# thomasdeppisch/eMagLS

Measured on AMD Instinct MI355X. Metric: eMagLS filter sets/s (N=4, 2702 dirs, 512 taps), higher is better.
Workload: dtype f64; 1 GPU; BASELINE config 3: getEMagLsFilters em32 r=4.2cm N=4 complex-SH, 2702 dirs, 512 taps, 48 kHz; one filter set per step, inputs resident in HBM; dirs=2702, taps=512, sim_order=19, bins=512, k_cut=43, designs_resident_per_gpu=128, designs_per_batch=32, batches_in_flight=4, distinct_hrir_sets_resident=20, parallelism=independent jobs per GPU, one RCCL gather

## Files before the change

emagls_amd/_lib.py:

```python
from __future__ import annotations

import ctypes as C
import os

_HERE = os.path.dirname(os.path.abspath(__file__))
LIB_PATH = os.environ.get("EMAGLS_LIB_PATH") or os.path.join(_HERE, "lib", "libemagls.so")

OK, ERR_ARG, ERR_UNSUPPORTED, ERR_HIP, ERR_NUMERIC = 0, 1, 2, 3, 4
BASIS = {"real": 0, "complex": 1}
KIND_LS, KIND_MAGLS, KIND_EMAGLS, KIND_EMAGLS2, KIND_FROM_ATF, KIND_EMA_CH, KIND_MAGLS_2D, KIND_EMA_SH = range(8)
RADIAL = {"tikhonov": 0, "softlimit": 1, "full": 2, "none": 3}
LAYOUT = {"sh": 0, "ch": 1}
MODEL = {"sh": 0, "emagls": 1, "emagls2": 2, "atf": 3, "ema_ch": 5, "ema_sh": 6}

c_dp = C.POINTER(C.c_double)
c_i64 = C.c_int64


class DesignDesc(C.Structure):
    _fields_ = [("kind", C.c_int), ("basis", C.c_int), ("order", C.c_int), ("fs", C.c_double), ("len", c_i64),
                ("nsamp", c_i64), ("ndirs", c_i64), ("mic_radius", C.c_double), ("nmics", c_i64),
                ("f_trans", C.c_double), ("atf_taps", c_i64), ("natf", c_i64), ("custom_basis", C.c_int),
                ("diffuseness", C.c_int), ("sim_order_pad", C.c_int)]


class PlanInfo(C.Structure):
    _fields_ = [("nfft", C.c_int), ("num_pos_freqs", C.c_int), ("k_cut", C.c_int), ("sim_order", C.c_int),
                ("num_sh_sim", C.c_int), ("num_channels", C.c_int), ("out_is_complex", C.c_int),
                ("out_rows", c_i64), ("out_cols", c_i64), ("grp_delay_l", C.c_double), ("grp_delay_r", C.c_double),
                ("mean_grid_dev_deg", C.c_double), ("num_sweep_launches", C.c_int), ("device_bytes", c_i64),
                ("gram_from", C.c_int), ("hh_end", C.c_int), ("hh_orders", C.c_int), ("g_first", C.c_int),
                ("sim_order_own", C.c_int), ("sweep_form", C.c_int), ("sweep_units", C.c_int)]


class Job(C.Structure):
    _fields_ = [("desc", DesignDesc), ("hL", C.c_void_p), ("hR", C.c_void_p), ("hrir_azi", C.c_void_p), ("hrir_zen", C.c_void_p),
                ("mic_azi", C.c_void_p), ("mic_zen", C.c_void_p), ("atf", C.c_void_p), ("atf_azi", C.c_void_p), ("atf_zen", C.c_void_p),
                ("wL", C.c_void_p), ("wR", C.c_void_p)]


JOBS_SHARE_GEOMETRY = 1
JOBS_INDEPENDENT = 2

SYMBOLS = {
    "emagls_last_error": (C.c_char_p, []),
    "emagls_version": (C.c_int, []),
    "emagls_device_count": (C.c_int, [C.POINTER(C.c_int)]),
    "emagls_set_device": (C.c_int, [C.c_int]),
    "emagls_cache_clear": (C.c_int, []),
    "emagls_cache_release_designs": (C.c_int, []),
    "emagls_fp64_peak_tflops": (C.c_int, [C.c_int, C.POINTER(C.c_double)]),
    "emagls_fp64_peak_tflops_ex": (C.c_int, [C.c_int, C.c_int, C.POINTER(C.c_double), C.POINTER(C.c_double)]),
    "emagls_self_test": (C.c_int, [C.c_int, C.POINTER(C.c_double)]),
    "emagls_debug_synth_operand": (C.c_int, [C.c_void_p, C.c_int, C.c_int, C.c_void_p, c_i64, C.c_int, C.c_void_p, C.c_void_p]),
    "emagls_debug_synth_cosines": (C.c_int, [C.c_void_p, C.c_void_p, c_i64, C.c_void_p, C.c_void_p, C.c_int, C.c_void_p]),
    "emagls_sh_basis": (C.c_int, [C.c_int, c_i64, C.c_void_p, C.c_void_p, C.c_int, C.c_void_p]),
    "emagls_sh_basis_device": (C.c_int, [C.c_int, c_i64, C.c_void_p, C.c_void_p, C.c_int, C.c_void_p, C.c_void_p]),
    "emagls_modal_bn": (C.c_int, [C.c_int, c_i64, C.c_void_p, C.c_void_p]),
    "emagls_get_ls_filters": (C.c_int, [C.c_void_p, C.c_void_p, c_i64, c_i64, C.c_void_p, C.c_void_p, C.c_int, C.c_int,
                                        C.c_void_p, C.c_void_p]),
    "emagls_get_magls_filters": (C.c_int, [C.c_void_p, C.c_void_p, c_i64, c_i64, C.c_void_p, C.c_void_p, C.c_int,
                                           C.c_double, c_i64, C.c_int, C.c_void_p, C.c_void_p]),
    "emagls_get_emagls_filters": (C.c_int, [C.c_void_p, C.c_void_p, c_i64, c_i64, C.c_void_p, C.c_void_p, C.c_double,
                                            C.c_void_p, C.c_void_p, c_i64, C.c_int, C.c_double, c_i64, C.c_int,
                                            C.c_void_p, C.c_void_p]),
    "emagls_get_emagls2_filters": (C.c_int, [C.c_void_p, C.c_void_p, c_i64, c_i64, C.c_void_p, C.c_void_p, C.c_double,
                                             C.c_void_p, C.c_void_p, c_i64, C.c_int, C.c_double, c_i64, C.c_int,
                                             C.c_void_p, C.c_void_p]),
    "emagls_get_emagls_filters_ema_in_ch": (C.c_int, [C.c_void_p, C.c_void_p, c_i64, c_i64, C.c_void_p, C.c_void_p, C.c_double,
                                                      C.c_void_p, c_i64, C.c_int, C.c_double, c_i64, C.c_int, C.c_void_p, C.c_void_p]),
    "emagls_get_emagls_filters_ema_in_sh": (C.c_int, [C.c_void_p, C.c_void_p, c_i64, c_i64, C.c_void_p, C.c_void_p, C.c_double,
                                                      C.c_void_p, c_i64, C.c_int, C.c_double, c_i64, C.c_int, C.c_void_p, C.c_void_p]),
    "emagls_get_emagls_filters_from_atf": (C.c_int, [C.c_void_p, C.c_void_p, c_i64, c_i64, C.c_void_p, C.c_void_p,
                                                     C.c_void_p, c_i64, c_i64, c_i64, C.c_void_p, C.c_void_p,
                                                     C.c_double, c_i64, C.c_double, C.c_void_p, C.c_void_p,
                                                     C.POINTER(C.c_double)]),
    "emagls_simulation_order": (C.c_int, [C.c_int, C.c_int, C.c_double, C.c_double]),
    "emagls_get_ls_filters_with_basis": (C.c_int, [C.c_void_p, C.c_void_p, c_i64, c_i64, C.c_void_p, C.c_int, C.c_int, C.c_void_p, C.c_void_p]),
    "emagls_get_magls_filters_with_basis": (C.c_int, [C.c_void_p, C.c_void_p, c_i64, c_i64, C.c_void_p, C.c_int, C.c_double, c_i64, C.c_int,
                                                      C.c_void_p, C.c_void_p]),
    "emagls_get_emagls_filters_with_basis": (C.c_int, [C.c_void_p, C.c_void_p, c_i64, c_i64, C.c_void_p, C.c_double, C.c_void_p, c_i64, C.c_int,
                                                       C.c_double, c_i64, C.c_int, C.c_void_p, C.c_void_p]),
    "emagls_get_emagls2_filters_with_basis": (C.c_int, [C.c_void_p, C.c_void_p, c_i64, c_i64, C.c_void_p, C.c_double, C.c_void_p, c_i64, C.c_int,
                                                        C.c_double, c_i64, C.c_int, C.c_void_p, C.c_void_p]),
    "emagls_plan_set_basis": (C.c_int, [C.c_void_p, C.c_void_p, C.c_void_p]),
    "emagls_binaural_decode": (C.c_int, [C.c_void_p, c_i64, c_i64, C.c_void_p, C.c_void_p, c_i64, C.c_int, C.c_void_p]),
    "emagls_binaural_decode_complex": (C.c_int, [C.c_void_p, C.c_int, c_i64, c_i64, C.c_void_p, C.c_void_p, C.c_int, c_i64, C.c_int,
                                                 C.c_void_p, C.c_void_p]),
    "emagls_binaural_decode_device": (C.c_int, [C.c_void_p, C.c_int, c_i64, c_i64, C.c_void_p, C.c_void_p, C.c_int, c_i64, C.c_void_p,
                                                C.c_void_p, C.c_void_p]),
    "emagls_rotate_yaw": (C.c_int, [C.c_void_p, C.c_int, c_i64, c_i64, C.c_int, C.c_int, C.c_void_p, c_i64, C.c_void_p]),
    "emagls_binaural_decode_render": (C.c_int, [C.c_void_p, C.c_int, c_i64, c_i64, C.c_void_p, C.c_void_p, C.c_int, c_i64, C.c_int,
                                                C.c_int, C.c_int, C.c_void_p, c_i64, C.c_void_p, c_i64, C.c_void_p, C.c_void_p]),
    "emagls_binaural_decode_render_device": (C.c_int, [C.c_void_p, C.c_int, c_i64, c_i64, C.c_void_p, C.c_void_p, C.c_int, c_i64,
                                                       C.c_int, C.c_int, C.c_void_p, c_i64, C.c_void_p, c_i64, C.c_void_p, C.c_void_p,
                                                       C.c_void_p]),
    "emagls_sh_rotation_matrix": (C.c_int, [C.c_int, C.c_int, C.c_double, C.c_double, C.c_double, C.c_void_p]),
    "emagls_rotate_sh": (C.c_int, [C.c_void_p, C.c_int, c_i64, c_i64, C.c_int, C.c_void_p, c_i64, C.c_void_p, c_i64, C.c_void_p, c_i64,
                                   C.c_void_p]),
    "emagls_binaural_decode_render_ypr": (C.c_int, [C.c_void_p, C.c_int, c_i64, c_i64, C.c_void_p, C.c_void_p, C.c_int, c_i64, C.c_int,
                                                    C.c_int, C.c_int, C.c_void_p, c_i64, C.c_void_p, c_i64, C.c_void_p, c_i64,
                                                    C.c_void_p, c_i64, C.c_void_p, C.c_void_p]),
    "emagls_binaural_decode_render_ypr_device": (C.c_int, [C.c_void_p, C.c_int, c_i64, c_i64, C.c_void_p, C.c_void_p, C.c_int, c_i64,
                                                           C.c_int, C.c_int, C.c_void_p, c_i64, C.c_void_p, c_i64, C.c_void_p, c_i64,
                                                           C.c_void_p, c_i64, C.c_void_p, C.c_void_p, C.c_void_p]),
    "emagls_resample_length": (c_i64, [c_i64, c_i64, c_i64]),
    "emagls_resample": (C.c_int, [C.c_void_p, C.c_int, c_i64, c_i64, c_i64, c_i64, C.c_void_p]),
    "emagls_resample_device": (C.c_int, [C.c_void_p, C.c_int, c_i64, c_i64, c_i64, c_i64, C.c_void_p, C.c_void_p]),
    "emagls_binaural_decode_render_fs": (C.c_int, [C.c_void_p, C.c_int, c_i64, c_i64, C.c_void_p, C.c_void_p, C.c_int, c_i64, C.c_int,
                                                   C.c_int, C.c_int, C.c_void_p, c_i64, C.c_void_p, c_i64, C.c_void_p, c_i64,
                                                   C.c_void_p, c_i64, C.c_double, C.c_double, C.c_double, C.c_void_p, C.c_void_p]),
    "emagls_binaural_decode_render_fs_device": (C.c_int, [C.c_void_p, C.c_int, c_i64, c_i64, C.c_void_p, C.c_void_p, C.c_int, c_i64,
                                                          C.c_int, C.c_int, C.c_void_p, c_i64, C.c_void_p, c_i64, C.c_void_p, c_i64,
                                                          C.c_void_p, c_i64, C.c_double, C.c_double, C.c_double, C.c_void_p,
                                                          C.c_void_p, C.c_void_p]),
    "emagls_decode_stream_create": (C.c_int, [c_i64, C.c_void_p, C.c_void_p, C.c_int, c_i64, C.c_int, C.c_int, C.c_int, c_i64,
                                              C.POINTER(C.c_void_p)]),
    "emagls_decode_stream_push": (C.c_int, [C.c_void_p, C.c_void_p, c_i64, C.c_void_p, c_i64, C.c_void_p, c_i64, C.c_void_p, c_i64,
                                            C.c_void_p]),
    "emagls_decode_stream_push_device": (C.c_int, [C.c_void_p, C.c_void_p, c_i64, C.c_void_p, c_i64, C.c_void_p, c_i64, C.c_void_p, c_i64,
                                                   C.c_void_p, C.c_void_p]),
    "emagls_decode_stream_reset": (C.c_int, [C.c_void_p]),
    "emagls_decode_stream_info": (C.c_int, [C.c_void_p, C.POINTER(c_i64), C.POINTER(c_i64), C.POINTER(c_i64), C.POINTER(c_i64),
                                            C.POINTER(C.c_int)]),
    "emagls_decode_stream_destroy": (C.c_int, [C.c_void_p]),
    "emagls_decode_stream_create_bank": (C.c_int, [c_i64, c_i64, C.c_void_p, C.c_void_p, C.c_int, c_i64, C.c_int, C.c_int, C.c_int, c_i64,
                                                   C.POINTER(C.c_void_p)]),
    "emagls_decode_stream_push_sets": (C.c_int, [C.c_void_p, C.c_void_p, c_i64, C.c_void_p, c_i64, C.c_void_p, c_i64, C.c_void_p, c_i64,
                                                 C.c_void_p, c_i64, C.c_void_p]),
    "emagls_decode_stream_push_sets_device": (C.c_int, [C.c_void_p, C.c_void_p, c_i64, C.c_void_p, c_i64, C.c_void_p, c_i64, C.c_void_p,
                                                        c_i64, C.c_void_p, c_i64, C.c_void_p, C.c_void_p]),
    "emagls_decode_stream_sets": (C.c_int, [C.c_void_p, C.POINTER(c_i64)]),
    "emagls_decode_group_create": (C.c_int, [c_i64, c_i64, C.c_void_p, C.c_void_p, C.c_int, c_i64, C.c_int, C.c_int, C.c_int, c_i64, c_i64,
                                             C.POINTER(C.c_void_p)]),
    "emagls_decode_group_push": (C.c_int, [C.c_void_p, C.c_void_p, c_i64, C.c_void_p, c_i64, C.c_void_p, c_i64, C.c_void_p, c_i64,
                                           C.c_void_p, c_i64, C.c_void_p]),
    "emagls_decode_group_push_device": (C.c_int, [C.c_void_p, C.c_void_p, c_i64, C.c_void_p, c_i64, C.c_void_p, c_i64, C.c_void_p, c_i64,
                                                  C.c_void_p, c_i64, C.c_void_p, C.c_void_p]),
    "emagls_decode_group_reset": (C.c_int, [C.c_void_p, c_i64]),
    "emagls_decode_group_info": (C.c_int, [C.c_void_p, C.POINTER(c_i64), C.POINTER(c_i64), C.POINTER(c_i64), C.POINTER(c_i64),
                                           C.POINTER(c_i64), C.POINTER(C.c_int)]),
    "emagls_decode_group_destroy": (C.c_int, [C.c_void_p]),
    "emagls_decode_stream_create_encoded": (C.c_int, [c_i64, C.c_void_p, C.c_int, c_i64, c_i64, C.c_void_p, C.c_void_p, C.c_int, c_i64, C.c_int,
                                                      C.c_int, c_i64, C.POINTER(C.c_void_p)]),
    "emagls_decode_group_create_encoded": (C.c_int, [c_i64, C.c_void_p, C.c_int, c_i64, c_i64, C.c_void_p, C.c_void_p, C.c_int, c_i64, C.c_int,
                                                     C.c_int, c_i64, c_i64, C.POINTER(C.c_void_p)]),
    "emagls_get_magls_filters_dc": (C.c_int, [C.c_void_p, C.c_void_p, c_i64, c_i64, C.c_void_p, C.c_void_p, C.c_int,
                                              C.c_double, c_i64, C.c_int, C.c_int, C.c_void_p, C.c_void_p]),
    "emagls_get_emagls_filters_dc": (C.c_int, [C.c_void_p, C.c_void_p, c_i64, c_i64, C.c_void_p, C.c_void_p, C.c_double,
                                               C.c_void_p, C.c_void_p, c_i64, C.c_int, C.c_double, c_i64, C.c_int, C.c_int,
                                               C.c_void_p, C.c_void_p]),
    "emagls_get_emagls2_filters_dc": (C.c_int, [C.c_void_p, C.c_void_p, c_i64, c_i64, C.c_void_p, C.c_void_p, C.c_double,
                                                C.c_void_p, C.c_void_p, c_i64, C.c_int, C.c_double, c_i64, C.c_int, C.c_int,
                                                C.c_void_p, C.c_void_p]),
    "emagls_get_magls_filters_2d": (C.c_int, [C.c_void_p, C.c_void_p, c_i64, c_i64, C.c_void_p, C.c_int, C.c_double, c_i64, C.c_int,
                                              C.c_void_p, C.c_void_p]),
    "emagls_get_radial_filter": (C.c_int, [C.c_int, C.c_double, C.c_double, c_i64, C.c_int, C.c_int, C.c_double, C.c_double, C.c_void_p]),
    "emagls_apply_radial_filter_rows": (c_i64, [c_i64, c_i64, C.c_int]),
    "emagls_apply_radial_filter": (C.c_int, [C.c_void_p, c_i64, C.c_int, C.c_double, C.c_double, c_i64, C.c_int, C.c_int, C.c_double,
                                             C.c_double, C.c_void_p]),
    "emagls_sh_encode": (C.c_int, [C.c_void_p, c_i64, c_i64, C.c_void_p, C.c_void_p, C.c_int, C.c_int, C.c_void_p]),
    "emagls_ch_basis": (C.c_int, [C.c_int, c_i64, C.c_void_p, C.c_int, C.c_void_p]),
    "emagls_get_smair_matrix": (C.c_int, [C.c_int, C.c_double, c_i64, C.c_int, C.c_double, C.c_void_p, C.c_void_p, c_i64, C.c_int, C.c_int,
                                          C.c_int, C.c_double, C.c_double, C.c_void_p, C.POINTER(C.c_int)]),
    "emagls_rendered_hrtfs": (C.c_int, [C.c_int, C.c_void_p, C.c_void_p, C.c_int, c_i64, c_i64, c_i64, C.c_void_p, C.c_void_p, c_i64, C.c_double,
                                        C.c_int, C.c_int, C.c_double, C.c_void_p, C.c_void_p, c_i64, C.c_void_p, c_i64, c_i64, C.c_void_p,
                                        C.c_void_p, c_i64, c_i64, C.c_void_p, C.c_void_p, C.c_void_p, C.c_void_p, C.c_void_p, C.c_void_p]),
    "emagls_eq_filter_nfft": (c_i64, [c_i64]),
    "emagls_get_magls_spherical_head_filter": (C.c_int, [C.c_double, C.c_int, C.c_double, c_i64, C.c_void_p, C.c_void_p]),
    "emagls_get_magls_array_diffuse_filter": (C.c_int, [C.c_double, C.c_void_p, C.c_void_p, c_i64, C.c_int, C.c_double, c_i64, C.c_int,
                                                        C.c_void_p, C.c_void_p]),
    "emagls_plan_create": (C.c_int, [C.POINTER(DesignDesc), C.POINTER(C.c_void_p)]),
    "emagls_plan_destroy": (C.c_int, [C.c_void_p]),
    "emagls_plan_set_hrir_grid": (C.c_int, [C.c_void_p, C.c_void_p, C.c_void_p]),
    "emagls_plan_set_mic_grid": (C.c_int, [C.c_void_p, C.c_void_p, C.c_void_p]),
    "emagls_plan_set_hrirs": (C.c_int, [C.c_void_p, C.c_void_p, C.c_void_p]),
    "emagls_plan_set_atfs": (C.c_int, [C.c_void_p, C.c_void_p, C.c_void_p, C.c_void_p]),
    "emagls_plan_execute": (C.c_int, [C.c_void_p]),
    "emagls_plan_synchronize": (C.c_int, [C.c_void_p]),
    "emagls_plan_get_filters": (C.c_int, [C.c_void_p, C.c_void_p, C.c_void_p]),
    "emagls_plan_get_info": (C.c_int, [C.c_void_p, C.POINTER(PlanInfo)]),
    "emagls_plan_sweep_form_in_batch": (C.c_int, [C.c_void_p, C.c_int, C.POINTER(C.c_int)]),
    "emagls_plan_set_profiling": (C.c_int, [C.c_void_p, C.c_int]),
    "emagls_plan_set_streams": (C.c_int, [C.c_void_p, C.c_int]),
    "emagls_plan_num_stages": (C.c_int, [C.c_void_p]),
    "emagls_plan_stage_name": (C.c_char_p, [C.c_void_p, C.c_int]),
    "emagls_plan_stage_times": (C.c_int, [C.c_void_p, c_dp, C.c_int]),
    "emagls_plan_sweep_kernel_time": (C.c_int, [C.c_void_p, c_dp, C.POINTER(C.c_int)]),
    "emagls_plan_debug_buffer": (C.c_int, [C.c_void_p, C.c_char_p, C.c_void_p, C.POINTER(C.c_size_t)]),
    "emagls_plan_stream": (C.c_void_p, [C.c_void_p]),
    "emagls_batch_create": (C.c_int, [C.POINTER(C.c_void_p), C.c_int, C.POINTER(C.c_void_p)]),
    "emagls_batch_execute": (C.c_int, [C.c_void_p]),
    "emagls_batch_synchronize": (C.c_int, [C.c_void_p]),
    "emagls_batch_get_filters": (C.c_int, [C.c_void_p, C.POINTER(C.c_void_p), C.POINTER(C.c_void_p)]),
    "emagls_batch_set_profiling": (C.c_int, [C.c_void_p, C.c_int]),
    "emagls_batch_lane_mode": (C.c_int, [C.c_void_p, C.POINTER(C.c_int)]),
    "emagls_batch_set_stream": (C.c_int, [C.c_void_p, C.c_void_p]),
    "emagls_set_batch_max": (C.c_int, [C.c_int, C.POINTER(C.c_int)]),
    "emagls_batch_shares_atf_side": (C.c_int, [C.c_void_p, C.POINTER(C.c_int)]),
    "emagls_design_hrir_sets": (C.c_int, [C.c_int, C.c_void_p, C.c_void_p, C.c_int64, C.c_int64, C.c_int64, C.c_void_p, C.c_void_p, C.c_double,
                                          C.c_void_p, C.c_void_p, C.c_int64, C.c_int, C.c_double, C.c_int64, C.c_int, C.c_void_p, C.c_void_p]),
    "emagls_from_atf_hrir_sets": (C.c_int, [C.c_void_p, C.c_void_p, C.c_int64, C.c_int64, C.c_int64, C.c_void_p, C.c_void_p, C.c_void_p, C.c_int64,
                                            C.c_int64, C.c_int64, C.c_void_p, C.c_void_p, C.c_double, C.c_int64, C.c_double, C.c_void_p, C.c_void_p,
                                            C.POINTER(C.c_double)]),
    "emagls_jobs_run": (C.c_int, [C.POINTER(Job), C.c_int64, C.c_int, C.c_int, C.c_int]),
    "emagls_design_out_shape": (C.c_int, [C.POINTER(DesignDesc), C.POINTER(c_i64), C.POINTER(c_i64), C.POINTER(C.c_int)]),
    "emagls_jobs_shard": (C.c_int, [C.POINTER(Job), C.c_int64, C.c_int, C.c_int, C.POINTER(C.c_int), C.POINTER(C.c_int), C.POINTER(C.c_int)]),
    "emagls_jobs_run_devices": (C.c_int, [C.POINTER(Job), C.c_int64, C.POINTER(C.c_int), C.c_int, C.c_int, C.c_int, C.c_int]),
    "emagls_jobs_set_profiling": (C.c_int, [C.c_int]),
    "emagls_jobs_sweep_times": (C.c_int, [C.POINTER(C.c_double), C.POINTER(C.c_int), C.c_int, C.POINTER(C.c_int)]),
    "emagls_batch_set_geometry_sharing": (C.c_int, [C.c_void_p, C.c_int]),
    "emagls_batch_shares_geometry": (C.c_int, [C.c_void_p, C.POINTER(C.c_int)]),
    "emagls_batch_geometry_runs": (C.c_int, [C.c_void_p, C.POINTER(C.c_longlong), C.POINTER(C.c_longlong)]),
    "emagls_jobs_geometry_runs": (C.c_int, [C.POINTER(C.c_longlong), C.POINTER(C.c_longlong), C.POINTER(C.c_longlong)]),
    "emagls_jobs_would_share_geometry": (C.c_int, [C.c_void_p, C.c_int, C.POINTER(C.c_int)]),
    "emagls_batch_set_side_stream": (C.c_int, [C.c_void_p, C.c_void_p]),
    "emagls_batch_set_streams": (C.c_int, [C.c_void_p, C.c_int]),
    "emagls_batch_set_stage_order": (C.c_int, [C.c_void_p, C.c_int]),
    "emagls_batch_sweep_time": (C.c_int, [C.c_void_p, C.POINTER(C.c_double)]),
    "emagls_batch_destroy": (C.c_int, [C.c_void_p]),
}


class EmaglsError(RuntimeError):
    def __init__(self, code, msg):
        super().__init__("emagls error %d: %s" % (code, msg))
        self.code = code


_lib = None


def load():
    global _lib
    if _lib is not None:
        return _lib
    if not os.path.exists(LIB_PATH):
        raise ImportError("HIP library not built: %s is missing (run `python -m emagls_amd.build`)" % LIB_PATH)
    lib = C.CDLL(LIB_PATH, mode=C.RTLD_GLOBAL)
    for name, (res, args) in SYMBOLS.items():
        fn = getattr(lib, name)
        fn.restype = res
        fn.argtypes = args
    _lib = lib
    return lib


def check(rc):
    if rc != OK:
        raise EmaglsError(rc, load().emagls_last_error().decode("utf-8", "replace"))
```

emagls_amd/csrc/batch_run.hip:

```cpp
#include "host_internal.hpp"

void emagls_batch_forget(emagls_batch* b, emagls_plan* p) {
    for (auto& q : b->plans) if (q == p) q = nullptr;
}

namespace {
void batch_sweep_stage(emagls_batch& b) {
    const int nb = (int)b.plans.size();
    std::vector<HalfSweepArgs> ha((size_t)nb);
    for (int j = 0; j < nb; ++j) ha[j] = emagls_half_args(*b.plans[j]);
    if (b.atf_share || b.geo_share)
        for (int j = 1; j < nb; ++j) {
            ha[j].G = ha[0].G; ha[j].Yri = ha[0].Yri; ha[j].Mw = ha[0].Mw; ha[j].cond_ok = ha[0].cond_ok;
            ha[j].bsc = ha[0].bsc; ha[j].smap = ha[0].smap;
            ha[j].skip_flag = ha[0].skip_flag;
        }
    const bool reg = b.plans[0]->sweep_persist && reg_sweep_wanted(b.plans.data(), nb);
    for (auto* q : b.plans) q->reg_sweep = reg;
    if (!reg && nb > SWEEP_MULTI_MAX) throw Error(EMAGLS_ERR_UNSUPPORTED, "internal: more than 16 designs in a batch need the register-resident sweep");
    HalfSweepMulti h{};
    h.n = std::min(nb, SWEEP_MULTI_MAX);
    for (int j = 0; j < h.n; ++j) h.a[j] = ha[j];
    emagls_plan& q0 = *b.plans[0];
    const int kk0 = std::max(q0.kcut0, 1);
    if (kk0 >= q0.P) return;
    if (q0.sweep_persist) {
        hipStream_t ss = b.stream;
        {
            SweepGate gate(ss, reg ? reg_sweep_gate_cost((int)q0.D, nb) : 0);
            if (b.lanes) { BatchScope sc(nb, b.stride); launch_zero(q0.get("ll"), q0.bufs["ll"].bytes, ss); }
            else for (auto* q : b.plans) launch_zero(q->get("ll"), q->bufs["ll"].bytes, ss);
            if (reg) {
                if (!b.sweep_args_dev) HIP_CHECK(hipMalloc(&b.sweep_args_dev, sizeof(HalfSweepArgs) * (size_t)REG_SWEEP_MAX));
                reg_args_upload(ha.data(), nb, b.sweep_args_dev, b.sweep_args_last, ss);
            }
            if (b.prof_level >= 1) HIP_CHECK(hipEventRecord(b.sweep_ev[0], ss));
            if (reg) launch_sweep_reg(static_cast<const HalfSweepArgs*>(b.sweep_args_dev), ha[0], nb, ss);
            else if (q0.synth) launch_sweep_synth(h, ss); else launch_sweep_persist(h, ss);
            if (b.prof_level >= 1) HIP_CHECK(hipEventRecord(b.sweep_ev[1], ss));
        }
        if (ss != b.stream) b.depend(b.stream, ss);
        return;
    }
    for (int kb = kk0; kb < q0.P; ++kb) launch_sweep_half(h, kb, b.stream);
    launch_sweep_half_finalize(h, q0.P - 1, b.stream);
}

static int stagger_mode() {
    static const int m = [] { const char* e = getenv("EMAGLS_STAGGER"); return e ? atoi(e) : 1; }();
    return m;
}
bool batch_defers_hh(const emagls_batch& b) {
    static const int defer_mode = [] { const char* e = getenv("EMAGLS_DEFER_HH"); return e ? atoi(e) : 1; }();
    if (!b.lanes || !(b.alone || defer_mode == 2) || b.geo_share || b.atf_share) return false;
    for (const emagls_plan* p : b.plans) if (!p || !plan_defers_hh_route(*p)) return false;
    return true;
}
void batch_lanes_part(emagls_batch& b, int part, int first, int count, hipStream_t st, int group = 0) {
    emagls_plan& p0 = *b.plans[first];
    const int ns = (part == 0 && b.groups == 1) ? b.nstreams : 1;
    int order = 0;
    if (part == 0 && ns == 1) {
        const int sm = stagger_mode();
        if (sm == 1) order = b.groups > 1 ? 1 + group % 2 : (b.order_hint ? 1 + (b.order_hint - 1) % 2 : 0);
        else if (sm >= 10) order = group == 0 ? sm / 10 % 10 : sm % 10;
    }
    Scoped stream(p0.stream, st);
    Scoped nstreams(p0.nstreams, ns);
    Scoped stage_order(p0.stage_order, order);
    Scoped side0(p0.side[0], ns > 1 ? b.side[0] : p0.side[0]), side1(p0.side[1], ns > 1 ? b.side[1] : p0.side[1]),
        side2(p0.side[2], ns > 1 ? b.side[2] : p0.side[2]);
    Scoped pre_phase(p0.pre_phase, part == 3 ? 2 : (part == 0 && b.defer_hh) ? 1 : 0);
    BatchScope sc(count, b.stride);
    if (part == 0) plan_pre_stage(p0); else if (part == 3) emagls_pre_sweep(p0); else emagls_post_sweep(p0);
}
void mark_executed(emagls_batch& b, int launches) {
    for (auto* p : b.plans) { p->executed = true; p->sweep_launches = launches; }
}
int sweep_launch_count(const emagls_plan& p0) { return p0.sweep_persist ? 1 : p0.P - std::max(p0.kcut0, 1); }
int batch_group_first(const emagls_batch& b, int g) { const int n = (int)b.plans.size(), h = (n + b.groups - 1) / b.groups; return std::min(n, g * h); }
void batch_execute_lanes(emagls_batch& b) {
    const bool replay = b.use_graph && b.eager_runs >= 1 && !(b.groups == 1 && b.nstreams > 1);
    const int n = (int)b.plans.size();
    const int ng = b.groups;
    for (int g = 1; g < ng; ++g) if (!b.side[g - 1]) b.side[g - 1] = emagls::pool_stream_take();
    hipStream_t gs[4] = {b.stream, b.stream, b.stream, b.stream};
    for (int g = 1; g < ng; ++g) gs[g] = b.side[g - 1];
    if (!replay || !b.group[0]) b.defer_hh = batch_defers_hh(b);
    const bool defer = b.defer_hh;
    if (defer) for (int g = 0; g < ng; ++g) if (!b.hh_stream[g]) b.hh_stream[g] = emagls::pool_stream_take();
    if (replay && !b.group[0]) {
        for (int g = 0; g < ng; ++g) {
            const int f = batch_group_first(b, g), c = batch_group_first(b, g + 1) - f;
            b.group[g].capture(gs[g], [&] { batch_lanes_part(b, 0, f, c, gs[g], g); });
            if (defer) b.group_hh[g].capture(b.hh_stream[g], [&] { batch_lanes_part(b, 3, f, c, b.hh_stream[g], g); });
        }
        b.post.capture(b.stream, [&] { batch_lanes_part(b, 2, 0, n, b.stream); });
    }
    b.used = 0;
    for (int g = 1; g < ng; ++g) b.depend(gs[g], b.stream);
    if (replay && ng > 1) {
        hipError_t err[4] = {hipSuccess, hipSuccess, hipSuccess, hipSuccess};
        const int dev = b.device;
        std::vector<std::thread> th;
        for (int g = 1; g < ng; ++g)
            th.emplace_back([&, g] { err[g] = hipSetDevice(dev); if (err[g] == hipSuccess) err[g] = hipGraphLaunch(b.group[g].exec, gs[g]); });
        err[0] = hipGraphLaunch(b.group[0].exec, gs[0]);
        for (auto& t : th) t.join();
        for (int g = 0; g < ng; ++g) HIP_CHECK(err[g]);
    } else {
        for (int g = 0; g < ng; ++g) {
            const int f = batch_group_first(b, g), c = batch_group_first(b, g + 1) - f;
            if (replay) b.group[g].launch(gs[g]); else batch_lanes_part(b, 0, f, c, gs[g], g);
        }
    }
    if (defer) for (int g = 0; g < ng; ++g) b.depend(b.hh_stream[g], gs[g]);
    for (int g = 1; g < ng; ++g) b.depend(b.stream, gs[g]);
    batch_sweep_stage(b);
    if (defer) {
        for (int g = 0; g < ng; ++g) {
            const int f = batch_group_first(b, g), c = batch_group_first(b, g + 1) - f;
            if (replay) b.group_hh[g].launch(b.hh_stream[g]); else batch_lanes_part(b, 3, f, c, b.hh_stream[g], g);
            b.depend(b.stream, b.hh_stream[g]);
        }
    }
    if (replay) b.post.launch(b.stream); else batch_lanes_part(b, 2, 0, n, b.stream);
    mark_executed(b, sweep_launch_count(*b.plans[0]));
    if (!replay) ++b.eager_runs;
}

bool batch_inputs_same(emagls_batch& b, std::initializer_list<const char*> names, uint64_t& checked_version, bool& same) {
    uint64_t ver = 0;
    for (auto* p : b.plans) ver = ver * 1000003ull + p->atf_side_version;
    if (ver == checked_version) return same;
    if (!b.cmp_flag) HIP_CHECK(hipMalloc(&b.cmp_flag, 16));
    HIP_CHECK(hipStreamSynchronize(b.stream));
    HIP_CHECK(hipMemsetAsync(b.cmp_flag, 0, 16, b.stream));
    emagls_plan& p0 = *b.plans[0];
    for (size_t j = 1; j < b.plans.size(); ++j)
        for (const char* name : names) launch_compare_words(p0.get(name), b.plans[j]->get(name), p0.bufs[name].bytes, b.cmp_flag, b.stream);
    int differ = 0;
    HIP_CHECK(hipMemcpyAsync(&differ, b.cmp_flag, sizeof differ, hipMemcpyDeviceToHost, b.stream));
    HIP_CHECK(hipStreamSynchronize(b.stream));
    checked_version = ver;
    return same = differ == 0;
}
void batch_set_sharing(emagls_batch& b, bool& field, bool share) {
    if (share == field) return;
    for (auto* p : b.plans) drop_plan_graphs(*p);
    drop_batch_graphs(b);
    if (&field == &b.geo_share) batch_geo_forget(b);
    field = share;
}
void batch_run_two_graphs(emagls_batch& b, CapturedGraph& pre, void (*stage)(emagls_batch&, int), int pre_part, int launches) {
    const bool replay = b.use_graph && b.eager_runs >= 1;
    if (replay && !pre) pre.capture(b.stream, [&] { stage(b, pre_part); });
    if (replay && !b.post) b.post.capture(b.stream, [&] { stage(b, 2); });
    b.used = 0;
    if (replay) pre.launch(b.stream); else stage(b, pre_part);
    batch_sweep_stage(b);
    if (replay) b.post.launch(b.stream); else stage(b, 2);
    mark_executed(b, launches);
    if (!replay) ++b.eager_runs;
}
template <typename Pre> void batch_run_per_plan(emagls_batch& b, bool replay, Pre pre, void (*post)(emagls_plan&), int launches) {
    emagls_plan& p0 = *b.plans[0];
    if (replay && !p0.pre) {
        for (auto* p : b.plans) p->pre.capture(p->stream, [&] { pre(*p); });
        if (!p0.sweep_persist) b.group[0].capture(b.stream, [&] { batch_sweep_stage(b); });
    }
    b.used = 0;
    for (auto* p : b.plans) b.depend(p->stream, b.stream);
    for (auto* p : b.plans) {
        if (replay) p->pre.launch(p->stream); else pre(*p);
        b.depend(b.stream, p->stream);
    }
    if (b.atf_share)
        for (size_t j = 1; j < b.plans.size(); ++j) from_atf_ls_rows(*b.plans[j], p0, b.stream);
    if (p0.sweep_persist) batch_sweep_stage(b);
    else if (replay) b.group[0].launch(b.stream); else batch_sweep_stage(b);
    for (auto* p : b.plans) {
        b.depend(p->stream, b.stream);
        post(*p);
        b.depend(b.stream, p->stream);
    }
    mark_executed(b, launches);
    if (!replay) ++b.eager_runs;
}

void batch_atf_decide_sharing(emagls_batch& b) {
    const bool same = batch_inputs_same(b, {"atf", "atf_azi", "atf_zen", "hrir_azi", "hrir_zen"}, b.atf_checked_version, b.atf_inputs_same);
    bool routes_ok = true;
    for (auto* p : b.plans) routes_ok = routes_ok && p->gram_from == 1 && p->sweep_persist == b.plans[0]->sweep_persist;
    batch_set_sharing(b, b.atf_share, same && routes_ok && b.plans.size() > 1);
}
void from_atf_subject_pre_stage(emagls_plan& p) {
    subject_reset(p, p.stream);
    from_atf_subject_stage(p);
}
void batch_atf_shared_stage(emagls_batch& b, int part) {
    emagls_plan& p0 = *b.plans[0];
    StreamLoan loan(b.plans, b.stream);
    if (part == 2) {
        for (auto* p : b.plans) from_atf_post_sweep(*p);
        return;
    }
    plan_pre_stage(p0);
    for (size_t j = 1; j < b.plans.size(); ++j) {
        emagls_plan& p = *b.plans[j];
        subject_reset(p, b.stream);
        HIP_CHECK(hipMemcpyAsync(p.get("match_idx"), p0.get("match_idx"), sizeof(int64_t) * (size_t)p.Dm, hipMemcpyDeviceToDevice, b.stream));
        HIP_CHECK(hipMemcpyAsync(p.get("match_dev"), p0.get("match_dev"), sizeof(double) * (size_t)p.Dm, hipMemcpyDeviceToDevice, b.stream));
        HIP_CHECK(hipMemcpyAsync(p.get("mean_dev"), p0.get("mean_dev"), sizeof(double), hipMemcpyDeviceToDevice, b.stream));
        stage_prologue(p, 1, p.hrir_smaller ? nullptr : p.get<int64_t>("match_idx"), p.Dm);
        from_atf_ls_rows(p, p0, b.stream);
    }
}
void batch_execute_atf(emagls_batch& b) {
    for (auto* p : b.plans)
        if (!p->have_hrirs || !p->have_hrir_grid || !p->have_atfs)
            throw Error(EMAGLS_ERR_ARG, "every plan of the batch needs its HRIRs, its grid and the ATFs");
    batch_atf_decide_sharing(b);
    emagls_plan& p0 = *b.plans[0];
    static const bool one_stream = [] { const char* e = getenv("EMAGLS_ATF_ONE_STREAM"); return !(e && e[0] == '0'); }();
    if (b.atf_share && p0.sweep_persist && one_stream) { batch_run_two_graphs(b, b.group[0], batch_atf_shared_stage, 0, 1); return; }
    batch_run_per_plan(b, b.use_graph && b.eager_runs >= 1,
                       [&](emagls_plan& p) { if (b.atf_share && &p != &p0) from_atf_subject_pre_stage(p); else plan_pre_stage(p); },
                       from_atf_post_sweep, sweep_launch_count(p0));
}

uint64_t batch_geo_version(const emagls_batch& b) {
    uint64_t ver = 0;
    for (const emagls_plan* p : b.plans) ver = (ver * 1000003ull + p->atf_side_version) * 1000003ull + p->solo_runs;
    return ver;
}
void batch_geo_decide_sharing(emagls_batch& b) {
    bool share = false;
    if (b.geo_want && b.plans.size() > 1) {
        emagls_plan& p0 = *b.plans[0];
        bool eligible = (p0.d.kind == EMAGLS_KIND_EMAGLS || p0.d.kind == EMAGLS_KIND_EMAGLS2 || p0.d.kind == EMAGLS_KIND_EMA_CH) && !p0.wide &&
                        !p0.diffuse && !p0.custom_basis;
        for (auto* p : b.plans) {
            const emagls_design_desc &x = p->d, &y = p0.d;
            eligible = eligible && x.kind == y.kind && x.order == y.order && x.fs == y.fs && x.len == y.len && x.nsamp == y.nsamp &&
                       x.ndirs == y.ndirs && x.mic_radius == y.mic_radius && x.nmics == y.nmics && x.basis == y.basis &&
                       x.sim_order_pad == y.sim_order_pad && p->wide == p0.wide && p->diffuse == p0.diffuse && p->custom_basis == p0.custom_basis &&
                       p->real_internal == p0.real_internal && p->gram_from == p0.gram_from && p->hh_end == p0.hh_end && p->n_h == p0.n_h &&
                       p->g0 == p0.g0 && p->sweep_persist == p0.sweep_persist;
        }
        share = eligible && batch_inputs_same(b, {"hrir_azi", "hrir_zen", "mic_azi", "mic_zen"}, b.geo_checked_version, b.geo_inputs_same);
    }
    batch_set_sharing(b, b.geo_share, share);
}
void geo_hrir_side(emagls_plan& h, emagls_plan& g, emagls_plan& p0, hipStream_t st) {
    subject_reset(h, st);
    h.sync_used = 0;
    hrir_spectra(h, p0, st);
    if (g.hh_end > 1) {
        hrir_hh_rows(h, g, st);
        hrir_hh_back(hh_factor_args(h, g, nullptr, g.get<double>("cond_ok")), g, st);
    }
    hrir_gram_ls_rows(h, g, p0, true, st);
    if (p0.synth) launch_synth_winit(h.get("W"), p0.get("Pm"), p0.C, (int)p0.d.nmics, std::max(p0.kcut0, 1), p0.P, h.get("Winit"), st, true);
}
void batch_geo_stage(emagls_batch& b, int part) {
    emagls_plan& p0 = *b.plans[0];
    StreamLoan loan(b.plans, b.stream);
    const int n = (int)b.plans.size();
    auto hrir_side = [&](int first) {
        if (first >= n) return;
        if (b.lanes) {
            BatchScope sc(n - first, b.stride);
            geo_hrir_side(*b.plans[first], *b.plans[first], p0, b.stream);
        } else {
            for (int j = first; j < n; ++j) geo_hrir_side(*b.plans[j], p0, p0, b.stream);
        }
    };
    if (part == 1) {
        hrir_side(0);
    } else if (part == 0) {
        plan_pre_stage(p0);
        if (b.lanes && n > 1) {
            emagls_plan& g = p0;
            const bool cb = g.cplx_basis;
            const int gf = g.gram_from, hh_end = g.hh_end, ldSh = g.ldS_h;
            const int ls_end = std::min(g.kcut0, g.P);
            const size_t g_stride_b = sizeof(cplx) * (size_t)g.C * g.ldD;
            auto bc = [&](const char* name, size_t off, size_t bytes) {
                if (!g.has(name) || bytes == 0) return;
                bytes = std::min(bytes, g.bufs[name].bytes - off);
                launch_broadcast_lanes(g.get<char>(name) + off, bytes, b.stride, n - 1, b.stream);
            };
            if (hh_end > 1) {
                bc("Yc", 0, g.bufs["Yc"].bytes);
                bc(cb ? "R" : "Rc", 0, g.bufs[cb ? "R" : "Rc"].bytes);
                bc("Vws", 0, sizeof(cplx) * (size_t)(hh_end - 1) * g.C * ldSh);
                bc("Nw", 0, sizeof(cplx) * (size_t)(hh_end - 1) * g.C * g.C);
                bc("tauw", 0, sizeof(double) * (size_t)(hh_end - 1) * g.C);
                bc("cond_ok", 0, sizeof(double) * (size_t)g.P);
            }
            if (gf > 0 && gf < ls_end) {
                bc("G", (size_t)(gf - g.g0) * g_stride_b, (size_t)(ls_end - gf) * g_stride_b);
                bc("Mw", 0, sizeof(cplx) * (size_t)ls_end * g.C * g.C);
            }
        }
        hrir_side(1);
    } else if (b.lanes) {
        BatchScope sc(n, b.stride);
        Scoped from(p0.geo_from, &p0);
        emagls_post_sweep(p0);
    } else {
        for (auto* p : b.plans) {
            Scoped from(p->geo_from, &p0);
            emagls_post_sweep(*p);
        }
    }
}
void batch_execute_geo(emagls_batch& b) {
    const bool warm = batch_geo_next_is_warm(b);
    if (!warm) {
        b.geo_kept_version = ~0ull;
        b.geo_ran_version = batch_geo_version(b);
        b.geo_cold_pending = true;
    }
    batch_run_two_graphs(b, warm ? b.warm : b.group[0], batch_geo_stage, warm ? 1 : 0, sweep_launch_count(*b.plans[0]));
    b.last_form = warm ? 2 : 1;
    ++(warm ? b.geo_warm_runs : b.geo_cold_runs);
}

void batch_magls_decide_sharing(emagls_batch& b, bool sweep_needed) {
    bool share = false;
    emagls_plan& p0 = *b.plans[0];
    if (b.geo_want && b.plans.size() > 1 && !p0.custom_basis && !p0.diffuse && (p0.sweep_persist || !sweep_needed)) {
        share = batch_inputs_same(b, {"hrir_azi", "hrir_zen"}, b.geo_checked_version, b.geo_inputs_same);
        for (auto* p : b.plans) share = share && !p->custom_basis && p->d.fs == p0.d.fs;
    }
    batch_set_sharing(b, b.geo_share, share);
}
void batch_magls_stage(emagls_batch& b, int part) {
    emagls_plan& g = *b.plans[0];
    StreamLoan loan(b.plans, b.stream);
    if (part == 2) {
        for (auto* p : b.plans) magls_post_sweep(*p);
        return;
    }
    for (size_t j = 0; j < b.plans.size(); ++j) {
        emagls_plan& p = *b.plans[j];
        if (j == 0 || !b.geo_share) { plan_pre_stage(p); continue; }
        subject_reset(p, b.stream);
        stage_prologue(p, 0, nullptr, p.D);
        launch_ls_apply(p.get("Hc"), p.ldD, std::min(p.kcut0, p.P), g.get("Ypinv"), g.cplx_basis, g.ldD, (int)p.D, p.C, p.P, 0,
                        std::min(p.kcut0, p.P), p.get("W"), b.stream);
    }
}
void batch_execute_magls(emagls_batch& b) {
    emagls_plan& p0 = *b.plans[0];
    for (auto* p : b.plans)
        if (!p->have_hrirs || (p->custom_basis ? !p->have_basis : !p->have_hrir_grid))
            throw Error(EMAGLS_ERR_ARG, "every plan of the batch needs its grid (or SH matrix) and HRIRs");
    if (p0.d.kind == EMAGLS_KIND_LS) {
        batch_magls_decide_sharing(b, false);
        for (size_t j = 0; j < b.plans.size(); ++j) {
            emagls_plan& p = *b.plans[j];
            {
                Scoped stream(p.stream, b.stream);
                p.stage_names.clear();
                launch_zero(p.get("flag"), sizeof(int) * NFLAG, b.stream);
                if (j == 0 || !b.geo_share) execute_ls(p);
                else launch_ls_filters(p.get<double>("hL"), p.get<double>("hR"), p.d.nsamp, (int)p.D, p0.get("Ypinv"), p0.cplx_basis, p0.ldD, p.C,
                                       p.get("wL"), p.get("wR"), b.stream);
            }
            p.executed = true;
        }
        return;
    }
    bool persist = true;
    for (auto* p : b.plans) persist = persist && p->sweep_persist;
    if (!persist) {
        batch_set_sharing(b, b.geo_share, false);
        for (auto* p : b.plans) {
            Scoped stream(p->stream, b.stream);
            plan_execute(*p);
        }
        return;
    }
    batch_magls_decide_sharing(b, true);
    batch_run_two_graphs(b, b.group[0], batch_magls_stage, 0, 1);
}
bool batch_unify_routes_once(emagls_batch& b) {
    int gf = 0, nh = 0;
    bool differ = false;
    for (auto* p : b.plans) {
        if (p->gram_from <= 0 || p->d.kind == EMAGLS_KIND_EMA_SH) return false;
        differ = differ || p->gram_from != b.plans[0]->gram_from || p->n_h != b.plans[0]->n_h;
        gf = std::max(gf, p->gram_from);
        nh = std::max(nh, p->n_h);
    }
    if (!differ) return false;
    for (auto* p : b.plans) {
        if (p->gram_from == gf && p->n_h == nh) continue;
        const int keep_floor = p->gram_floor, keep_nh = p->nh_floor;
        try {
            p->gram_floor = std::max(p->gram_floor, gf);
            p->nh_floor = nh;
            plan_routes(*p);
            plan_alloc_routes(*p);
        } catch (const Error& e) {
            if (getenv("EMAGLS_DEBUG_LANES")) fprintf(stderr, "common routes refused: %s\n", e.what());
            p->gram_floor = keep_floor; p->nh_floor = keep_nh;
            plan_routes(*p);
            plan_alloc_routes(*p);
            return false;
        }
        drop_plan_graphs(*p);
    }
    return true;
}
void batch_unify_routes(emagls_batch& b) {
    for (int it = 0; it < 4 && batch_unify_routes_once(b); ++it) {}
}
std::vector<int> batch_read_flags(emagls_batch& b) {
    const size_t n = b.plans.size();
    std::vector<int> flags(NFLAG * n, 0);
    for (size_t j = 0; j < n; ++j)
        HIP_CHECK(hipMemcpyAsync(&flags[NFLAG * j], b.plans[j]->get("flag"), NFLAG * sizeof(int), hipMemcpyDeviceToHost, b.stream));
    HIP_CHECK(hipStreamSynchronize(b.stream));
    return flags;
}
}

namespace emagls {
void batch_geo_forget(emagls_batch& b) {
    b.geo_kept_version = ~0ull;
    b.geo_cold_pending = false;
}
bool batch_geo_next_is_warm(const emagls_batch& b) {
    static const bool keep = [] { const char* e = getenv("EMAGLS_GEO_KEEP"); return !(e && e[0] == '0'); }();
    if (!keep || !b.geo_share || b.geo_kept_version == ~0ull || b.geo_kept_version != batch_geo_version(b)) return false;
    for (const emagls_plan* p : b.plans) if (p->prof_level > 0) return false;
    return true;
}

void batch_execute(emagls_batch& b) {
    for (auto* p : b.plans)
        if (!p) throw Error(EMAGLS_ERR_ARG, "a plan of this batch has been destroyed");
    b.last_form = 0;
    if (b.atf) { batch_execute_atf(b); return; }
    if (b.magls) { batch_execute_magls(b); return; }
    for (auto* p : b.plans)
        if (!p->have_hrirs || (p->custom_basis ? !p->have_basis : (!p->have_hrir_grid || !p->have_mic_grid)))
            throw Error(EMAGLS_ERR_ARG, "every plan of the batch needs its grids (or SH matrices) and HRIRs");
    batch_geo_decide_sharing(b);
    if (b.geo_share) { batch_execute_geo(b); return; }
    if (b.lanes) {
        batch_execute_lanes(b);
        return;
    }
    const bool replay = b.use_graph && b.eager_runs >= 1 && std::none_of(b.plans.begin(), b.plans.end(), [](const emagls_plan* p) { return forks_streams(*p); });
    batch_run_per_plan(b, replay, plan_pre_stage, emagls_post_sweep, b.plans[0]->P - std::max(b.plans[0]->kcut0, 1));
}
void drop_batch_graphs(emagls_batch& b) {
    for (auto& g : b.group) g.reset();
    for (auto& g : b.group_hh) g.reset();
    b.post.reset();
    b.warm.reset();
    b.eager_runs = 0;
}

void batch_unify_synth(emagls_batch& b) {
    bool all = true, any = false;
    for (auto* p : b.plans) { all = all && p->synth; any = any || p->synth; }
    if (all || !any) return;
    for (auto* p : b.plans)
        if (p->synth) { p->synth_block = true; plan_alloc_routes(*p); HIP_CHECK(hipStreamSynchronize(p->stream)); drop_plan_graphs(*p); }
}
void batch_decide_residency(emagls_batch& b) {
    emagls_plan& f0 = *b.plans[0];
    const int n = (int)b.plans.size();
    if (f0.d.kind == EMAGLS_KIND_LS) return;
    bool all_persist = true;
    for (auto* p : b.plans) all_persist = all_persist && p->sweep_persist;
    if (!all_persist) return;
    const int64_t Dh0 = f0.d.kind == EMAGLS_KIND_FROM_ATF ? f0.Dm : f0.D;
    const bool fits = f0.synth ? (reg_sweep_wanted(b.plans.data(), n) || (n <= SWEEP_MULTI_MAX && synth_sweep_fits((int)Dh0, (int)f0.d.nmics, f0.simOrder + 1, n)))
                               : (n <= SWEEP_MULTI_MAX && persist_sweep_fits((int)Dh0, f0.C, n));
    if (fits) return;
    for (auto* p : b.plans) {
        p->sweep_persist = false;
        if (p->synth_want) { plan_alloc_routes(*p); HIP_CHECK(hipStreamSynchronize(p->stream)); }
    }
}

void batch_try_lanes(emagls_batch& b) {
    if (const char* e = getenv("EMAGLS_BATCH_LANES")) if (e[0] == '0') return;
    emagls_plan& q = *b.plans[0];
    if (!q.sweep_persist) return;
    for (auto* p : b.plans)
        if (p->S != q.S || p->simOrder != q.simOrder || p->d.kind != q.d.kind || p->C != q.C || p->P != q.P) return;
    trace_mark("lanes: start");
    batch_unify_routes(b);
    trace_mark("lanes: routes unified");
    batch_unify_synth(b);
    const bool dbg = getenv("EMAGLS_DEBUG_LANES") != nullptr;
    for (auto* p : b.plans) {
        if (p->S != q.S || p->simOrder != q.simOrder || p->nOut != q.nOut || p->nfft != q.nfft || p->ldS != q.ldS || p->ldD != q.ldD ||
            p->Dpad != q.Dpad || p->k_cut != q.k_cut || p->cplx_basis != q.cplx_basis || p->out_cplx != q.out_cplx ||
            p->d.kind != q.d.kind || p->d.nsamp != q.d.nsamp || p->d.nmics != q.d.nmics || p->d.len != q.d.len || p->d.order != q.d.order ||
            p->bufs.size() != q.bufs.size()) {
            if (dbg) fprintf(stderr, "lanes refused: shape fields differ (bufs %zu vs %zu, gram_from %d vs %d, n_h %d vs %d)\n", p->bufs.size(),
                             q.bufs.size(), p->gram_from, q.gram_from, p->n_h, q.n_h);
            return;
        }
        auto it = q.bufs.begin();
        for (auto& kv : p->bufs) {
            if (kv.first != it->first || kv.second.bytes != it->second.bytes) {
                if (dbg) fprintf(stderr, "lanes refused: buffer %s %zu vs %s %zu (gram_from %d vs %d, hh_end %d vs %d, n_h %d vs %d)\n", kv.first.c_str(),
                                 kv.second.bytes, it->first.c_str(), it->second.bytes, p->gram_from, q.gram_from, p->hh_end, q.hh_end, p->n_h, q.n_h);
                return;
            }
            ++it;
        }
    }
    size_t stride = 0;
    std::vector<size_t> off;
    for (auto& kv : q.bufs) {
        off.push_back(stride);
        stride += (kv.second.bytes + 255) / 256 * 256;
    }
    stride = (stride + 4095) / 4096 * 4096;
    trace_mark("lanes: shapes compared");
    auto arena = std::make_shared<Arena>();
    {
        const size_t need = stride * b.plans.size();
        arena->base = BlockPool::get().take(need, &arena->bytes, BlockPool::size_class(need + need / 8));
    }
    for (size_t j = 0; j < b.plans.size(); ++j) {
        emagls_plan& p = *b.plans[j];
        size_t i = 0;
        BufferMoves mv{};
        for (auto& kv : p.bufs) {
            char* dst = static_cast<char*>(arena->base) + j * stride + off[i++];
            if ((reinterpret_cast<uintptr_t>(kv.second.p) & 15) != 0) { HIP_CHECK(hipMemcpyAsync(dst, kv.second.p, kv.second.bytes, hipMemcpyDeviceToDevice, b.stream)); continue; }
            mv.src[mv.n] = kv.second.p; mv.dst[mv.n] = dst; mv.bytes[mv.n] = kv.second.bytes;
            if (++mv.n == 96) { launch_move_buffers(mv, b.stream); mv.n = 0; }
        }
        launch_move_buffers(mv, b.stream);
    }
    trace_mark("lanes: arena taken, copies enqueued");
    HIP_CHECK(hipStreamSynchronize(b.stream));
    trace_mark("lanes: copies done");
    for (size_t j = 0; j < b.plans.size(); ++j) {
        emagls_plan& p = *b.plans[j];
        size_t i = 0;
        for (auto& kv : p.bufs) {
            if (kv.second.owned) HIP_CHECK(hipFree(kv.second.p));
            kv.second.p = static_cast<char*>(arena->base) + j * stride + off[i++];
            kv.second.owned = false;
        }
        p.release_slabs();
        p.arena = arena;
        drop_plan_graphs(p);
    }
    HIP_CHECK(hipDeviceSynchronize());
    b.lanes = true;
    b.stride = stride;
    {
        const char* e = getenv("EMAGLS_BATCH_GROUPS");
        const int cap = e ? std::max(1, std::min(4, atoi(e))) : 2;
        b.groups = std::max(1, std::min(cap, (int)ceil_div((int64_t)b.plans.size(), 8)));
    }
}

void batch_redo(emagls_batch& b, const std::vector<int>& flags) {
    int any[NFLAG] = {};
    for (size_t j = 0; j < b.plans.size(); ++j) for (int i = 0; i < NFLAG; ++i) any[i] = std::max(any[i], flags[NFLAG * j + i]);
    bool moved = false;
    for (auto* q : b.plans) {
        const int64_t before = q->total_bytes;
        plan_recover(*q, any, true);
        moved = moved || q->total_bytes != before;
        drop_plan_graphs(*q);
    }
    drop_batch_graphs(b);
    batch_geo_forget(b);
    {
        const std::vector<int64_t> before = [&] { std::vector<int64_t> v; for (auto* q : b.plans) v.push_back(q->total_bytes); return v; }();
        batch_unify_synth(b);
        batch_decide_residency(b);
        for (size_t j = 0; j < b.plans.size(); ++j) moved = moved || b.plans[j]->total_bytes != before[j];
    }
    if (b.lanes && moved) {
        b.lanes = false;
        batch_try_lanes(b);
    }
    batch_execute(b);
    HIP_CHECK(hipStreamSynchronize(b.stream));
}
void plan_check_flags(emagls_plan& p) {
    int flag[NFLAG] = {};
    HIP_CHECK(hipMemcpy(flag, p.get("flag"), sizeof flag, hipMemcpyDeviceToHost));
    if (plan_recover(p, flag, false)) {
        if (p.owner) {
            emagls_batch& b = *p.owner;
            for (auto* q : b.plans) if (!q) throw Error(EMAGLS_ERR_ARG, "a plan of this batch has been destroyed");
            batch_redo(b, batch_read_flags(b));
        } else {
            plan_recover(p, flag, true);
            drop_plan_graphs(p);
            plan_execute(p);
            HIP_CHECK(hipStreamSynchronize(p.stream));
        }
        HIP_CHECK(hipMemcpy(flag, p.get("flag"), sizeof flag, hipMemcpyDeviceToHost));
        if (plan_recover(p, flag, false)) {
            if (p.owner) batch_redo(*p.owner, batch_read_flags(*p.owner));
            else { plan_recover(p, flag, true); drop_plan_graphs(p); plan_execute(p); HIP_CHECK(hipStreamSynchronize(p.stream)); }
            HIP_CHECK(hipMemcpy(flag, p.get("flag"), sizeof flag, hipMemcpyDeviceToHost));
        }
    }
    if (p.persist_suspended) {
        p.persist_suspended = false;
        p.sweep_persist = true;
    }
    throw_fatal_flags(flag);
    p.geo_done_version = p.geo_run_version;
}
}
```

emagls_amd/csrc/capi.hip:

```cpp
#include "host_internal.hpp"

namespace {

struct CachedPlan {
    std::unique_ptr<emagls_plan> plan;
    emagls_design_desc desc{};
    int device = 0;
    bool busy = false;
    uint64_t last_use = 0;
};
std::mutex g_cache_mu;
std::vector<CachedPlan> g_cache;
uint64_t g_cache_tick = 0;

size_t plan_cache_capacity() {
    static const size_t cap = [] { const char* e = getenv("EMAGLS_PLAN_CACHE"); return e ? (size_t)std::max(0, atoi(e)) : (size_t)4; }();
    return cap;
}

int one_shot(const emagls_design_desc& desc, const double* hL, const double* hR, const double* azi, const double* zen,
             const double* mic_azi, const double* mic_zen, const double* atf, const double* atf_azi, const double* atf_zen,
             void* wL, void* wR, double* mean_dev, const void* Y_hrir = nullptr, const void* Y_mic = nullptr) {
    return guarded([&] {
        int dev = 0;
        HIP_CHECK(hipGetDevice(&dev));
        emagls_plan* p = nullptr;
        std::unique_ptr<emagls_plan> fresh;
        bool cached = false;
        {
            std::lock_guard<std::mutex> lk(g_cache_mu);
            for (auto& c : g_cache)
                if (!c.busy && c.device == dev && same_desc(c.desc, desc)) { c.busy = true; p = c.plan.get(); cached = true; break; }
        }
        if (!p) {
            fresh.reset(new emagls_plan);
            fresh->d = desc;
            plan_setup(*fresh);
            if (array_kind(desc.kind)) {
                const char* e = getenv("EMAGLS_ONESHOT_STREAMS");
                fresh->nstreams = e ? std::max(1, std::min(3, atoi(e))) : 1;
                fresh->alone = true;
            }
            p = fresh.get();
        }
        auto release = [&](bool ok) {
            std::lock_guard<std::mutex> lk(g_cache_mu);
            if (cached) {
                for (size_t i = 0; i < g_cache.size(); ++i)
                    if (g_cache[i].plan.get() == p) {
                        if (ok) { g_cache[i].busy = false; g_cache[i].last_use = ++g_cache_tick; }
                        else g_cache.erase(g_cache.begin() + i);
                        break;
                    }
            } else if (ok && plan_cache_capacity() > 0) {
                if (g_cache.size() >= plan_cache_capacity()) {
                    size_t victim = g_cache.size();
                    for (size_t i = 0; i < g_cache.size(); ++i)
                        if (!g_cache[i].busy && (victim == g_cache.size() || g_cache[i].last_use < g_cache[victim].last_use)) victim = i;
                    if (victim < g_cache.size()) g_cache.erase(g_cache.begin() + victim);
                }
                if (g_cache.size() < plan_cache_capacity()) {
                    CachedPlan c;
                    c.plan = std::move(fresh);
                    c.desc = desc; c.device = dev; c.busy = false; c.last_use = ++g_cache_tick;
                    g_cache.push_back(std::move(c));
                }
            }
        };
        try {
            auto req = [](int rc) { if (rc != EMAGLS_OK) throw Error(rc, g_last_error); };
            if (desc.custom_basis) {
                req(emagls_plan_set_basis(p, Y_hrir, Y_mic));
            } else {
                req(emagls_plan_set_hrir_grid(p, azi, zen));
                if (mic_azi) req(emagls_plan_set_mic_grid(p, mic_azi, mic_zen));
            }
            req(emagls_plan_set_hrirs(p, hL, hR));
            if (atf) req(emagls_plan_set_atfs(p, atf, atf_azi, atf_zen));
            plan_execute(*p);
            req(emagls_plan_get_filters(p, wL, wR));
            if (mean_dev) {
                emagls_plan_info info;
                req(emagls_plan_get_info(p, &info));
                *mean_dev = info.mean_grid_dev_deg;
            }
        } catch (...) {
            release(false);
            throw;
        }
        release(true);
    });
}

std::atomic<int> g_batch_max{[] { const char* e = getenv("EMAGLS_BATCH_MAX"); return e ? std::max(1, std::min(REG_SWEEP_MAX, atoi(e))) : 8; }()};
}

namespace emagls {
bool same_desc(const emagls_design_desc& a, const emagls_design_desc& b) {
    return a.kind == b.kind && a.basis == b.basis && a.order == b.order && a.fs == b.fs && a.len == b.len && a.nsamp == b.nsamp &&
           a.ndirs == b.ndirs && a.mic_radius == b.mic_radius && a.nmics == b.nmics && a.f_trans == b.f_trans &&
           a.atf_taps == b.atf_taps && a.natf == b.natf && a.custom_basis == b.custom_basis && a.diffuseness == b.diffuseness &&
           a.sim_order_pad == b.sim_order_pad;
}
thread_local int g_batch_max_override = 0;
}

extern "C" {

const char* emagls_last_error(void) { return g_last_error.c_str(); }
int emagls_version(void) { return 100; }

int emagls_device_count(int* count) {
    return guarded([&] {
        if (!count) throw Error(EMAGLS_ERR_ARG, "null pointer");
        HIP_CHECK(hipGetDeviceCount(count));
    });
}
int emagls_set_device(int device) {
    return guarded([&] { HIP_CHECK(hipSetDevice(device)); });
}

void emagls_sets_cache_clear_internal();
void emagls_atfsets_cache_clear_internal();
void emagls_jobs_cache_clear_internal();
int emagls_cache_release_designs(void) {
    return guarded([&] {
        {
            std::lock_guard<std::mutex> lk(g_cache_mu);
            for (size_t i = g_cache.size(); i-- > 0;)
                if (!g_cache[i].busy) g_cache.erase(g_cache.begin() + i);
        }
        emagls_sets_cache_clear_internal();
        emagls_atfsets_cache_clear_internal();
        emagls_jobs_cache_clear_internal();
    });
}
int emagls_cache_clear(void) {
    return guarded([&] {
        {
            std::lock_guard<std::mutex> lk(g_cache_mu);
            for (size_t i = g_cache.size(); i-- > 0;)
                if (!g_cache[i].busy) g_cache.erase(g_cache.begin() + i);
        }
        decode_family_cache_clear();
        emagls_sets_cache_clear_internal();
        emagls_atfsets_cache_clear_internal();
        emagls_jobs_cache_clear_internal();
        BlockPool::get().clear();
    });
}

int emagls_fp64_peak_tflops(int which, double* tflops) {
    return guarded([&] {
        if (!tflops || which < 0 || which > 2) throw Error(EMAGLS_ERR_ARG, "invalid argument");
        *tflops = measure_fp64_peak(which, 3);
    });
}

int emagls_self_test(int which, double* max_err) {
    return guarded([&] {
        if (!max_err || which < 0 || which > 2) throw Error(EMAGLS_ERR_ARG, "invalid argument");
        *max_err = which == 0 ? reg_contract_selftest() : gram_tile_selftest(which == 2);
    });
}

int emagls_debug_synth_operand(const void* bsc, int nbins, int nord_pad, const double* x, int64_t nx, int gs, void* g_plus, void* g_minus) {
    return guarded([&] { synth_operand_debug(bsc, nbins, nord_pad, x, nx, gs, g_plus, g_minus); });
}

int emagls_debug_synth_cosines(const double* dir_azi, const double* dir_zen, int64_t ndirs, const double* mic_azi, const double* mic_zen, int nmics, double* x2) {
    return guarded([&] { synth_cosines_debug(dir_azi, dir_zen, ndirs, mic_azi, mic_zen, nmics, x2); });
}

int emagls_fp64_peak_tflops_ex(int which, int burst, double* tflops, double* shader_mhz) {
    return guarded([&] {
        if (!tflops || which < 0 || which > 2) throw Error(EMAGLS_ERR_ARG, "invalid argument");
        *tflops = measure_fp64_peak(which, 3, burst != 0, shader_mhz);
    });
}

int emagls_sh_basis(int order, int64_t ndirs, const double* azi, const double* zen, int basis, void* Y) {
    return guarded([&] {
        if (order < 0 || ndirs < 0 || !azi || !zen || !Y) throw Error(EMAGLS_ERR_ARG, "invalid argument");
        if (ndirs == 0) return;
        const bool cb = basis == EMAGLS_BASIS_COMPLEX;
        const size_t S = (size_t)(order + 1) * (order + 1);
        double *d_azi = nullptr, *d_zen = nullptr, *d_tab = nullptr;
        void* d_Y = nullptr;
        auto cleanup = [&] { hipFree(d_azi); hipFree(d_zen); hipFree(d_tab); hipFree(d_Y); };
        try {
            HIP_CHECK(hipMalloc(&d_azi, sizeof(double) * ndirs));
            HIP_CHECK(hipMalloc(&d_zen, sizeof(double) * ndirs));
            HIP_CHECK(hipMalloc(&d_tab, sizeof(double) * sh_coeff_count(order)));
            HIP_CHECK(hipMalloc(&d_Y, esz(cb) * S * ndirs));
            HIP_CHECK(hipMemcpy(d_azi, azi, sizeof(double) * ndirs, hipMemcpyDefault));
            HIP_CHECK(hipMemcpy(d_zen, zen, sizeof(double) * ndirs, hipMemcpyDefault));
            launch_sh_coeff(order, d_tab, nullptr);
            launch_sh_basis(order, ndirs, d_azi, d_zen, d_tab, cb, d_Y, ndirs, nullptr);
            HIP_CHECK(hipDeviceSynchronize());
            HIP_CHECK(hipMemcpy(Y, d_Y, esz(cb) * S * ndirs, hipMemcpyDefault));
        } catch (...) { cleanup(); throw; }
        cleanup();
    });
}

int emagls_sh_basis_device(int order, int64_t ndirs, const double* d_azi, const double* d_zen, int basis, void* d_Y,
                           void* stream) {
    return guarded([&] {
        if (order < 0 || ndirs < 0 || !d_azi || !d_zen || !d_Y) throw Error(EMAGLS_ERR_ARG, "invalid argument");
        if (ndirs == 0) return;
        thread_local int tab_order = -1;
        thread_local double* tab = nullptr;
        hipStream_t st = (hipStream_t)stream;
        if (tab_order != order) {
            if (tab) { HIP_CHECK(hipFree(tab)); tab = nullptr; }
            HIP_CHECK(hipMalloc(&tab, sizeof(double) * sh_coeff_count(order)));
            tab_order = order;
            launch_sh_coeff(order, tab, st);
        }
        launch_sh_basis(order, ndirs, d_azi, d_zen, tab, basis == EMAGLS_BASIS_COMPLEX, d_Y, ndirs, st);
    });
}

int emagls_modal_bn(int order, int64_t nfreq, const double* kr, void* bn) {
    return guarded([&] {
        if (order < 0 || nfreq < 0 || !kr || !bn) throw Error(EMAGLS_ERR_ARG, "invalid argument");
        if (nfreq == 0) return;
        double* d_kr = nullptr;
        void* d_bn = nullptr;
        auto cleanup = [&] { hipFree(d_kr); hipFree(d_bn); };
        try {
            HIP_CHECK(hipMalloc(&d_kr, sizeof(double) * nfreq));
            HIP_CHECK(hipMalloc(&d_bn, sizeof(cplx) * nfreq * (order + 1)));
            HIP_CHECK(hipMemcpy(d_kr, kr, sizeof(double) * nfreq, hipMemcpyDefault));
            launch_modal_bn(order, nfreq, d_kr, 1.0, 1.0, d_bn, 1, nfreq, nullptr);
            HIP_CHECK(hipDeviceSynchronize());
            HIP_CHECK(hipMemcpy(bn, d_bn, sizeof(cplx) * nfreq * (order + 1), hipMemcpyDefault));
        } catch (...) { cleanup(); throw; }
        cleanup();
    });
}

int emagls_plan_create(const emagls_design_desc* desc, emagls_plan** plan) {
    return guarded([&] {
        if (!desc || !plan) throw Error(EMAGLS_ERR_ARG, "null pointer");
        std::unique_ptr<emagls_plan> p(new emagls_plan);
        p->d = *desc;
        plan_setup(*p);
        *plan = p.release();
    });
}
int emagls_plan_destroy(emagls_plan* plan) {
    return guarded([&] {
        DeviceGuard dg(plan ? plan->device : -1);
        delete plan;
    });
}
int emagls_plan_set_hrir_grid(emagls_plan* p, const double* azi, const double* zen) {
    return guarded([&] {
        DeviceGuard dg(p ? p->device : -1);
        if (!p || !azi) throw Error(EMAGLS_ERR_ARG, "null pointer");
        std::vector<double> equator;
        if (p->d.kind == EMAGLS_KIND_MAGLS_2D) { equator.assign((size_t)p->d.ndirs, kPi / 2.0); zen = equator.data(); }
        if (!zen) throw Error(EMAGLS_ERR_ARG, "null pointer");
        p->upload("hrir_azi", azi, sizeof(double) * p->d.ndirs);
        p->upload("hrir_zen", zen, sizeof(double) * p->d.ndirs);
        HIP_CHECK(hipStreamSynchronize(p->stream));
        p->have_hrir_grid = true;
        ++p->atf_side_version;
    });
}
int emagls_plan_set_mic_grid(emagls_plan* p, const double* azi, const double* zen) {
    return guarded([&] {
        DeviceGuard dg(p ? p->device : -1);
        if (!p || !azi) throw Error(EMAGLS_ERR_ARG, "null pointer");
        if (!p->has("mic_azi")) throw Error(EMAGLS_ERR_ARG, "this design kind has no microphone grid");
        std::vector<double> equator;
        if (p->d.kind == EMAGLS_KIND_EMA_CH || p->d.kind == EMAGLS_KIND_EMA_SH) { equator.assign((size_t)p->d.nmics, kPi / 2.0); zen = equator.data(); }
        if (!zen) throw Error(EMAGLS_ERR_ARG, "null pointer");
        p->upload("mic_azi", azi, sizeof(double) * p->d.nmics);
        p->upload("mic_zen", zen, sizeof(double) * p->d.nmics);
        if (p->has("smap")) {
            int smap[34];
            synth_pairing(azi, zen, (int)p->d.nmics, smap);
            p->upload("smap", smap, sizeof smap);
            p->synth_units = smap[32] + smap[33];
            HIP_CHECK(hipStreamSynchronize(p->stream));
        }
        std::vector<double> kr(p->P);
        for (int k = 0; k < p->P; ++k) {
            const double f = (double)k * (p->d.fs / 2.0) / (double)(p->P - 1);
            kr[k] = 2.0 * kPi * f / C_SOUND * p->d.mic_radius;
        }
        p->upload("kr", kr.data(), sizeof(double) * p->P);
        HIP_CHECK(hipStreamSynchronize(p->stream));
        p->have_mic_grid = true;
        ++p->atf_side_version;
    });
}
int emagls_plan_set_basis(emagls_plan* p, const void* Y_hrir, const void* Y_mic) {
    return guarded([&] {
        DeviceGuard dg(p ? p->device : -1);
        if (!p || !Y_hrir) throw Error(EMAGLS_ERR_ARG, "null pointer");
        if (!p->custom_basis) throw Error(EMAGLS_ERR_ARG, "the plan was not created with custom_basis = 1");
        const size_t es = esz(p->cplx_basis);
        HIP_CHECK(hipMemcpy2DAsync(p->get("Ycm"), (size_t)p->ldD * es, Y_hrir, (size_t)p->D * es, (size_t)p->D * es, (size_t)p->S, hipMemcpyDefault,
                                   p->stream));
        if (array_kind(p->d.kind)) {
            if (!Y_mic) throw Error(EMAGLS_ERR_ARG, "the array designs need the SH matrix of the microphone grid too");
            p->upload("Ymic_cm", Y_mic, es * (size_t)p->S * p->d.nmics);
            std::vector<double> kr(p->P);
            for (int k = 0; k < p->P; ++k) kr[k] = 2.0 * kPi * ((double)k * (p->d.fs / 2.0) / (double)(p->P - 1)) / C_SOUND * p->d.mic_radius;
            p->upload("kr", kr.data(), sizeof(double) * p->P);
        }
        HIP_CHECK(hipStreamSynchronize(p->stream));
        p->have_basis = true;
    });
}
int emagls_plan_set_hrirs(emagls_plan* p, const double* hL, const double* hR) {
    return guarded([&] {
        DeviceGuard dg(p ? p->device : -1);
        if (!p || !hL || !hR) throw Error(EMAGLS_ERR_ARG, "null pointer");
        p->upload("hL", hL, sizeof(double) * p->d.nsamp * p->d.ndirs);
        p->upload("hR", hR, sizeof(double) * p->d.nsamp * p->d.ndirs);
        HIP_CHECK(hipStreamSynchronize(p->stream));
        p->have_hrirs = true;
    });
}
int emagls_plan_set_atfs(emagls_plan* p, const double* atf, const double* azi, const double* zen) {
    return guarded([&] {
        DeviceGuard dg(p ? p->device : -1);
        if (!p || !atf || !azi || !zen) throw Error(EMAGLS_ERR_ARG, "null pointer");
        if (!p->has("atf")) throw Error(EMAGLS_ERR_ARG, "this design kind has no ATFs");
        p->upload("atf", atf, sizeof(double) * p->d.atf_taps * p->d.nmics * p->d.natf);
        p->upload("atf_azi", azi, sizeof(double) * p->d.natf);
        p->upload("atf_zen", zen, sizeof(double) * p->d.natf);
        HIP_CHECK(hipStreamSynchronize(p->stream));
        p->have_atfs = true;
        ++p->atf_side_version;
    });
}
int emagls_plan_execute(emagls_plan* p) {
    return guarded([&] {
        DeviceGuard dg(p ? p->device : -1);
        if (!p) throw Error(EMAGLS_ERR_ARG, "null pointer");
        plan_execute(*p);
    });
}
int emagls_plan_synchronize(emagls_plan* p) {
    return guarded([&] {
        DeviceGuard dg(p ? p->device : -1);
        if (!p) throw Error(EMAGLS_ERR_ARG, "null pointer");
        HIP_CHECK(hipStreamSynchronize(p->sync_stream ? p->sync_stream : p->stream));
    });
}
int emagls_plan_get_filters(emagls_plan* p, void* wL, void* wR) {
    return guarded([&] {
        DeviceGuard dg(p ? p->device : -1);
        if (!p || !wL || !wR) throw Error(EMAGLS_ERR_ARG, "null pointer");
        if (!p->executed) throw Error(EMAGLS_ERR_ARG, "plan has not been executed");
        HIP_CHECK(hipStreamSynchronize(p->sync_stream ? p->sync_stream : p->stream));
        plan_check_flags(*p);
        const size_t bytes = (p->out_cplx ? sizeof(cplx) : sizeof(double)) * (size_t)p->out_rows * p->out_cols;
        HIP_CHECK(hipMemcpy(wL, p->get("wL"), bytes, hipMemcpyDefault));
        HIP_CHECK(hipMemcpy(wR, p->get("wR"), bytes, hipMemcpyDefault));
    });
}
int emagls_plan_sweep_form_in_batch(emagls_plan* p, int designs, int* form) {
    return guarded([&] {
        DeviceGuard dg(p ? p->device : -1);
        if (!p || !form || designs < 1 || designs > REG_SWEEP_MAX) throw Error(EMAGLS_ERR_ARG, "emagls_plan_sweep_form_in_batch: null pointer or designs outside 1..32");
        std::vector<emagls_plan*> same((size_t)designs, p);
        const bool reg = p->synth && reg_sweep_wanted(same.data(), designs);
        *form = p->d.kind == EMAGLS_KIND_LS ? 0 : (p->synth ? (reg ? 3 : 2) : (p->sweep_persist ? 1 : 0));
    });
}
int emagls_plan_get_info(emagls_plan* p, emagls_plan_info* info) {
    return guarded([&] {
        DeviceGuard dg(p ? p->device : -1);
        if (!p || !info) throw Error(EMAGLS_ERR_ARG, "null pointer");
        std::memset(info, 0, sizeof *info);
        info->nfft = p->nfft; info->num_pos_freqs = p->P; info->k_cut = p->k_cut; info->sim_order = p->simOrder;
        info->num_sh_sim = p->S; info->num_channels = p->C; info->out_is_complex = p->out_cplx;
        info->out_rows = p->out_rows; info->out_cols = p->out_cols; info->num_sweep_launches = p->sweep_launches;
        info->device_bytes = p->total_bytes;
        info->gram_from = p->gram_from; info->hh_end = p->hh_end; info->hh_orders = p->n_h + 1; info->g_first = p->g0;
        info->sim_order_own = array_kind(p->d.kind) ? p->simOrderOwn : p->simOrder;
        bool reg = false;
        if (p->synth) {
            bool whole = p->owner != nullptr;
            if (whole) for (auto* q : p->owner->plans) whole = whole && q != nullptr;
            reg = whole ? reg_sweep_wanted(p->owner->plans.data(), (int)p->owner->plans.size()) : reg_sweep_wanted(&p, 1);
        }
        info->sweep_form = p->d.kind == EMAGLS_KIND_LS ? 0 : (p->synth ? (reg ? 3 : 2) : (p->sweep_persist ? 1 : 0));
        info->sweep_units = p->synth ? p->synth_units : 0;
        if (p->executed) {
            HIP_CHECK(hipStreamSynchronize(p->stream));
            double g[2];
            HIP_CHECK(hipMemcpy(g, p->get("grpd"), sizeof g, hipMemcpyDeviceToHost));
            info->grp_delay_l = g[0]; info->grp_delay_r = g[1];
            if (p->has("mean_dev")) HIP_CHECK(hipMemcpy(&info->mean_grid_dev_deg, p->get("mean_dev"), sizeof(double), hipMemcpyDeviceToHost));
        }
    });
}
int emagls_plan_set_profiling(emagls_plan* p, int level) {
    return guarded([&] {
        DeviceGuard dg(p ? p->device : -1);
        if (!p) throw Error(EMAGLS_ERR_ARG, "null pointer");
        p->prof_level = level;
    });
}
int emagls_plan_set_streams(emagls_plan* p, int nstreams) {
    return guarded([&] {
        DeviceGuard dg(p ? p->device : -1);
        if (!p) throw Error(EMAGLS_ERR_ARG, "null pointer");
        if (nstreams < 1 || nstreams > 4) throw Error(EMAGLS_ERR_ARG, "nstreams must be 1..4");
        HIP_CHECK(hipStreamSynchronize(p->stream));
        drop_plan_graphs(*p);
        p->nstreams = nstreams;
    });
}
int emagls_plan_num_stages(emagls_plan* p) { return p ? (int)p->stage_names.size() : 0; }
const char* emagls_plan_stage_name(emagls_plan* p, int i) {
    if (!p || i < 0 || i >= (int)p->stage_names.size()) return "";
    return p->stage_names[i].c_str();
}
int emagls_plan_stage_times(emagls_plan* p, double* ms, int n) {
    return guarded([&] {
        DeviceGuard dg(p ? p->device : -1);
        if (!p || !ms) throw Error(EMAGLS_ERR_ARG, "null pointer");
        HIP_CHECK(hipStreamSynchronize(p->stream));
        const int ns = (int)p->stage_names.size();
        for (int i = 0; i < n; ++i) {
            ms[i] = 0.0;
            if (i >= 1 && i < ns) {
                float t = 0.f;
                HIP_CHECK(hipEventElapsedTime(&t, p->stage_events[i - 1], p->stage_events[i]));
                ms[i] = t;
            }
        }
    });
}
int emagls_plan_sweep_kernel_time(emagls_plan* p, double* total_ms, int* launches) {
    return guarded([&] {
        DeviceGuard dg(p ? p->device : -1);
        if (!p || !total_ms || !launches) throw Error(EMAGLS_ERR_ARG, "null pointer");
        HIP_CHECK(hipStreamSynchronize(p->stream));
        double tot = 0.0;
        int n = 0;
        if (p->prof_level >= 2) {
            for (int i = 0; i < p->sweep_launches && 2 * (size_t)i + 1 < p->sweep_events.size(); ++i) {
                float t = 0.f;
                HIP_CHECK(hipEventElapsedTime(&t, p->sweep_events[2 * i], p->sweep_events[2 * i + 1]));
                tot += t;
                ++n;
            }
        }
        *total_ms = tot;
        *launches = n;
    });
}
int emagls_plan_debug_buffer(emagls_plan* p, const char* name, void* dst, size_t* nbytes) {
    return guarded([&] {
        DeviceGuard dg(p ? p->device : -1);
        if (!p || !name || !nbytes) throw Error(EMAGLS_ERR_ARG, "null pointer");
        auto it = p->bufs.find(name);
        if (it == p->bufs.end()) throw Error(EMAGLS_ERR_ARG, std::string("unknown buffer ") + name);
        if (!dst) { *nbytes = it->second.bytes; return; }
        HIP_CHECK(hipStreamSynchronize(p->stream));
        const size_t n = std::min(*nbytes, it->second.bytes);
        HIP_CHECK(hipMemcpy(dst, it->second.p, n, hipMemcpyDeviceToHost));
        *nbytes = n;
    });
}
void* emagls_plan_stream(emagls_plan* p) { return p ? (void*)p->stream : nullptr; }

int emagls_batch_create(emagls_plan** plans, int nplans, emagls_batch** batch) {
    return guarded([&] {
        if (!plans || !batch || nplans < 1) throw Error(EMAGLS_ERR_ARG, "invalid argument");
        const int batch_max = std::max(g_batch_max.load(), g_batch_max_override);
        if (nplans > batch_max)
            throw Error(EMAGLS_ERR_UNSUPPORTED, batch_max >= REG_SWEEP_MAX ? "at most 32 designs per batch"
                                                                             : "at most 8 designs per batch (emagls_set_batch_max(16) / EMAGLS_BATCH_MAX=16 allows 16)");
        std::unique_ptr<emagls_batch> b(new emagls_batch);
        for (int j = 0; j < nplans; ++j) {
            emagls_plan* p = plans[j];
            if (!p) throw Error(EMAGLS_ERR_ARG, "null plan");
            if (!array_kind(p->d.kind) && p->d.kind != EMAGLS_KIND_FROM_ATF && !magls_kind(p->d.kind) && p->d.kind != EMAGLS_KIND_LS)
                throw Error(EMAGLS_ERR_UNSUPPORTED, "batches take eMagLS / eMagLS2 / EMAinCH / EMAinSH plans, LS / MagLS / MagLS-2D plans, or FromAtf plans "
                                                    "(subjects of one ATF set)");
            if ((p->d.kind == EMAGLS_KIND_LS) != (plans[0]->d.kind == EMAGLS_KIND_LS) ||
                (p->d.kind == EMAGLS_KIND_LS && (p->cplx_basis != plans[0]->cplx_basis || p->d.order != plans[0]->d.order || p->d.nsamp != plans[0]->d.nsamp)))
                throw Error(EMAGLS_ERR_ARG, "LS plans share a batch only with LS plans of the same order, basis and HRIR length");
            if ((p->d.kind == EMAGLS_KIND_FROM_ATF) != (plans[0]->d.kind == EMAGLS_KIND_FROM_ATF))
                throw Error(EMAGLS_ERR_ARG, "FromAtf plans cannot share a batch with array designs");
            if (magls_kind(p->d.kind) != magls_kind(plans[0]->d.kind) || (magls_kind(p->d.kind) && p->d.kind != plans[0]->d.kind))
                throw Error(EMAGLS_ERR_ARG, "MagLS plans share a batch only with MagLS plans of the same kind");
            if (magls_kind(p->d.kind) && (p->diffuse != plans[0]->diffuse || p->cplx_basis != plans[0]->cplx_basis || p->d.order != plans[0]->d.order))
                throw Error(EMAGLS_ERR_ARG, "all designs of a batch must have the same shape (order, basis, constraint)");
            if (p->wide) throw Error(EMAGLS_ERR_UNSUPPORTED, "designs with more than 32 channels run one at a time");
            if (p->owner) throw Error(EMAGLS_ERR_ARG, "a plan belongs to another batch (destroy that batch first)");
            if (p->device != plans[0]->device) throw Error(EMAGLS_ERR_ARG, "the plans of a batch must live on one device");
            for (int i = 0; i < j; ++i) if (plans[i] == p) throw Error(EMAGLS_ERR_ARG, "the same plan appears twice in the batch");
            const emagls_plan* q = plans[0];
            if (p->P != q->P || p->kcut0 != q->kcut0 || p->C != q->C || p->nWG_dense != q->nWG_dense || p->D != q->D || p->sweep_persist != q->sweep_persist ||
                p->Dm != q->Dm || p->d.natf != q->d.natf || p->d.atf_taps != q->d.atf_taps || p->d.len != q->d.len)
                throw Error(EMAGLS_ERR_ARG, "all designs of a batch must have the same shape (directions, channels, bins, k_cut)");
            b->plans.push_back(p);
        }
        b->device = b->plans[0]->device;
        DeviceGuard dg(b->device);
        b->stream = StreamPool::get().take();
        if (const char* ng = getenv("EMAGLS_NO_GRAPH")) b->use_graph = !(ng[0] == '1');
        const bool array_batch = b->plans[0]->d.kind != EMAGLS_KIND_FROM_ATF && !magls_kind(b->plans[0]->d.kind) && b->plans[0]->d.kind != EMAGLS_KIND_LS;
        for (auto* p : b->plans) HIP_CHECK(hipStreamSynchronize(p->stream));
        trace_mark("batch create: plans synchronised");
        if (array_batch) batch_unify_synth(*b);
        trace_mark("batch create: sweep form unified");
        batch_decide_residency(*b);
        trace_mark("batch create: residency decided");
        if (nplans > SWEEP_MULTI_MAX && !(b->plans[0]->synth && b->plans[0]->sweep_persist && reg_sweep_wanted(b->plans.data(), nplans)))
            throw Error(EMAGLS_ERR_UNSUPPORTED, "more than 16 designs per batch: only array designs that take the register-resident sweep (built-in SH basis, "
                                                "microphone grids set, at most 18 antipodal pairs + single microphones, a launch the device can hold)");
        for (auto* p : b->plans) {
            p->nstreams = 1;
            p->prof_level = 0;
            p->sync_stream = b->stream;
            p->owner = b.get();
        }
        b->atf = b->plans[0]->d.kind == EMAGLS_KIND_FROM_ATF;
        b->magls = magls_kind(b->plans[0]->d.kind) || b->plans[0]->d.kind == EMAGLS_KIND_LS;
        if (!b->atf && !b->magls) { batch_unify_synth(*b); batch_try_lanes(*b); }
        trace_mark("batch create: lanes tried");
        *batch = b.release();
    });
}
int emagls_batch_execute(emagls_batch* b) {
    return guarded([&] {
        DeviceGuard dg(b ? b->device : -1);
        if (!b) throw Error(EMAGLS_ERR_ARG, "null pointer");
        batch_execute(*b);
    });
}
int emagls_batch_synchronize(emagls_batch* b) {
    return guarded([&] {
        DeviceGuard dg(b ? b->device : -1);
        if (!b) throw Error(EMAGLS_ERR_ARG, "null pointer");
        HIP_CHECK(hipStreamSynchronize(b->stream));
    });
}
int emagls_batch_get_filters(emagls_batch* b, void* const* wL, void* const* wR) {
    return guarded([&] {
        DeviceGuard dg(b ? b->device : -1);
        if (!b || !wL || !wR) throw Error(EMAGLS_ERR_ARG, "null pointer");
        const size_t n = b->plans.size();
        for (size_t j = 0; j < n; ++j) {
            if (!wL[j] || !wR[j]) throw Error(EMAGLS_ERR_ARG, "null pointer");
            if (!b->plans[j]) throw Error(EMAGLS_ERR_ARG, "a plan of this batch has been destroyed");
            if (!b->plans[j]->executed) throw Error(EMAGLS_ERR_ARG, "batch has not been executed");
        }
        emagls_plan& p0 = *b->plans[0];
        const size_t bytes = (p0.out_cplx ? sizeof(cplx) : sizeof(double)) * (size_t)p0.out_rows * p0.out_cols;
        std::vector<int> flags(NFLAG * n, 0);
        for (int attempt = 0; attempt < 3; ++attempt) {
            if (b->lanes)
                HIP_CHECK(hipMemcpy2DAsync(flags.data(), NFLAG * sizeof(int), p0.get("flag"), b->stride, NFLAG * sizeof(int), n,
                                           hipMemcpyDeviceToHost, b->stream));
            else
                for (size_t j = 0; j < n; ++j)
                    HIP_CHECK(hipMemcpyAsync(&flags[NFLAG * j], b->plans[j]->get("flag"), NFLAG * sizeof(int), hipMemcpyDeviceToHost, b->stream));
            bool scattered = false;
            if (b->lanes && n <= 32 && bytes % 16 == 0) {
                bool dev_dst = true;
                for (size_t j = 0; j < n && dev_dst; ++j)
                    for (void* q : {wL[j], wR[j]}) {
                        hipPointerAttribute_t at{};
                        if (hipPointerGetAttributes(&at, q) != hipSuccess) { (void)hipGetLastError(); dev_dst = false; break; }
                        if (at.type != hipMemoryTypeDevice || at.device != b->device || ((uintptr_t)q & 15)) { dev_dst = false; break; }
                    }
                if (dev_dst) {
                    LanePtrs lp{};
                    for (size_t j = 0; j < n; ++j) { lp.p[2 * j] = wL[j]; lp.p[2 * j + 1] = wR[j]; }
                    launch_scatter_lanes(p0.get("wL"), p0.get("wR"), b->stride, bytes, (int)n, lp, b->stream);
                    scattered = true;
                }
            }
            if (!scattered)
                for (size_t j = 0; j < n; ++j) {
                    HIP_CHECK(hipMemcpyAsync(wL[j], b->plans[j]->get("wL"), bytes, hipMemcpyDefault, b->stream));
                    HIP_CHECK(hipMemcpyAsync(wR[j], b->plans[j]->get("wR"), bytes, hipMemcpyDefault, b->stream));
                }
            HIP_CHECK(hipStreamSynchronize(b->stream));
            bool redo = false;
            for (size_t j = 0; j < n; ++j) redo = plan_recover(*b->plans[j], &flags[NFLAG * j], false) || redo;
            if (!redo) break;
            batch_redo(*b, flags);
        }
        for (auto* q : b->plans)
            if (q->persist_suspended) { q->persist_suspended = false; q->sweep_persist = true; }
        for (size_t j = 0; j < n; ++j) throw_fatal_flags(&flags[NFLAG * j]);
        if (b->geo_cold_pending) { b->geo_kept_version = b->geo_ran_version; b->geo_cold_pending = false; }
    });
}
int emagls_batch_geometry_runs(emagls_batch* b, long long* cold, long long* warm) {
    return guarded([&] {
        if (!b || !cold || !warm) throw Error(EMAGLS_ERR_ARG, "null pointer");
        *cold = b->geo_cold_runs;
        *warm = b->geo_warm_runs;
    });
}
int emagls_batch_lane_mode(emagls_batch* b, int* lanes) {
    return guarded([&] {
        DeviceGuard dg(b ? b->device : -1);
        if (!b || !lanes) throw Error(EMAGLS_ERR_ARG, "null pointer");
        *lanes = b->lanes ? 1 : 0;
    });
}
int emagls_set_batch_max(int max_designs, int* previous) {
    return guarded([&] {
        if (max_designs < 1 || max_designs > REG_SWEEP_MAX) throw Error(EMAGLS_ERR_ARG, "a batch holds 1..32 designs (more than 16: array designs on the register-resident sweep)");
        const int prev = g_batch_max.exchange(max_designs);
        if (previous) *previous = prev;
    });
}
int emagls_batch_set_geometry_sharing(emagls_batch* b, int enable) {
    return guarded([&] {
        DeviceGuard dg(b ? b->device : -1);
        if (!b) throw Error(EMAGLS_ERR_ARG, "null pointer");
        HIP_CHECK(hipStreamSynchronize(b->stream));
        b->geo_want = enable != 0;
        b->geo_checked_version = ~0ull;
        batch_geo_forget(*b);
    });
}
int emagls_batch_shares_geometry(emagls_batch* b, int* shared) {
    return guarded([&] {
        if (!b || !shared) throw Error(EMAGLS_ERR_ARG, "null pointer");
        *shared = b->geo_share ? 1 : 0;
    });
}
int emagls_batch_shares_atf_side(emagls_batch* b, int* shared) {
    return guarded([&] {
        if (!b || !shared) throw Error(EMAGLS_ERR_ARG, "null pointer");
        *shared = b->atf_share ? 1 : 0;
    });
}
int emagls_batch_set_stream(emagls_batch* b, void* stream) {
    return guarded([&] {
        DeviceGuard dg(b ? b->device : -1);
        if (!b || !stream) throw Error(EMAGLS_ERR_ARG, "null pointer");
        HIP_CHECK(hipStreamSynchronize(b->stream));
        if (b->own_stream) emagls::pool_stream_give(b->stream);
        b->stream = (hipStream_t)stream;
        b->own_stream = false;
        for (auto* p : b->plans) if (p) p->sync_stream = b->stream;
    });
}
int emagls_batch_set_streams(emagls_batch* b, int nstreams) {
    return guarded([&] {
        DeviceGuard dg(b ? b->device : -1);
        if (!b) throw Error(EMAGLS_ERR_ARG, "null pointer");
        if (nstreams < 1 || nstreams > 4) throw Error(EMAGLS_ERR_ARG, "nstreams must be 1..4");
        HIP_CHECK(hipStreamSynchronize(b->stream));
        for (int i = 0; i < nstreams - 1; ++i) if (!b->side[i]) b->side[i] = emagls::pool_stream_take();
        if (nstreams != b->nstreams) drop_batch_graphs(*b);
        b->nstreams = nstreams;
    });
}
int emagls_batch_set_stage_order(emagls_batch* b, int order) {
    return guarded([&] {
        DeviceGuard dg(b ? b->device : -1);
        if (!b) throw Error(EMAGLS_ERR_ARG, "null pointer");
        if (order < 0 || order > 2) throw Error(EMAGLS_ERR_ARG, "stage order must be 0, 1 or 2");
        HIP_CHECK(hipStreamSynchronize(b->stream));
        if (order != b->order_hint) drop_batch_graphs(*b);
        b->order_hint = order;
    });
}
int emagls_batch_set_side_stream(emagls_batch* b, void* stream) {
    return guarded([&] {
        DeviceGuard dg(b ? b->device : -1);
        if (!b || !stream) throw Error(EMAGLS_ERR_ARG, "null pointer");
        HIP_CHECK(hipStreamSynchronize(b->stream));
        if (b->side[0] && !b->side0_external) { HIP_CHECK(hipStreamSynchronize(b->side[0])); emagls::pool_stream_give(b->side[0]); }
        b->side[0] = (hipStream_t)stream;
        b->side0_external = true;
    });
}
int emagls_batch_set_profiling(emagls_batch* b, int level) {
    return guarded([&] {
        DeviceGuard dg(b ? b->device : -1);
        if (!b) throw Error(EMAGLS_ERR_ARG, "null pointer");
        HIP_CHECK(hipStreamSynchronize(b->stream));
        if (level >= 1)
            for (auto& e : b->sweep_ev) if (!e) HIP_CHECK(hipEventCreate(&e));
        b->prof_level = level;
    });
}
int emagls_batch_sweep_time(emagls_batch* b, double* ms) {
    return guarded([&] {
        DeviceGuard dg(b ? b->device : -1);
        if (!b || !ms) throw Error(EMAGLS_ERR_ARG, "null pointer");
        if (b->prof_level < 1 || !b->sweep_ev[0]) throw Error(EMAGLS_ERR_ARG, "batch profiling is off");
        HIP_CHECK(hipStreamSynchronize(b->stream));
        float t = 0.f;
        HIP_CHECK(hipEventElapsedTime(&t, b->sweep_ev[0], b->sweep_ev[1]));
        *ms = t;
    });
}
int emagls_batch_destroy(emagls_batch* b) {
    return guarded([&] {
        DeviceGuard dg(b ? b->device : -1);
        delete b;
    });
}

int emagls_get_ls_filters(const double* hL, const double* hR, int64_t nsamp, int64_t ndirs, const double* azi,
                          const double* zen, int order, int basis, void* wL, void* wR) {
    emagls_design_desc d{};
    d.kind = EMAGLS_KIND_LS; d.basis = basis; d.order = order; d.nsamp = nsamp; d.ndirs = ndirs;
    return one_shot(d, hL, hR, azi, zen, nullptr, nullptr, nullptr, nullptr, nullptr, wL, wR, nullptr);
}
int emagls_get_magls_filters(const double* hL, const double* hR, int64_t nsamp, int64_t ndirs, const double* azi,
                             const double* zen, int order, double fs, int64_t len, int basis, void* wL, void* wR) {
    emagls_design_desc d{};
    d.kind = EMAGLS_KIND_MAGLS; d.basis = basis; d.order = order; d.fs = fs; d.len = len; d.nsamp = nsamp; d.ndirs = ndirs;
    return one_shot(d, hL, hR, azi, zen, nullptr, nullptr, nullptr, nullptr, nullptr, wL, wR, nullptr);
}
int emagls_get_emagls_filters(const double* hL, const double* hR, int64_t nsamp, int64_t ndirs, const double* azi,
                              const double* zen, double mic_radius, const double* mic_azi, const double* mic_zen,
                              int64_t nmics, int order, double fs, int64_t len, int basis, void* wL, void* wR) {
    emagls_design_desc d{};
    d.kind = EMAGLS_KIND_EMAGLS; d.basis = basis; d.order = order; d.fs = fs; d.len = len; d.nsamp = nsamp; d.ndirs = ndirs;
    d.mic_radius = mic_radius; d.nmics = nmics;
    if (!mic_azi || !mic_zen) { g_last_error = "null microphone grid"; return EMAGLS_ERR_ARG; }
    return one_shot(d, hL, hR, azi, zen, mic_azi, mic_zen, nullptr, nullptr, nullptr, wL, wR, nullptr);
}
int emagls_get_emagls2_filters(const double* hL, const double* hR, int64_t nsamp, int64_t ndirs, const double* azi,
                               const double* zen, double mic_radius, const double* mic_azi, const double* mic_zen,
                               int64_t nmics, int order, double fs, int64_t len, int basis, void* wL, void* wR) {
    emagls_design_desc d{};
    d.kind = EMAGLS_KIND_EMAGLS2; d.basis = basis; d.order = order; d.fs = fs; d.len = len; d.nsamp = nsamp; d.ndirs = ndirs;
    d.mic_radius = mic_radius; d.nmics = nmics;
    if (!mic_azi || !mic_zen) { g_last_error = "null microphone grid"; return EMAGLS_ERR_ARG; }
    return one_shot(d, hL, hR, azi, zen, mic_azi, mic_zen, nullptr, nullptr, nullptr, wL, wR, nullptr);
}
int emagls_get_emagls_filters_ema_in_ch(const double* hL, const double* hR, int64_t nsamp, int64_t ndirs, const double* azi,
                                        const double* zen, double mic_radius, const double* mic_azi, int64_t nmics, int order,
                                        double fs, int64_t len, int basis, void* wL, void* wR) {
    emagls_design_desc d{};
    d.kind = EMAGLS_KIND_EMA_CH; d.basis = basis; d.order = order; d.fs = fs; d.len = len; d.nsamp = nsamp; d.ndirs = ndirs;
    d.mic_radius = mic_radius; d.nmics = nmics;
    if (!mic_azi || nmics < 1) { g_last_error = "invalid array geometry"; return EMAGLS_ERR_ARG; }
    std::vector<double> mic_zen((size_t)nmics, kPi / 2.0);
    return one_shot(d, hL, hR, azi, zen, mic_azi, mic_zen.data(), nullptr, nullptr, nullptr, wL, wR, nullptr);
}
int emagls_get_emagls_filters_ema_in_sh(const double* hL, const double* hR, int64_t nsamp, int64_t ndirs, const double* azi,
                                        const double* zen, double mic_radius, const double* mic_azi, int64_t nmics, int order,
                                        double fs, int64_t len, int basis, void* wL, void* wR) {
    emagls_design_desc d{};
    d.kind = EMAGLS_KIND_EMA_SH; d.basis = basis; d.order = order; d.fs = fs; d.len = len; d.nsamp = nsamp; d.ndirs = ndirs;
    d.mic_radius = mic_radius; d.nmics = nmics;
    if (!mic_azi || nmics < 1) { g_last_error = "invalid array geometry"; return EMAGLS_ERR_ARG; }
    std::vector<double> mic_zen((size_t)nmics, kPi / 2.0);
    return one_shot(d, hL, hR, azi, zen, mic_azi, mic_zen.data(), nullptr, nullptr, nullptr, wL, wR, nullptr);
}
int emagls_get_emagls_filters_from_atf(const double* hL, const double* hR, int64_t nsamp, int64_t ndirs,
                                       const double* azi, const double* zen, const double* atf_irs, int64_t atf_taps,
                                       int64_t nmics, int64_t natf, const double* atf_azi, const double* atf_zen, double fs,
                                       int64_t filter_len, double f_trans, double* wL, double* wR, double* mean_dev) {
    emagls_design_desc d{};
    d.kind = EMAGLS_KIND_FROM_ATF; d.basis = EMAGLS_BASIS_REAL; d.fs = fs; d.len = filter_len; d.nsamp = nsamp; d.ndirs = ndirs;
    d.nmics = nmics; d.f_trans = f_trans; d.atf_taps = atf_taps; d.natf = natf;
    if (!atf_irs || !atf_azi || !atf_zen) { g_last_error = "null ATF set"; return EMAGLS_ERR_ARG; }
    return one_shot(d, hL, hR, azi, zen, nullptr, nullptr, atf_irs, atf_azi, atf_zen, wL, wR, mean_dev);
}

int emagls_get_magls_filters_dc(const double* hL, const double* hR, int64_t nsamp, int64_t ndirs, const double* azi, const double* zen,
                                int order, double fs, int64_t len, int apply_dc, int basis, void* wL, void* wR) {
    emagls_design_desc d{};
    d.kind = EMAGLS_KIND_MAGLS; d.basis = basis; d.order = order; d.fs = fs; d.len = len; d.nsamp = nsamp; d.ndirs = ndirs;
    d.diffuseness = apply_dc != 0;
    return one_shot(d, hL, hR, azi, zen, nullptr, nullptr, nullptr, nullptr, nullptr, wL, wR, nullptr);
}
static int emagls_array_dc(int kind, const double* hL, const double* hR, int64_t nsamp, int64_t ndirs, const double* azi, const double* zen,
                           double mic_radius, const double* mic_azi, const double* mic_zen, int64_t nmics, int order, double fs, int64_t len,
                           int apply_dc, int basis, void* wL, void* wR) {
    emagls_design_desc d{};
    d.kind = kind; d.basis = basis; d.order = order; d.fs = fs; d.len = len; d.nsamp = nsamp; d.ndirs = ndirs;
    d.mic_radius = mic_radius; d.nmics = nmics; d.diffuseness = apply_dc != 0;
    return one_shot(d, hL, hR, azi, zen, mic_azi, mic_zen, nullptr, nullptr, nullptr, wL, wR, nullptr);
}
int emagls_get_emagls_filters_dc(const double* hL, const double* hR, int64_t nsamp, int64_t ndirs, const double* azi, const double* zen,
                                 double mic_radius, const double* mic_azi, const double* mic_zen, int64_t nmics, int order, double fs,
                                 int64_t len, int apply_dc, int basis, void* wL, void* wR) {
    return emagls_array_dc(EMAGLS_KIND_EMAGLS, hL, hR, nsamp, ndirs, azi, zen, mic_radius, mic_azi, mic_zen, nmics, order, fs, len, apply_dc,
                           basis, wL, wR);
}
int emagls_get_emagls2_filters_dc(const double* hL, const double* hR, int64_t nsamp, int64_t ndirs, const double* azi, const double* zen,
                                  double mic_radius, const double* mic_azi, const double* mic_zen, int64_t nmics, int order, double fs,
                                  int64_t len, int apply_dc, int basis, void* wL, void* wR) {
    return emagls_array_dc(EMAGLS_KIND_EMAGLS2, hL, hR, nsamp, ndirs, azi, zen, mic_radius, mic_azi, mic_zen, nmics, order, fs, len, apply_dc,
                           basis, wL, wR);
}
int emagls_get_magls_filters_2d(const double* hL, const double* hR, int64_t nsamp, int64_t ndirs, const double* azi, int order, double fs,
                                int64_t len, int basis, void* wL, void* wR) {
    emagls_design_desc d{};
    d.kind = EMAGLS_KIND_MAGLS_2D; d.basis = basis; d.order = order; d.fs = fs; d.len = len; d.nsamp = nsamp; d.ndirs = ndirs;
    return one_shot(d, hL, hR, azi, nullptr, nullptr, nullptr, nullptr, nullptr, nullptr, wL, wR, nullptr);
}

int emagls_simulation_order(int kind, int order, double fs, double mic_radius) {
    switch (kind) {
        case EMAGLS_KIND_EMAGLS: case EMAGLS_KIND_EMA_CH: case EMAGLS_KIND_EMA_SH:
            return std::max(order, (int)std::ceil(fs * kPi * mic_radius / C_SOUND));
        case EMAGLS_KIND_EMAGLS2:
            return std::max(SMAIR_DEFAULT_ORDER, (int)std::ceil(fs * kPi * mic_radius / C_SOUND));
        default: return order;
    }
}
int emagls_design_out_shape(const emagls_design_desc* desc, int64_t* rows, int64_t* cols, int* is_complex) {
    return guarded([&] {
        if (!desc || !rows || !cols || !is_complex) throw Error(EMAGLS_ERR_ARG, "invalid argument");
        const emagls_design_desc& d = *desc;
        if (d.kind < EMAGLS_KIND_LS || d.kind > EMAGLS_KIND_EMA_SH || d.order < 0) throw Error(EMAGLS_ERR_ARG, "invalid design kind or order");
        switch (d.kind) {
            case EMAGLS_KIND_EMAGLS2: case EMAGLS_KIND_FROM_ATF: *cols = d.nmics; break;
            case EMAGLS_KIND_MAGLS_2D: case EMAGLS_KIND_EMA_CH: *cols = 2 * (int64_t)d.order + 1; break;
            default: *cols = ((int64_t)d.order + 1) * (d.order + 1);
        }
        *rows = d.kind == EMAGLS_KIND_LS ? d.nsamp : d.len;
        *is_complex = d.basis == EMAGLS_BASIS_COMPLEX && d.kind != EMAGLS_KIND_FROM_ATF;
    });
}
int emagls_get_ls_filters_with_basis(const double* hL, const double* hR, int64_t nsamp, int64_t ndirs, const void* Y_hrir, int order,
                                     int basis, void* wL, void* wR) {
    emagls_design_desc d{};
    d.kind = EMAGLS_KIND_LS; d.basis = basis; d.order = order; d.nsamp = nsamp; d.ndirs = ndirs; d.custom_basis = 1;
    return one_shot(d, hL, hR, nullptr, nullptr, nullptr, nullptr, nullptr, nullptr, nullptr, wL, wR, nullptr, Y_hrir, nullptr);
}
int emagls_get_magls_filters_with_basis(const double* hL, const double* hR, int64_t nsamp, int64_t ndirs, const void* Y_hrir, int order,
                                        double fs, int64_t len, int basis, void* wL, void* wR) {
    emagls_design_desc d{};
    d.kind = EMAGLS_KIND_MAGLS; d.basis = basis; d.order = order; d.fs = fs; d.len = len; d.nsamp = nsamp; d.ndirs = ndirs; d.custom_basis = 1;
    return one_shot(d, hL, hR, nullptr, nullptr, nullptr, nullptr, nullptr, nullptr, nullptr, wL, wR, nullptr, Y_hrir, nullptr);
}
int emagls_get_emagls_filters_with_basis(const double* hL, const double* hR, int64_t nsamp, int64_t ndirs, const void* Y_hrir,
                                         double mic_radius, const void* Y_mic, int64_t nmics, int order, double fs, int64_t len, int basis,
                                         void* wL, void* wR) {
    emagls_design_desc d{};
    d.kind = EMAGLS_KIND_EMAGLS; d.basis = basis; d.order = order; d.fs = fs; d.len = len; d.nsamp = nsamp; d.ndirs = ndirs;
    d.mic_radius = mic_radius; d.nmics = nmics; d.custom_basis = 1;
    if (!Y_mic) { g_last_error = "null microphone SH matrix"; return EMAGLS_ERR_ARG; }
    return one_shot(d, hL, hR, nullptr, nullptr, nullptr, nullptr, nullptr, nullptr, nullptr, wL, wR, nullptr, Y_hrir, Y_mic);
}
int emagls_get_emagls2_filters_with_basis(const double* hL, const double* hR, int64_t nsamp, int64_t ndirs, const void* Y_hrir,
                                          double mic_radius, const void* Y_mic, int64_t nmics, int order, double fs, int64_t len, int basis,
                                          void* wL, void* wR) {
    emagls_design_desc d{};
    d.kind = EMAGLS_KIND_EMAGLS2; d.basis = basis; d.order = order; d.fs = fs; d.len = len; d.nsamp = nsamp; d.ndirs = ndirs;
    d.mic_radius = mic_radius; d.nmics = nmics; d.custom_basis = 1;
    if (!Y_mic) { g_last_error = "null microphone SH matrix"; return EMAGLS_ERR_ARG; }
    return one_shot(d, hL, hR, nullptr, nullptr, nullptr, nullptr, nullptr, nullptr, nullptr, wL, wR, nullptr, Y_hrir, Y_mic);
}

}
```

emagls_amd/csrc/kernels.hpp:

```cpp
#pragma once
#include <algorithm>
#include <functional>

#include "common.hpp"

namespace emagls {

void launch_zero(void* p, size_t bytes, hipStream_t st);
void launch_compare_words(const void* a, const void* b, size_t bytes, int* differ, hipStream_t st);
void launch_broadcast_lanes(const void* src, size_t bytes, size_t stride, int nlanes, hipStream_t st);
struct LanePtrs { void* p[64]; };
void launch_scatter_lanes(const void* srcL, const void* srcR, size_t stride, size_t bytes, int n, const LanePtrs& dst, hipStream_t st);
void launch_gather_buffers(const LanePtrs& src, const LanePtrs& dst, int nbuf, size_t bytes, hipStream_t st);
struct BufferMoves { const void* src[96]; void* dst[96]; size_t bytes[96]; int n; };
void launch_move_buffers(const BufferMoves& m, hipStream_t st);
void launch_ch_basis(int N, int M, const double* azi, bool cplx_basis, void* out, int ld, hipStream_t st, bool out_real = false);
void launch_sh_coeff(int N, double* tab, hipStream_t st);
inline size_t esz(bool c) { return c ? sizeof(cplx) : sizeof(double); }
inline size_t sh_coeff_count(int N) { return (size_t)2 * (N + 1) * (N + 1) + 2 * (N + 1); }
void launch_sh_basis(int N, int64_t D, const double* azi, const double* zen, const double* tab, bool cplx_basis,
                     void* Y, int64_t ld, hipStream_t st);
void launch_transpose_conj(const void* Y, int64_t D, int64_t S, int64_t ldY, void* Yt, int64_t Dpad, int64_t ldYt,
                           bool is_cplx, bool conj_it, hipStream_t st);

void launch_modal_bn(int N, int64_t nfreq, const double* kr, double kr_scale, double out_scale, void* bn,
                     int64_t stride_k, int64_t stride_n, hipStream_t st, const int* n_valid = nullptr);

void launch_twiddles(int nfft, void* tw, hipStream_t st);
int hrir_dirsum_chunks(int64_t D);
void launch_hrir_grpdelay(const double* hL, const double* hR, int64_t L, int64_t D, int nfft, const void* tw,
                          double* partial, double* grpd, hipStream_t st);
void launch_hrir_fft(const double* hL, const double* hR, int64_t L, int64_t D, const int64_t* didx, int nfft,
                     const void* tw, const double* grpd, int mode, int n_c, int kabs0, void* Hc, double* Habs,
                     int64_t ldD, hipStream_t st, double* HcT = nullptr, int ldT = 0);
void launch_real_fft_gather(const double* x, int64_t L, int64_t ncols, const int64_t* colidx, int nfft, const void* tw,
                            void* out, int64_t ldo, int64_t inner, int64_t ld_inner, hipStream_t st);
void launch_filter_epilogue(const void* W, int C, int nfft, int len, const void* tw, const double* grpd, int conj_mode,
                            int dc_rule, int shift_mode, int out_cplx, void* outL, void* outR, hipStream_t st, int n_ears = 2,
                            double fade_rel = 0.15);

int gram_ksplit(int64_t D, int S);
int64_t gram_dpad(int64_t D, int S);
void launch_gram(const void* Yc, int64_t D, int S, int64_t ld, bool is_cplx, void* Gp, void* G, void* R, int Sh, hipStream_t st);
void launch_cholesky(void* G, int S, bool is_cplx, int* flag, hipStream_t st);
void launch_qform(const void* Yc, const void* R, void* Rinv, int S, int64_t D, int64_t ld, bool is_cplx, void* Q, hipStream_t st);
void launch_zsolve_flagged(void* Z, int ldS, const void* R, const void* Rinv, const double* cond_ok, int S, int C, int P, int k0,
                           hipStream_t st);
void launch_tn(const void* R, const void* E, int S, int C, int ldE, int nOrders, bool is_cplx, void* Tn, int64_t ldS,
               hipStream_t st);
void launch_small_gemm(const void* A, int lda, bool a_cplx, const void* B, int ldb, bool b_cplx, void* Cm, int ldc,
                       bool c_cplx, int M, int N, int K, hipStream_t st);

void launch_magls_m(const void* R, int C, bool is_cplx, int P, void* Mw, double* cond_ok, int* status, hipStream_t st);

struct FactorArgs;
void launch_factor(const FactorArgs& a, int nbins, bool tn_cplx, hipStream_t st, int phases = 3);
void launch_factor_jacobi_gram(const FactorArgs& a, int nbins, hipStream_t st);
void launch_factor_jacobi_pair(const FactorArgs& gram, int nb_gram, const FactorArgs& hh, int nb_hh, hipStream_t st);

void launch_gram_kmat(const void* Gy, const void* E, int S, int ldE, int C, int nOrd, bool is_cplx, void* F, int64_t ldF, double* Kmat, int ldK,
                      hipStream_t st);
void launch_gram_gemm(const void* bn, int nOrd, int P, int kb0, int nbins, double* Cf, int ldC, const double* Kmat, int ldK, int C, double* Apk,
                      int ldA, hipStream_t st);
void launch_gram_solve(const double* Apk, int ldA, int C, int kb0, int nbins, double reg_c, void* Mw, void* R2w, double* sv, int* route,
                       int* sweeps_out, hipStream_t st);
size_t hy_mfma_workspace_doubles(int n_c, int S, bool y_cplx);
int hy_mfma_kpad(int D);
void launch_hy_conj_mfma(const double* HcT, int ldT, int n_c, const void* Yc, int64_t ldY, bool y_cplx, int D, int S, double* Pw, void* out,
                         int ldS, hipStream_t st);
void launch_ls_gram(const void* Hc, int64_t ldH, int n_c, const void* G, int64_t g_stride, int64_t ldD, const void* Mw, int D, int C, int P,
                    int kb_lo, int kb_hi, void* W, hipStream_t st);

struct DenseSweepArgs;
struct HalfSweepArgs;
struct HalfSweepMulti;
void launch_sweep_dense(const DenseSweepArgs& a, int kb, bool x_cplx, hipStream_t st);
int dense_sweep_nwg(int D, int C);
void launch_sweep_half(const HalfSweepMulti& m, int kb, hipStream_t st);
void launch_sweep_half_finalize(const HalfSweepMulti& m, int kb_last, hipStream_t st);
int persist_sweep_nwg(int D);
bool persist_sweep_supported(int D, int C);
size_t persist_sweep_ll_bytes(int D, int C);
void launch_sweep_persist(const HalfSweepMulti& m, hipStream_t st);
int persist_sweep_dpw(int D);
int sweep_cu_budget();
bool persist_sweep_fits(int D, int C, int ndesigns);
bool synth_sweep_fits(int D, int nmics, int nOrd, int ndesigns);
bool synth_sweep_supported(int D, int nmics, int nOrd);
int synth_nord_pad(int nOrd);
void launch_synth_prepare(const void* bn, int nOrd, int P, void* bsc, const void* Zlo, int ldZ, int nOut, int M, const int* smap, double* Pm, hipStream_t st);
void launch_synth_mt(const void* Mw, const double* Pm, int nOut, int M, int k0, int P, const void* W, void* Mt, void* Winit, hipStream_t st);
void launch_synth_winit(const void* W, const void* Pm, int nOut, int M, int k0, int P, void* Winit, hipStream_t st, bool shared_geometry);
void launch_synth_rows(const void* U, int nchunks, const void* Pm, const void* Mw, int nOut, int M, int k_lo, int k_hi, int P, void* W, hipStream_t st,
                       bool shared_geometry = false);
int synth_ls_chunks(int D);
void launch_synth_ls(const void* Hc, int64_t ldH, int n_c, const void* bsc, int nord_pad, const double* dir_azi, const double* dir_zen, const double* mic_azi,
                     const double* mic_zen, const int* smap, int D, int M, int P, int kb_lo, int kb_hi, void* Upart, hipStream_t st, bool shared_geometry = false);
void launch_sweep_synth(const HalfSweepMulti& m, hipStream_t st);
void synth_cosines_debug(const double* dir_azi, const double* dir_zen, int64_t ndirs, const double* mic_azi, const double* mic_zen, int nmics, double* x2);
void synth_operand_debug(const void* bsc, int nbins, int nord_pad, const double* x, int64_t nx, int gs, void* g_plus, void* g_minus);
int reg_sweep_max_units();
bool reg_sweep_supported(int D, int nmics, int nunits, int nOrd);
size_t reg_sweep_ll_bytes(int D, int nmics);
int reg_sweep_capacity(int D);
int reg_sweep_slots_per_xcd();
int reg_sweep_pick_waves(int D, int ndesigns);
int reg_sweep_gate_cost(int D, int ndesigns);
bool reg_sweep_fits(int D, int nmics, int nunits, int nOrd, int ndesigns);
void launch_sweep_reg(const HalfSweepArgs* args_dev, const HalfSweepArgs& a0, int n, hipStream_t st);
double reg_contract_selftest();
double gram_tile_selftest(bool four);
void store_sweep_args(const HalfSweepArgs* host, int n, HalfSweepArgs* dev, hipStream_t st);
void launch_sweep_finalize(const void* Wpart, void* W, int nWG, int C, int P, int kb_last, hipStream_t st);
void launch_hy_conj(const void* Hc, int64_t ldD, int nrows, const void* Yc, int64_t ldY, bool y_cplx, int D, int S, void* Pw, void* out,
                    int ldS, hipStream_t st);
size_t hy_workspace_elems(int nrows, int ldS);
void launch_ypinv(const void* Q, int64_t ldQ, bool q_cplx, const void* Zb, int ldS, int D, int S, int C, void* Ypinv,
                  int64_t ldD, hipStream_t st);
void launch_ls_apply(const void* Hc, int64_t ldH, int n_c, const void* Zf, bool z_cplx, int64_t ldD, int D, int C, int P,
                     int kb_lo, int kb_hi, void* W, hipStream_t st);
void launch_ls_filters(const double* hL, const double* hR, int64_t L, int D, const void* Yp, bool cplx_basis, int64_t ldD,
                       int C, void* wL, void* wR, hipStream_t st);
void launch_conj_copy(const void* in, void* out, int64_t n, bool is_cplx, hipStream_t st);
void launch_sh_rows_to_complex(void* W, int C, int nrows, int order, hipStream_t st);
void launch_widen(const void* in, int64_t ldi, bool in_cplx, void* out, int64_t ldo, int rows, int cols, bool transpose,
                  bool upper_only, hipStream_t st);

void launch_gram_inverse(const void* R, int S, bool is_cplx, void* M, int* status, hipStream_t st, void* work = nullptr);
void launch_ypinv_gram(const void* Ycm, int64_t ldD, bool is_cplx, const void* M, int S, int D, void* Ypinv, hipStream_t st);
void launch_sweep_wide(const DenseSweepArgs& a, int kb, bool x_cplx, hipStream_t st);
void launch_sweep_wide_finalize(const void* Wpart, void* W, int nWG, int C, int P, int kb_last, hipStream_t st);

void launch_wa_assemble(const void* Tn, const void* bn, int nOrd, int S, int C, int ldS, int P, int kb0, int nbins, void* B, hipStream_t st);
void launch_wa_factor(void* B, void* Vw, int S, int C, int ldS, int nbins, double reg_c, double* tauw, void* R2w, void* Nw, double* sv, int* sweeps,
                      void* Z, hipStream_t st);
struct WaTiling { int leaves, leaf_h, ldT; size_t off_stack, off_vt, off_zt, off_tau, bytes; };
WaTiling wa_tiling(int S, int C, int nbins);
void launch_wa_factor_tiled(void* B, void* Vw, int S, int C, int ldS, int nbins, double reg_c, double* tauw, void* R2w, void* Nw, double* sv,
                            int* sweeps, void* Z, void* ws, hipStream_t st);
void launch_wa_yri(const void* Q, int64_t ldQ, const void* Z, int S, int C, int ldS, int D, int64_t ldD, int nbins, void* Yri, hipStream_t st);
void launch_wa_ls(const void* Hc, int64_t ldH, int n_c, const void* Yri, int64_t ldD, int D, int C, int P, int kb_first, int kb_end, void* W, hipStream_t st);
void launch_wa_lo_gram(const void* Ycm, int M, int nOut, double* Ag, hipStream_t st);
void launch_wa_e(const void* Ycm, int M, int nOut, int S, const void* Minv, void* E, int ldE, hipStream_t st);

void launch_qt(const void* Yc, int64_t ldY, const void* E, int ldE, int D, int S, int C, int nOrders, bool is_cplx, void* QT,
               int64_t ldD, hipStream_t st);
void launch_dspace_g(const void* QT, int64_t ldD, bool is_cplx, const void* bn, int nOrders, int D, int C, int P, int k0, void* G,
                     hipStream_t st, int real_mode = 0, int sh_order = -1, int k_end = -1);
void launch_cond_flags(const double* sv, int C, int P, int hh_end, double* cond_ok, hipStream_t st);
void launch_yri_accurate(const void* Q, int64_t ldQ, bool is_cplx, const void* Z, int ldS, const double* cond_ok, int D, int S,
                         int C, int P, int k0, void* Yri, int64_t ldD, hipStream_t st, const void* Ycm = nullptr, int64_t ldYcm = 0);

void launch_grid_match(const double* aziA, const double* zenA, int64_t nA, const double* aziB, const double* zenB,
                       int64_t nB, double* cartB, int64_t* idx, double* dev_deg, double* mean_dev, hipStream_t st);
void launch_atf_colidx(const int64_t* idx, int64_t nA, int M, int64_t* colidx, hipStream_t st);

double measure_fp64_peak(int which, int reps, bool burst = false, double* mhz = nullptr);

void binaural_decode_real(const double* sig, int64_t n, int C, const double* wL, const double* wR, int64_t len,
                          double* out , hipStream_t st,
                          const cplx* sigc = nullptr );
bool decode_wave_form(int64_t len);
void binaural_decode_complex(const void* sig, bool sig_cplx, int64_t n, int C, const void* wL, const void* wR, bool w_cplx, int64_t len,
                             double* sig2, double* w2L, double* w2R, double* out, double* imag_abs, double* d_tmp, hipStream_t st,
                             int64_t imag_skip = 0 );
void decode_cache_clear();
void launch_abs_sum_cols(const double* x, int64_t n, int64_t skip, int ncols, double* out, hipStream_t st);

int rotate_order(int layout, int64_t C);
void launch_rotate_yaw(const void* in, bool in_cplx, int64_t n, int C, int layout, bool cplx_basis, const double* yaw, bool per_sample,
                       bool transpose, void* out, hipStream_t st, int64_t ld_in = 0, int64_t ld_out = 0, int L = 1, int64_t la = 0,
                       int64_t lo = 0);
int rotate3_max_order();
void launch_rotate3(const void* in, bool in_cplx, int64_t n, int C, bool cplx_basis, const double* yaw, bool yaw_ps, const double* pitch,
                    bool pitch_ps, const double* roll, bool roll_ps, bool transpose, void* out, hipStream_t st, int64_t ld_in = 0,
                    int64_t ld_out = 0, int L = 1, const int64_t* la = nullptr, int64_t lo = 0);
void launch_rotate3_matrix(int N, bool cplx_basis, double yaw, double pitch, double roll, void* out, hipStream_t st);
void rotate3_cache_clear();
struct EncodeBlock { const double* enc; bool enc_cplx; int M; const double* x; int64_t ldx; };
void launch_rotate_yaw_encoded(const EncodeBlock& e, int64_t n, int C, int layout, bool cplx_basis, const double* yaw, bool per_sample, void* out,
                               hipStream_t st, int64_t ld_out = 0, int L = 1, int64_t la = 0, int64_t lo = 0);
void launch_rotate3_encoded(const EncodeBlock& e, int64_t n, int C, bool cplx_basis, const double* yaw, bool yaw_ps, const double* pitch, bool pitch_ps,
                            const double* roll, bool roll_ps, void* out, hipStream_t st, int64_t ld_out = 0, int L = 1, const int64_t* la = nullptr,
                            int64_t lo = 0);
void launch_encode_block(const EncodeBlock& e, int64_t n, int C, void* out, int64_t ld_out, hipStream_t st);
constexpr int64_t kResampleMaxRatio = 65536;
int64_t resample_length(int64_t n, int64_t p, int64_t q);
void launch_resample(const void* in, bool cplx_in, int64_t n, int64_t nch, int64_t p, int64_t q, void* out, hipStream_t st);
void resample_cache_clear();

struct DecodeStreamState {
    int C = 0;
    bool planes2 = false;
    int B = 0, P = 0;
    int S = 1;
    int L = 1;
    cplx* Wf = nullptr;
    cplx* ring = nullptr;
    void* hist = nullptr;
    int* pos = nullptr;
};
bool decode_stream_block_ok(int64_t B);
void launch_decode_stream_filters(const double* wpl, int Cp, int64_t len, int B, int P, int64_t S, cplx* Wf, hipStream_t st);
void launch_decode_stream_block(const DecodeStreamState& s, const void* x, bool x_cplx, int64_t ldx, const int* set, int standing, double* out,
                                int64_t ldo, hipStream_t st, int64_t lsx = 0, int lset = 0, int64_t lso = 0);

void decode_family_cache_clear();

void filter_channels_by_order(const double* sig, int64_t n_in, int64_t n, int C, const double* ir , int nOrd, int64_t len,
                              int64_t skip, double* out , hipStream_t st);

void launch_ema_sh_e0(const void* Ech, int ldS, const void* Ypts, int C, int S, bool cb, void* E0, hipStream_t st);
void launch_rot_points(const double* azi, const double* zen, int D, int npts, double* azr, double* znr, hipStream_t st);
void launch_rot_from_points(const void* A, int64_t ldA, const void* Z, int ldP, int C, int npts, const double* zen, int D, bool cb, void* Rot,
                            hipStream_t st);
void launch_qt_rotate(void* QT, int64_t ldD, int nOrd, int C, int N, int D, const void* Rot, bool cb, hipStream_t st);
void launch_gram_from_g(const void* G, int64_t g_stride, int64_t ldD, int D, int C, int kb0, int nbins, int g0, double* Apk, int ldK,
                        hipStream_t st);

void launch_radial_filter(const void* bn, int nOrd, int P, int type, double regul, double g, bool nyq_abs, bool zero_nan,
                          void* out_kn, void* out_cm, hipStream_t st);
void launch_diffuse_field(const void* bn, int nOrd, int n_lo, int P, double* df_hi, double* df_lo, hipStream_t st);
void launch_array_diffuse(const void* bn, int nOrd, const void* Y, bool y_cplx, int ldY, int S, int M, int nOut, int P,
                          double* df_lo, hipStream_t st);
void launch_eq_spectrum(const double* df_hi, const double* df_lo, const double* df_arr, int P, int mode, void* W, double* W_full,
                        hipStream_t st);
void launch_diffuse_constraint(void* W, const void* G, bool g_cplx, int64_t g_stride, int g0, const void* H, int D, int C, int64_t ldD,
                               int P, hipStream_t st);
void launch_smair(const void* E, bool e_cplx, int ldS, const void* bn, int nOrd, const void* rad, int nRad, int rows, int S, int P, void* out,
                  hipStream_t st);
void launch_sh_encode(const double* sig, int64_t n, int M, const void* Z, int ldZ, int nOut, bool out_cplx, void* out, hipStream_t st);

int rh_num_metrics();
int rh_bins_padded(int P);
int rh_gemm_tiles(int64_t D);
int rh_atf_tiles(int64_t D);
void launch_rh_split(const void* in, int64_t ncols, int64_t len, double* out, hipStream_t st);
void launch_rh_join(const void* F, int64_t n, void* W, hipStream_t st);
void launch_rh_modes(const void* W, int C, int P, int nsets, const void* A, bool a_cplx, int ldA, const void* bn, int nOrd, int S, bool y_cplx,
                     double* Tt, int64_t ldR, hipStream_t st);
void launch_rh_order_rows(const void* W, int C, int P, int nsets, const void* bn, int nOrd, bool q_cplx, double* Tt, int64_t ldR, hipStream_t st);
void launch_rh_interleave(const void* Y, int64_t ldi, int S, int64_t D, double* Yk, int64_t ldo, hipStream_t st);
struct RhOut {
    const void* H = nullptr;
    int64_t hset_stride = 0;
    const double* w = nullptr;
    void* Hhat = nullptr;
    double* partial = nullptr;
};
void launch_rh_gemm(const double* Tt, int64_t ldR, const double* Yk, int64_t ldY, int K, int P, int64_t D, int nsets, const RhOut& o,
                    hipStream_t st);
void launch_rh_atf(const void* W, const void* A, int M, int P, int64_t D, int nsets, const RhOut& o, hipStream_t st);
void launch_rh_reduce(const double* partial, int64_t nrows, int ntile, double* out, hipStream_t st);

hipStream_t pool_stream_take();
void pool_stream_give(hipStream_t st);
int guarded_call(const std::function<void()>& f);

}

#include "args.hpp"
```

emagls_amd/csrc/sweep_reg.hip:

```cpp
#include "kernels.hpp"
#include "persist_common.hpp"
#include "synth_common.hpp"

#include <algorithm>
#include <map>
#include <mutex>

namespace emagls {

namespace {

constexpr int RG_MLD = 36;

constexpr int DPP_ROR4 = 0x124, DPP_ROR8 = 0x128;
__device__ __forceinline__ int rg_slot_set(int i, int x) { return i < 4 ? 0 : i < 8 ? 1 : x >> 1; }
__device__ __forceinline__ int rg_slot_unit(int i, int x) { return i < 8 ? 4 * (i & 3) + x : 16 + (x & 1); }

template <int NUL>
__device__ __forceinline__ void rg_contract(const cplx (&E)[NUL], const cplx (&O)[NUL], const cplx (&ts)[2], int lane, bool slot8, double* wp) {
    static_assert(NUL == 9, "quad layout of 18 units");
    const int x = lane & 3;
    double ar[2], ai[2];
#pragma unroll
    for (int s = 0; s < 2; ++s) { ar[s] = (x & 1) ? ts[s].y : ts[s].x; ai[s] = (x & 1) ? -ts[s].x : ts[s].y; }
    double aE[5], aO[5];
#pragma unroll
    for (int r = 0; r < 5; ++r) { aE[r] = 0.0; aO[r] = 0.0; }
#pragma unroll
    for (int s = 0; s < 2; ++s)
#pragma unroll
        for (int c = 0; c < 2; ++c) {
            const double a = c ? ai[s] : ar[s];
#pragma unroll
            for (int r = 0; r < 4; ++r) {
                aE[r] = __builtin_amdgcn_mfma_f64_4x4x4f64(a, c ? E[4 * s + r].y : E[4 * s + r].x, aE[r], 0, 0, 0);
                aO[r] = __builtin_amdgcn_mfma_f64_4x4x4f64(a, c ? O[4 * s + r].y : O[4 * s + r].x, aO[r], 0, 0, 0);
            }
        }
    if (slot8) {
#pragma unroll
        for (int s = 0; s < 2; ++s) {
            const bool mine = (x >> 1) == s;
#pragma unroll
            for (int c = 0; c < 2; ++c) {
                const double a = c ? ai[s] : ar[s];
                aE[4] = __builtin_amdgcn_mfma_f64_4x4x4f64(a, mine ? (c ? E[8].y : E[8].x) : 0.0, aE[4], 0, 0, 0);
                aO[4] = __builtin_amdgcn_mfma_f64_4x4x4f64(a, mine ? (c ? O[8].y : O[8].x) : 0.0, aO[4], 0, 0, 0);
            }
        }
    }
    const int nacc = slot8 ? 5 : 4;
#pragma unroll
    for (int r = 0; r < 5; ++r) {
        if (r >= nacc) break;
        aE[r] += dpp_d<DPP_ROR4>(aE[r]); aE[r] += dpp_d<DPP_ROR8>(aE[r]);
        aO[r] += dpp_d<DPP_ROR4>(aO[r]); aO[r] += dpp_d<DPP_ROR8>(aO[r]);
    }
    if (slot8) { aE[4] += dpp_d<DPP_XOR2>(aE[4]); aO[4] += dpp_d<DPP_XOR2>(aO[4]); }
    if ((lane & 12) == 0) {
        const int y = lane >> 4;
#pragma unroll
        for (int r = 0; r < 4; ++r) { wp[8 * (4 * r + x) + y] = aE[r]; wp[8 * (4 * r + x) + 4 + y] = aO[r]; }
        if (slot8 && x < 2) { wp[8 * (16 + x) + y] = aE[4]; wp[8 * (16 + x) + 4 + y] = aO[4]; }
    }
}

template <int U0, int GS, int NUL, int NT>
__device__ __forceinline__ void synth_units(const double* xcol, cplx (&E)[NUL], cplx (&O)[NUL], const cplx* bs, int nord_pad) {
    double x2[GS], pa[GS], pb[GS];
#pragma unroll
    for (int i = 0; i < GS; ++i) x2[i] = xcol[(U0 + i) * NT];
#pragma unroll
    for (int i = 0; i < GS; ++i) { pa[i] = 1.0; pb[i] = 0.5 * x2[i]; E[U0 + i] = mk(0.0, 0.0); O[U0 + i] = mk(0.0, 0.0); }
    const unsigned bs0 = lds_addr(bs);
    d2_t b0, b1, c0, c1;
    auto request = [&](int n, d2_t& q0, d2_t& q1) __attribute__((always_inline)) {
        const int nn = n < nord_pad ? n : nord_pad - 2;
        lds_read16_async(q0, bs0 + 16 * nn, pa[0]); lds_read16_async(q1, bs0 + 16 * nn + 16, pa[0]);
    };
    auto pass = [&](const d2_t& q0, const d2_t& q1) __attribute__((always_inline)) {
#pragma unroll
        for (int i = 0; i < GS; ++i) {
            E[U0 + i].x = fma(q0.x, pa[i], E[U0 + i].x); E[U0 + i].y = fma(q0.y, pa[i], E[U0 + i].y);
            O[U0 + i].x = fma(q1.x, pb[i], O[U0 + i].x); O[U0 + i].y = fma(q1.y, pb[i], O[U0 + i].y);
            pa[i] = fma(x2[i], pb[i], -pa[i]);
            pb[i] = fma(x2[i], pa[i], -pb[i]);
        }
    };
    request(0, b0, b1);
    lds_wait2(b0, b1, pa[0]);
    for (int n = 0; n < nord_pad; n += 4) {
        request(n + 2, c0, c1);
        pass(b0, b1);
        lds_wait2(c0, c1, pb[GS - 1]);
        if (n + 2 >= nord_pad) break;
        request(n + 4, b0, b1);
        pass(c0, c1);
        lds_wait2(b0, b1, pb[GS - 1]);
    }
}

__device__ __forceinline__ int launder(int v) { asm volatile("" : "+v"(v)); return v; }

#define RG_GLOBAL(T, p) ((T __attribute__((address_space(1)))*)(p))
typedef const double __attribute__((address_space(1)))* gcd_t;
typedef const cplx __attribute__((address_space(1)))* gcc_t;
typedef u64 __attribute__((address_space(1)))* gu64_t;
typedef unsigned u32x4_t __attribute__((ext_vector_type(4)));
__device__ __forceinline__ cplx ldg(gcc_t p) { return mk(p->x, p->y); }
__device__ __forceinline__ u64 gll_load(gu64_t p) { return __hip_atomic_load(p, __ATOMIC_RELAXED, __HIP_MEMORY_SCOPE_AGENT); }
__device__ __forceinline__ void gll_put(gu64_t dst, u64 word, bool local) {
    if (local) __hip_atomic_store(dst, word, __ATOMIC_RELAXED, __HIP_MEMORY_SCOPE_WORKGROUP);
    else __hip_atomic_store(dst, word, __ATOMIC_RELAXED, __HIP_MEMORY_SCOPE_AGENT);
}
__device__ __forceinline__ void gll_load16_async(u32x4_t& out, gu64_t p) { asm volatile("global_load_dwordx4 %0, %1, off sc1" : "=v"(out) : "v"(p) : "memory"); }

constexpr int RG_POLL = 12;
__device__ __forceinline__ void rg_wait_loads(u32x4_t (&g)[RG_POLL]) {
    asm volatile("s_waitcnt vmcnt(0)" : "+v"(g[0]), "+v"(g[1]), "+v"(g[2]), "+v"(g[3]), "+v"(g[4]), "+v"(g[5]), "+v"(g[6]), "+v"(g[7]), "+v"(g[8]), "+v"(g[9]),
                 "+v"(g[10]), "+v"(g[11]) :: "memory");
}
constexpr int RG_NUL = 9;
constexpr int RG_NEX = 4 * PS_CMAX;
constexpr int RG_SVC = 256;

template <int NUL, int NW>
__global__ void __launch_bounds__(64 * NW) __attribute__((amdgpu_waves_per_eu(3))) sweep_reg_kernel(const HalfSweepArgs* __restrict__ args, int n, int nWG, int spread, int prio) {
    constexpr int NT = 64 * NW, DPW = 32 * NW;
    constexpr int NU2 = 2 * NUL;
    constexpr int NVW = 8 * NU2;
    constexpr int GA = (NUL + 1) / 2, GB = NUL - GA;
    static_assert(GB >= 1 && NW % 2 == 0 && NT >= RG_SVC, "layout");
    extern __shared__ __attribute__((aligned(16))) char dyn[];
    cplx* ring = reinterpret_cast<cplx*>(dyn);
    cplx* ms = ring + 2 * SY_NORD;
    cplx* WE = ms + PS_CMAX * RG_MLD;
    cplx* WO = WE + 2 * NU2;
    double* vt = reinterpret_cast<double*>(WO + 2 * NU2);
    double* wpart = vt + 2 * RG_NEX;
    double* xs = wpart + NW * NVW;
    __shared__ int s_abort, s_local;

    int design, member;
    if (spread) {
        design = (int)blockIdx.x / nWG;
        member = (int)blockIdx.x - design * nWG;
    } else {
        const int xcd = blockIdx.x & 7, rest = blockIdx.x >> 3;
        const int sub = rest / nWG;
        member = rest - sub * nWG;
        design = xcd + 8 * sub;
    }
    if (design >= n) return;
    if (prio) __builtin_amdgcn_s_setprio(3);
    const HalfSweepArgs& a = args[design];
    const int tid = threadIdx.x;
    const int C = a.C, P = a.P, D = a.D, kfirst = a.kfirst, kabs0 = a.kabs0;
    const int64_t ldH = a.ldH;
    const int nord_pad = a.nord_pad;
    const gcd_t Habs = RG_GLOBAL(const double, a.Habs);
    const gcc_t Mw = RG_GLOBAL(const cplx, a.Mw);
    const gcc_t bsc = RG_GLOBAL(const cplx, a.bsc);
    const gcd_t Winit = RG_GLOBAL(const double, a.Winit);
    cplx __attribute__((address_space(1)))* const Uout = RG_GLOBAL(cplx, a.U);
    long long* const timing = a.timing;
    int* const abort_flag = a.abort_flag;
    const long long wait_ticks = a.wait_ticks;
    const int* smap = a.smap;
    const int npr = smap[32], nsg = smap[33], nun = npr + nsg;
    const gu64_t part_ll = RG_GLOBAL(u64, a.ll);
    const gu64_t xcc_ll = part_ll + (size_t)2 * nWG * RG_NEX * 2;
    if (tid == 0) { s_abort = 0; s_local = 0; }
    const int d0 = member * DPW;
    auto dir_of = [&](int t, int s) __attribute__((always_inline)) { return d0 + 32 * (t >> 6) + 16 * s + ((t & 63) >> 2); };

    {
        const size_t ncplx = (size_t)2 * SY_NORD + PS_CMAX * RG_MLD + 4 * NU2;
        for (size_t i = tid; i < ncplx; i += NT) ring[i] = mk(0, 0);
        for (int i = tid; i < 2 * RG_NEX + NW * NVW; i += NT) vt[i] = 0.0;
        double sd[2], cd[2], daz[2];
#pragma unroll
        for (int s = 0; s < 2; ++s) {
            const int dgi = dir_of(tid, s) < D ? dir_of(tid, s) : D - 1;
            synth_zen(a.dir_zen[dgi], sd[s], cd[s]);
            daz[s] = a.dir_azi[dgi];
        }
#pragma unroll 1
        for (int i = 0; i < NUL; ++i) {
            const int u = rg_slot_unit(i, tid & 3), s = rg_slot_set(i, tid & 3);
            double v = 0.0;
            if (u < nun) {
                const int jm = smap[u < npr ? 2 * u : 2 * npr + (u - npr)];
                double sm, cm;
                synth_zen(a.mic_zen ? a.mic_zen[jm] : 1.5707963267948966, sm, cm);
                v = synth_x2(s ? sd[1] : sd[0], s ? cd[1] : cd[0], sm, cm, (s ? daz[1] : daz[0]) - a.mic_azi[jm]);
            }
            xs[i * NT + tid] = v;
        }
    }
    __syncthreads();

    if (tid < nord_pad) {
        ring[(kfirst & 1) * SY_NORD + tid] = ldg(bsc + (int64_t)kfirst * nord_pad + tid);
        const int k1 = kfirst + 1 < P ? kfirst + 1 : P - 1;
        ring[((kfirst + 1) & 1) * SY_NORD + tid] = ldg(bsc + (int64_t)k1 * nord_pad + tid);
    }
    constexpr int NLM = 4;
    cplx mReg[NLM];
    auto fetch_m = [&](int kbm, int t) __attribute__((always_inline)) {
        const int r = t >> 3, c0 = (t & 7) * 4;
        const gcc_t M = Mw + (int64_t)kbm * C * C + r * C + c0;
#pragma unroll
        for (int i = 0; i < NLM; ++i) mReg[i] = ldg(M + i);
    };
    auto stage_m = [&](int t) __attribute__((always_inline)) {
        const int r = t >> 3, c0 = (t & 7) * 4;
#pragma unroll
        for (int i = 0; i < NLM; ++i) ms[r * RG_MLD + c0 + i] = (r < C && c0 + i < C) ? mReg[i] : mk(0, 0);
    };
    double hCur[2], hNext[2] = {0.0, 0.0};
    auto fetch_h = [&](int kb, double (&h)[2], int t) __attribute__((always_inline)) {
        const int kbg = (kb < P ? kb : P - 1) - kabs0;
        const gcd_t He = Habs + ((int64_t)((t >> 1) & 1) * (P - kabs0) + kbg) * ldH;
#pragma unroll
        for (int s = 0; s < 2; ++s) h[s] = He[dir_of(t, s) < D ? dir_of(t, s) : D - 1];
    };
    fetch_h(kfirst, hCur, tid);
    if (tid < RG_SVC) { fetch_m(kfirst, tid); stage_m(tid); }

    if (tid < 64) {
        const int lane = tid;
        const unsigned xcc = read_xcc_id();
        const unsigned tag0 = 0x58434300u;
        if (lane == 0) gll_put(xcc_ll + member, ((u64)tag0 << 32) | xcc, false);
        bool alive = true, same = true;
        for (int base = 0; base < nWG && alive; base += 64) {
            u64 w = 0;
            alive = ll_wait([&] {
                if (base + lane >= nWG) return true;
                w = gll_load(xcc_ll + base + lane);
                return ll_ok(w, tag0);
            }, abort_flag, wait_ticks);
            same = same && __builtin_amdgcn_ballot_w64(base + lane < nWG && (unsigned)w != xcc) == 0;
        }
        if (lane == 0) {
            s_local = alive && same && a.force_global == 0;
            if (!alive) s_abort = 1;
            if (timing && member == 1) timing[15] = s_local;
        }
    }
    __syncthreads();
    const bool local = s_local != 0;
    if (s_abort) return;

    const bool slot8 = nun > 16 || GB < 2;
    cplx E[NUL], O[NUL];
#pragma unroll
    for (int u = 0; u < NUL; ++u) { E[u] = mk(0, 0); O[u] = mk(0, 0); }

#define RSTAMP(i) do { if (timing && member == 1 && tid == 0 && kb < P) timing[(int64_t)kb * 16 + (i)] = (long long)wall_clock64(); } while (0)
    for (int kb = kfirst; kb <= P; ++kb) {
        const bool first = (kb == kfirst);
        const bool last = (kb == P);
        const bool nyq = (kb == P - 1);
        RSTAMP(7);
        if (!last) {
            const cplx* bs = ring + (kb & 1) * SY_NORD;
            const double* xcol = xs + launder(tid);
            synth_units<0, GA, NUL, NT>(xcol, E, O, bs, nord_pad);
            __builtin_amdgcn_sched_barrier(0);
            if (slot8) synth_units<GA, GB, NUL, NT>(xcol, E, O, bs, nord_pad);
            else synth_units<GA, GB - 1, NUL, NT>(xcol, E, O, bs, nord_pad);
            __builtin_amdgcn_sched_barrier(0);
        }
        RSTAMP(0);
        if (launder(tid) < RG_SVC) {
            const int t = launder(tid);
            const int j = t & (RG_NEX - 1), half = t >> 7;
            if (first) {
                vt[t] = half == 0 ? Winit[j] : 0.0;
            } else {
                const unsigned tag = (unsigned)(kb - 1);
                const gu64_t src = part_ll + ((size_t)((kb - 1) & 1) * nWG * RG_NEX + j) * 2;
                double sum = 0.0;
                const bool alive = ll_wait([&] {
                    bool ok = true;
                    double s = 0.0;
                    for (int base = half; base < nWG; base += 2 * RG_POLL) {
                        u32x4_t g[RG_POLL];
#pragma unroll
                        for (int i = 0; i < RG_POLL; ++i) {
                            const int w = base + 2 * i < nWG ? base + 2 * i : half;
                            gll_load16_async(g[i], src + (size_t)w * RG_NEX * 2);
                        }
                        rg_wait_loads(g);
#pragma unroll
                        for (int i = 0; i < RG_POLL; ++i) {
                            ok = ok && g[i].y == tag && g[i].w == tag;
                            if (base + 2 * i < nWG) s += __hiloint2double((int)g[i].z, (int)g[i].x);
                        }
                    }
                    sum = s;
                    return ok;
                }, abort_flag, wait_ticks);
                vt[t] = sum;
                if (!alive && (t & 63) == 0) s_abort = 1;
            }
        }
        RSTAMP(2);
        __syncthreads();
        if (s_abort) break;
        if (launder(tid) < RG_SVC) {
            const int t = launder(tid);
            const int part = t & 3, pair = t >> 2, e = pair >> 5, c = pair & 31;
            const cplx* vc = reinterpret_cast<const cplx*>(vt) + e * PS_CMAX;
            cplx acc = mk(0, 0);
            if (first) {
                if (part == 0) acc = vc[c];
            } else {
#pragma unroll
                for (int i = 0; i < PS_CMAX / 4; ++i)
                    cfma(acc, vc[part + 4 * i] + vc[RG_NEX / 2 + part + 4 * i], conj(ms[(part + 4 * i) * RG_MLD + c]));
            }
            acc = group_sum<4>(acc);
            const cplx other = shfl_xor_c(acc, 4);
            if (part == 0 && c < C) {
                if (c < 2 * npr) {
                    if ((c & 1) == 0) { WE[e * NU2 + (c >> 1)] = acc + other; WO[e * NU2 + (c >> 1)] = acc - other; }
                } else {
                    WE[e * NU2 + npr + (c - 2 * npr)] = acc; WO[e * NU2 + npr + (c - 2 * npr)] = acc;
                }
                if (member == 0 && !first) {
                    cplx __attribute__((address_space(1)))* dst = Uout + ((int64_t)e * P + (kb - 1)) * PS_CMAX + c;
                    const cplx v = vc[c] + vc[RG_NEX / 2 + c];
                    dst->x = v.x; dst->y = v.y;
                }
            }
        }
        if (last) break;
        __syncthreads();
        RSTAMP(3);
        const bool svc = launder(tid) < RG_SVC;
        if (svc) fetch_m(kb, launder(tid));
        cplx ts[2];
        {
            const int t = launder(tid);
            const int x = t & 3;
            cplx p[2][2];
#pragma unroll
            for (int s = 0; s < 2; ++s) { p[s][0] = mk(0, 0); p[s][1] = mk(0, 0); }
#pragma unroll
            for (int r = 0; r < 4; ++r) {
                const int u = 4 * r + x;
                const cplx we0 = WE[u], wo0 = WO[u], we1 = WE[NU2 + u], wo1 = WO[NU2 + u];
#pragma unroll
                for (int s = 0; s < 2; ++s) {
                    cfma(p[s][0], we0, E[4 * s + r]); cfma(p[s][0], wo0, O[4 * s + r]);
                    cfma(p[s][1], we1, E[4 * s + r]); cfma(p[s][1], wo1, O[4 * s + r]);
                }
            }
            if (slot8) {
                const int u = 16 + (x & 1);
                cplx q0 = mk(0, 0), q1 = mk(0, 0);
                cfma(q0, WE[u], E[8]); cfma(q0, WO[u], O[8]);
                cfma(q1, WE[NU2 + u], E[8]); cfma(q1, WO[NU2 + u], O[8]);
                const bool s1 = (x & 2) != 0;
                const cplx z = mk(0, 0);
                p[0][0] = p[0][0] + (s1 ? z : q0); p[0][1] = p[0][1] + (s1 ? z : q1);
                p[1][0] = p[1][0] + (s1 ? q0 : z); p[1][1] = p[1][1] + (s1 ? q1 : z);
            }
            if (svc) stage_m(t);
            RSTAMP(8);
#pragma unroll
            for (int s = 0; s < 2; ++s) {
                const cplx pe0 = group_sum<4>(p[s][0]), pe1 = group_sum<4>(p[s][1]);
                const cplx pe = (x & 2) ? pe1 : pe0;
                ts[s] = dir_of(t, s) < D ? unit_phase(hCur[s], pe, nyq) : mk(0, 0);
            }
        }
        __builtin_amdgcn_sched_barrier(0);
        {
            const int t = launder(tid);
            rg_contract<NUL>(E, O, ts, t & 63, slot8, wpart + (t >> 6) * NVW);
        }
        {
            const int t = launder(tid);
            fetch_h(kb + 1, hNext, t);
            if (t < nord_pad) ring[(kb & 1) * SY_NORD + t] = ldg(bsc + (int64_t)(kb + 2 < P ? kb + 2 : P - 1) * nord_pad + t);
        }
        __syncthreads();
        RSTAMP(4);
        if (launder(tid) < RG_NEX) {
            const int t = launder(tid);
            const int xe = t >> 6, xr = (t >> 1) & 31, xri = t & 1;
            double v = 0.0;
            if (xr < C) {
                const int xu = xr < 2 * npr ? (xr >> 1) : npr + (xr - 2 * npr);
                const bool xneg = xr < 2 * npr && (xr & 1);
                const double* wE = wpart + 8 * xu + 2 * xe + xri;
                double sE = 0.0, sO = 0.0;
#pragma unroll
                for (int w = 0; w < NW; ++w) { sE += wE[w * NVW]; sO += wE[w * NVW + 4]; }
                v = xneg ? sE - sO : sE + sO;
            }
            const gu64_t dst = part_ll + (((size_t)(kb & 1) * nWG + member) * RG_NEX + t) * 2;
            const u64 bits = (u64)__double_as_longlong(v), tg = (u64)(unsigned)kb << 32;
            gll_put(dst, tg | (bits & 0xffffffffull), local);
            gll_put(dst + 1, tg | (bits >> 32), local);
        }
        RSTAMP(5);
        hCur[0] = hNext[0]; hCur[1] = hNext[1];
    }
#undef RSTAMP
}

__global__ void __launch_bounds__(64) reg_contract_selftest_kernel(const cplx* __restrict__ t, const cplx* __restrict__ g, double* __restrict__ out) {
    const int lane = threadIdx.x, x = lane & 3;
    cplx E[RG_NUL], O[RG_NUL], ts[2];
#pragma unroll
    for (int i = 0; i < RG_NUL; ++i) {
        const int d = 16 * rg_slot_set(i, x) + (lane >> 2), u = rg_slot_unit(i, x);
        E[i] = ldc(g + (d * 18 + u) * 2);
        O[i] = ldc(g + (d * 18 + u) * 2 + 1);
    }
#pragma unroll
    for (int s = 0; s < 2; ++s) ts[s] = ldc(t + (16 * s + (lane >> 2)) * 2 + (x >> 1));
    rg_contract<RG_NUL>(E, O, ts, lane, true, out);
}

__global__ void __launch_bounds__(64) store_args_kernel(HalfSweepMulti m, HalfSweepArgs* dst) {
    const int nw = (int)(sizeof(HalfSweepArgs) / 8);
    for (int j = 0; j < m.n; ++j) {
        const unsigned long long* src = reinterpret_cast<const unsigned long long*>(&m.a[j]);
        unsigned long long* d = reinterpret_cast<unsigned long long*>(dst + j);
        for (int i = threadIdx.x; i < nw; i += 64) d[i] = src[i];
    }
}
static_assert(sizeof(HalfSweepArgs) % 8 == 0, "argument block in whole words");

size_t reg_dyn_bytes(int nul, int nw) {
    const size_t nu2 = 2 * (size_t)nul, nvw = 8 * nu2;
    return sizeof(cplx) * ((size_t)2 * SY_NORD + PS_CMAX * RG_MLD + 4 * nu2) +
           sizeof(double) * (2 * RG_NEX + (size_t)nw * nvw + (size_t)nul * 64 * nw);
}
constexpr int RG_WAVES[] = {4, 6, 8, 10, 12};
const void* reg_kernel_ptr(int nw) {
    switch (nw) {
        case 4: return reinterpret_cast<const void*>(sweep_reg_kernel<RG_NUL, 4>);
        case 6: return reinterpret_cast<const void*>(sweep_reg_kernel<RG_NUL, 6>);
        case 8: return reinterpret_cast<const void*>(sweep_reg_kernel<RG_NUL, 8>);
        case 10: return reinterpret_cast<const void*>(sweep_reg_kernel<RG_NUL, 10>);
        default: return reinterpret_cast<const void*>(sweep_reg_kernel<RG_NUL, 12>);
    }
}
void reg_set_attributes() {
    static PerDeviceOnce attr_once;
    if (attr_once.first())
        for (int nw : RG_WAVES) HIP_CHECK(hipFuncSetAttribute(reg_kernel_ptr(nw), hipFuncAttributeMaxDynamicSharedMemorySize, 150 * 1024));
}
int reg_nwg(int D, int nw) { return (int)ceil_div(D, 32 * nw); }
int reg_occupancy(int nw) {
    static std::mutex mu;
    static std::map<std::pair<int, int>, int> cache;
    int dev = 0;
    HIP_CHECK(hipGetDevice(&dev));
    std::lock_guard<std::mutex> lk(mu);
    auto it = cache.find({dev, nw});
    if (it != cache.end()) return it->second;
    reg_set_attributes();
    int nb = 0;
    if (hipOccupancyMaxActiveBlocksPerMultiprocessor(&nb, reg_kernel_ptr(nw), 64 * nw, reg_dyn_bytes(RG_NUL, nw)) != hipSuccess) { (void)hipGetLastError(); nb = 0; }
    cache[{dev, nw}] = nb;
    return nb;
}
int reg_wg_cost(int nw) { return nw == 4 ? 1 : 3; }

}

int reg_sweep_max_units() { return 2 * RG_NUL; }
bool reg_sweep_supported(int D, int nmics, int nunits, int nOrd) {
    return nmics >= 2 && nmics <= PS_CMAX && nunits >= 1 && nunits <= 2 * RG_NUL && D >= 1 && reg_nwg(D, 12) <= 32 && nOrd <= SY_NORD;
}
size_t reg_sweep_ll_bytes(int D, int nmics) {
    const size_t nwg = (size_t)reg_nwg(D, 4);
    (void)nmics;
    return sizeof(u64) * ((size_t)2 * nwg * RG_NEX * 2 + nwg + 64);
}
int reg_sweep_slots_per_xcd() { return 3 * (sweep_cu_budget() / 8); }
int reg_sweep_pick_waves(int D, int ndesigns) {
    if (ndesigns < 1 || ndesigns > REG_SWEEP_MAX) return 0;
    const int nsub = (int)ceil_div(ndesigns, 8), cus = sweep_cu_budget() / 8;
    if (const char* e = getenv("EMAGLS_REG_WAVES")) {
        const int nw = atoi(e);
        if ((nw == 4 || nw == 6 || nw == 8 || nw == 10 || nw == 12) && nsub * reg_nwg(D, nw) * reg_wg_cost(nw) <= 3 * cus && reg_occupancy(nw) >= (nw == 4 ? 3 : 1)) return nw;
    }
    for (int nw : RG_WAVES) if (nsub * reg_nwg(D, nw) <= cus && reg_occupancy(nw) >= 1) return nw;
    return (nsub * reg_nwg(D, 4) <= 3 * cus && reg_occupancy(4) >= 3) ? 4 : 0;
}
int reg_sweep_spread_waves(int D, int ndesigns) {
    const char* es = getenv("EMAGLS_REG_SPREAD");
    const int mode = es ? atoi(es) : 2;
    if (mode == 0 || ndesigns < 1 || ndesigns > REG_SWEEP_MAX || getenv("EMAGLS_REG_WAVES")) return 0;
    const int cus = sweep_cu_budget(), local = reg_sweep_pick_waves(D, ndesigns);
    for (int nw : RG_WAVES)
        if (ndesigns * reg_nwg(D, nw) <= cus && reg_occupancy(nw) >= 1) return (mode == 1 || local == 0 || nw < local) ? nw : 0;
    return 0;
}
int reg_sweep_gate_cost(int D, int ndesigns) {
    if (const int ns = reg_sweep_spread_waves(D, ndesigns)) return (int)ceil_div((int64_t)ndesigns * reg_nwg(D, ns), 8) * reg_wg_cost(ns);
    const int nw = reg_sweep_pick_waves(D, ndesigns);
    return nw ? (int)ceil_div(ndesigns, 8) * reg_nwg(D, nw) * reg_wg_cost(nw) : 0;
}
int reg_sweep_capacity(int D) {
    int n = 0;
    for (int k = 8; k <= REG_SWEEP_MAX; k += 8) if (reg_sweep_pick_waves(D, k)) n = k;
    return n;
}
bool reg_sweep_fits(int D, int nmics, int nunits, int nOrd, int ndesigns) {
    return reg_sweep_supported(D, nmics, nunits, nOrd) && reg_sweep_pick_waves(D, ndesigns) != 0;
}

void launch_sweep_reg(const HalfSweepArgs* args_dev, const HalfSweepArgs& a0, int n, hipStream_t st) {
    const int ns = reg_sweep_spread_waves(a0.D, n);
    const int nw = ns ? ns : reg_sweep_pick_waves(a0.D, n);
    if (!nw) throw Error(2, "register-resident sweep: the launch cannot be resident");
    const int nWG = reg_nwg(a0.D, nw), spread = ns ? 1 : 0;
    const unsigned nblocks = spread ? (unsigned)(n * nWG) : 8u * (unsigned)nWG * (unsigned)ceil_div(n, 8);
    const size_t dyn = reg_dyn_bytes(RG_NUL, nw);
    reg_set_attributes();
    static const int prio = [] { const char* e = getenv("EMAGLS_REG_PRIO"); return e ? atoi(e) : 1; }();
    switch (nw) {
        case 4: sweep_reg_kernel<RG_NUL, 4><<<dim3(nblocks), 256, dyn, st>>>(args_dev, n, nWG, spread, prio); break;
        case 6: sweep_reg_kernel<RG_NUL, 6><<<dim3(nblocks), 384, dyn, st>>>(args_dev, n, nWG, spread, prio); break;
        case 8: sweep_reg_kernel<RG_NUL, 8><<<dim3(nblocks), 512, dyn, st>>>(args_dev, n, nWG, spread, prio); break;
        case 10: sweep_reg_kernel<RG_NUL, 10><<<dim3(nblocks), 640, dyn, st>>>(args_dev, n, nWG, spread, prio); break;
        default: sweep_reg_kernel<RG_NUL, 12><<<dim3(nblocks), 768, dyn, st>>>(args_dev, n, nWG, spread, prio); break;
    }
    KERNEL_CHECK();
}

double reg_contract_selftest() {
    constexpr int ND = 32, NU = 2 * RG_NUL, NO = 8 * NU;
    cplx h_t[ND * 2], h_g[ND * NU * 2];
    double h_out[NO], want[NO] = {0};
    unsigned long long x = 88172645463325252ull;
    auto rnd = [&] { x ^= x << 13; x ^= x >> 7; x ^= x << 17; return (double)(x % 2000001ull) / 1000000.0 - 1.0; };
    for (cplx& v : h_t) { v.x = rnd(); v.y = rnd(); }
    for (cplx& v : h_g) { v.x = rnd(); v.y = rnd(); }
    for (int d = 0; d < ND; ++d)
        for (int u = 0; u < NU; ++u)
            for (int eo = 0; eo < 2; ++eo)
                for (int e = 0; e < 2; ++e) {
                    const cplx tv = h_t[d * 2 + e], gv = h_g[(d * NU + u) * 2 + eo];
                    want[8 * u + 4 * eo + 2 * e] += tv.x * gv.x + tv.y * gv.y;
                    want[8 * u + 4 * eo + 2 * e + 1] += tv.y * gv.x - tv.x * gv.y;
                }
    cplx *d_t = nullptr, *d_g = nullptr;
    double* d_out = nullptr;
    HIP_CHECK(hipMalloc(&d_t, sizeof h_t));
    HIP_CHECK(hipMalloc(&d_g, sizeof h_g));
    HIP_CHECK(hipMalloc(&d_out, sizeof h_out));
    HIP_CHECK(hipMemcpy(d_t, h_t, sizeof h_t, hipMemcpyHostToDevice));
    HIP_CHECK(hipMemcpy(d_g, h_g, sizeof h_g, hipMemcpyHostToDevice));
    HIP_CHECK(hipMemset(d_out, 0, sizeof h_out));
    reg_contract_selftest_kernel<<<1, 64>>>(d_t, d_g, d_out);
    KERNEL_CHECK();
    HIP_CHECK(hipMemcpy(h_out, d_out, sizeof h_out, hipMemcpyDeviceToHost));
    HIP_CHECK(hipFree(d_t));
    HIP_CHECK(hipFree(d_g));
    HIP_CHECK(hipFree(d_out));
    double err = 0.0;
    for (int i = 0; i < NO; ++i) err = std::max(err, std::fabs(h_out[i] - want[i]));
    return err;
}

void store_sweep_args(const HalfSweepArgs* host, int n, HalfSweepArgs* dev, hipStream_t st) {
    for (int first = 0; first < n; first += SWEEP_MULTI_MAX) {
        HalfSweepMulti m{};
        m.n = std::min(SWEEP_MULTI_MAX, n - first);
        for (int j = 0; j < m.n; ++j) m.a[j] = host[first + j];
        store_args_kernel<<<1, 64, 0, st>>>(m, dev + first);
        KERNEL_CHECK();
    }
}

}
```

include/emagls.h:

```cpp
#ifndef EMAGLS_H
#define EMAGLS_H

#include <stddef.h>
#include <stdint.h>

#ifdef __cplusplus
extern "C" {
#endif

#define EMAGLS_OK 0
#define EMAGLS_ERR_ARG 1
#define EMAGLS_ERR_UNSUPPORTED 2
#define EMAGLS_ERR_HIP 3
#define EMAGLS_ERR_NUMERIC 4

#define EMAGLS_BASIS_REAL 0
#define EMAGLS_BASIS_COMPLEX 1

#define EMAGLS_KIND_LS 0
#define EMAGLS_KIND_MAGLS 1
#define EMAGLS_KIND_EMAGLS 2
#define EMAGLS_KIND_EMAGLS2 3
#define EMAGLS_KIND_FROM_ATF 4
#define EMAGLS_KIND_EMA_CH 5
#define EMAGLS_KIND_MAGLS_2D 6
#define EMAGLS_KIND_EMA_SH 7

const char* emagls_last_error(void);
int emagls_version(void);
int emagls_device_count(int* count);
int emagls_set_device(int device);

int emagls_cache_clear(void);
int emagls_cache_release_designs(void);

int emagls_fp64_peak_tflops(int which, double* tflops);
int emagls_fp64_peak_tflops_ex(int which, int burst, double* tflops, double* shader_mhz);
int emagls_self_test(int which, double* max_err);
int emagls_debug_synth_operand(const void* bsc, int nbins, int nord_pad, const double* x, int64_t nx, int gs, void* g_plus, void* g_minus);
int emagls_debug_synth_cosines(const double* dir_azi, const double* dir_zen, int64_t ndirs, const double* mic_azi, const double* mic_zen, int nmics, double* x2);


int emagls_sh_basis(int order, int64_t ndirs, const double* azi, const double* zen, int basis, void* Y);

int emagls_sh_basis_device(int order, int64_t ndirs, const double* d_azi, const double* d_zen, int basis, void* d_Y,
                           void* stream);

int emagls_modal_bn(int order, int64_t nfreq, const double* kr, void* bn);


int emagls_get_ls_filters(const double* hL, const double* hR, int64_t nsamp, int64_t ndirs,
                          const double* hrir_azi, const double* hrir_zen, int order, int basis,
                          void* wL, void* wR );

int emagls_get_magls_filters(const double* hL, const double* hR, int64_t nsamp, int64_t ndirs,
                             const double* hrir_azi, const double* hrir_zen, int order, double fs, int64_t len,
                             int basis, void* wL, void* wR );

int emagls_get_emagls_filters(const double* hL, const double* hR, int64_t nsamp, int64_t ndirs,
                              const double* hrir_azi, const double* hrir_zen, double mic_radius,
                              const double* mic_azi, const double* mic_zen, int64_t nmics, int order, double fs,
                              int64_t len, int basis, void* wL, void* wR );

int emagls_get_emagls2_filters(const double* hL, const double* hR, int64_t nsamp, int64_t ndirs,
                               const double* hrir_azi, const double* hrir_zen, double mic_radius,
                               const double* mic_azi, const double* mic_zen, int64_t nmics, int order, double fs,
                               int64_t len, int basis, void* wL, void* wR );

int emagls_get_emagls_filters_ema_in_ch(const double* hL, const double* hR, int64_t nsamp, int64_t ndirs,
                                        const double* hrir_azi, const double* hrir_zen, double mic_radius,
                                        const double* mic_azi, int64_t nmics, int order, double fs, int64_t len, int basis,
                                        void* wL, void* wR);

int emagls_simulation_order(int kind, int order, double fs, double mic_radius);
int emagls_get_ls_filters_with_basis(const double* hL, const double* hR, int64_t nsamp, int64_t ndirs, const void* Y_hrir, int order,
                                     int basis, void* wL, void* wR);
int emagls_get_magls_filters_with_basis(const double* hL, const double* hR, int64_t nsamp, int64_t ndirs, const void* Y_hrir, int order,
                                        double fs, int64_t len, int basis, void* wL, void* wR);
int emagls_get_emagls_filters_with_basis(const double* hL, const double* hR, int64_t nsamp, int64_t ndirs, const void* Y_hrir,
                                         double mic_radius, const void* Y_mic, int64_t nmics, int order, double fs, int64_t len,
                                         int basis, void* wL, void* wR);
int emagls_get_emagls2_filters_with_basis(const double* hL, const double* hR, int64_t nsamp, int64_t ndirs, const void* Y_hrir,
                                          double mic_radius, const void* Y_mic, int64_t nmics, int order, double fs, int64_t len,
                                          int basis, void* wL, void* wR);

int emagls_get_emagls_filters_ema_in_sh(const double* hL, const double* hR, int64_t nsamp, int64_t ndirs, const double* azi,
                                        const double* zen, double mic_radius, const double* mic_azi, int64_t nmics, int order,
                                        double fs, int64_t len, int basis, void* wL, void* wR);

int emagls_get_emagls_filters_from_atf(const double* hL, const double* hR, int64_t nsamp, int64_t ndirs,
                                       const double* hrir_azi, const double* hrir_zen, const double* atf_irs,
                                       int64_t atf_taps, int64_t nmics, int64_t natf, const double* atf_azi,
                                       const double* atf_zen, double fs, int64_t filter_len, double f_trans,
                                       double* wL, double* wR, double* mean_grid_dev_deg);

int emagls_binaural_decode(const double* in, int64_t nsamp, int64_t nch, const double* wL, const double* wR,
                           int64_t len, int compensate_delay, double* out);

int emagls_binaural_decode_complex(const void* in, int in_is_complex, int64_t nsamp, int64_t nch, const void* wL, const void* wR,
                                   int filters_are_complex, int64_t len, int compensate_delay, double* out, double* imag_abs_sum);

int emagls_binaural_decode_device(const void* d_in, int in_is_complex, int64_t nsamp, int64_t nch, const void* d_wL, const void* d_wR,
                                  int filters_are_complex, int64_t len, double* d_out, double* imag_abs_sum, void* stream);

#define EMAGLS_LAYOUT_SH 0
#define EMAGLS_LAYOUT_CH 1

int emagls_rotate_yaw(const void* in, int in_is_complex, int64_t nsamp, int64_t nch, int layout, int basis, const double* yaw,
                      int64_t n_yaw, void* out);

int emagls_binaural_decode_render(const void* in, int in_is_complex, int64_t nsamp, int64_t nch, const void* wL, const void* wR,
                                  int filters_are_complex, int64_t len, int compensate_delay, int layout, int basis, const double* yaw,
                                  int64_t n_yaw, const double* signal, int64_t n_signal, double* out, double* imag_abs_sum);

int emagls_binaural_decode_render_device(const void* d_in, int in_is_complex, int64_t nsamp, int64_t nch, const void* d_wL,
                                         const void* d_wR, int filters_are_complex, int64_t len, int layout, int basis,
                                         const double* d_yaw, int64_t n_yaw, const double* d_signal, int64_t n_signal, double* d_out,
                                         double* imag_abs_sum, void* stream);

int emagls_sh_rotation_matrix(int order, int basis, double yaw, double pitch, double roll, void* out);

int emagls_rotate_sh(const void* in, int in_is_complex, int64_t nsamp, int64_t nch, int basis, const double* yaw, int64_t n_yaw,
                     const double* pitch, int64_t n_pitch, const double* roll, int64_t n_roll, void* out);

int emagls_binaural_decode_render_ypr(const void* in, int in_is_complex, int64_t nsamp, int64_t nch, const void* wL, const void* wR,
                                      int filters_are_complex, int64_t len, int compensate_delay, int layout, int basis, const double* yaw,
                                      int64_t n_yaw, const double* pitch, int64_t n_pitch, const double* roll, int64_t n_roll,
                                      const double* signal, int64_t n_signal, double* out, double* imag_abs_sum);

int emagls_binaural_decode_render_ypr_device(const void* d_in, int in_is_complex, int64_t nsamp, int64_t nch, const void* d_wL,
                                             const void* d_wR, int filters_are_complex, int64_t len, int layout, int basis, const double* d_yaw,
                                             int64_t n_yaw, const double* d_pitch, int64_t n_pitch, const double* d_roll, int64_t n_roll,
                                             const double* d_signal, int64_t n_signal, double* d_out, double* imag_abs_sum, void* stream);

int64_t emagls_resample_length(int64_t nsamp, int64_t p, int64_t q);

int emagls_resample(const void* in, int in_is_complex, int64_t nsamp, int64_t nch, int64_t p, int64_t q, void* out);

int emagls_resample_device(const void* d_in, int in_is_complex, int64_t nsamp, int64_t nch, int64_t p, int64_t q, void* d_out,
                           void* stream);

int emagls_binaural_decode_render_fs(const void* in, int in_is_complex, int64_t nsamp, int64_t nch, const void* wL, const void* wR,
                                     int filters_are_complex, int64_t len, int compensate_delay, int layout, int basis, const double* yaw,
                                     int64_t n_yaw, const double* pitch, int64_t n_pitch, const double* roll, int64_t n_roll,
                                     const double* signal, int64_t n_signal, double in_fs, double filter_fs, double signal_fs, double* out,
                                     double* imag_abs_sum);

int emagls_binaural_decode_render_fs_device(const void* d_in, int in_is_complex, int64_t nsamp, int64_t nch, const void* d_wL,
                                            const void* d_wR, int filters_are_complex, int64_t len, int layout, int basis, const double* d_yaw,
                                            int64_t n_yaw, const double* d_pitch, int64_t n_pitch, const double* d_roll, int64_t n_roll,
                                            const double* d_signal, int64_t n_signal, double in_fs, double filter_fs, double signal_fs,
                                            double* d_out, double* imag_abs_sum, void* stream);

typedef struct emagls_decode_stream emagls_decode_stream;
int emagls_decode_stream_create(int64_t nch, const void* wL, const void* wR, int filters_are_complex, int64_t len, int in_is_complex,
                                int layout, int basis, int64_t block, emagls_decode_stream** s);

int emagls_decode_stream_push(emagls_decode_stream* s, const void* in, int64_t nsamp, const double* yaw, int64_t n_yaw,
                              const double* pitch, int64_t n_pitch, const double* roll, int64_t n_roll, double* out);

int emagls_decode_stream_push_device(emagls_decode_stream* s, const void* d_in, int64_t nsamp, const double* d_yaw, int64_t n_yaw,
                                     const double* d_pitch, int64_t n_pitch, const double* d_roll, int64_t n_roll, double* d_out,
                                     void* stream);

int emagls_decode_stream_reset(emagls_decode_stream* s);

int emagls_decode_stream_info(const emagls_decode_stream* s, int64_t* block, int64_t* partitions, int64_t* state_bytes,
                              int64_t* filter_bytes, int* launches_per_block);

int emagls_decode_stream_destroy(emagls_decode_stream* s);

int emagls_decode_stream_create_bank(int64_t nch, int64_t n_sets, const void* wL, const void* wR, int filters_are_complex, int64_t len,
                                     int in_is_complex, int layout, int basis, int64_t block, emagls_decode_stream** s);

int emagls_decode_stream_push_sets(emagls_decode_stream* s, const void* in, int64_t nsamp, const int32_t* set, int64_t n_set,
                                   const double* yaw, int64_t n_yaw, const double* pitch, int64_t n_pitch, const double* roll,
                                   int64_t n_roll, double* out);

int emagls_decode_stream_push_sets_device(emagls_decode_stream* s, const void* d_in, int64_t nsamp, const int32_t* d_set, int64_t n_set,
                                          const double* d_yaw, int64_t n_yaw, const double* d_pitch, int64_t n_pitch,
                                          const double* d_roll, int64_t n_roll, double* d_out, void* stream);

int emagls_decode_stream_sets(const emagls_decode_stream* s, int64_t* n_sets);

typedef struct emagls_decode_group emagls_decode_group;
int emagls_decode_group_create(int64_t nch, int64_t n_sets, const void* wL, const void* wR, int filters_are_complex, int64_t len,
                               int in_is_complex, int layout, int basis, int64_t block, int64_t n_listeners, emagls_decode_group** g);

int emagls_decode_group_push(emagls_decode_group* g, const void* in, int64_t nsamp, const int32_t* set, int64_t n_set, const double* yaw,
                             int64_t n_yaw, const double* pitch, int64_t n_pitch, const double* roll, int64_t n_roll, double* out);

int emagls_decode_group_push_device(emagls_decode_group* g, const void* d_in, int64_t nsamp, const int32_t* d_set, int64_t n_set,
                                    const double* d_yaw, int64_t n_yaw, const double* d_pitch, int64_t n_pitch, const double* d_roll,
                                    int64_t n_roll, double* d_out, void* stream);

int emagls_decode_group_reset(emagls_decode_group* g, int64_t listener);

int emagls_decode_group_info(const emagls_decode_group* g, int64_t* block, int64_t* partitions, int64_t* listeners, int64_t* state_bytes,
                             int64_t* filter_bytes, int* launches_per_block);

int emagls_decode_group_destroy(emagls_decode_group* g);

int emagls_decode_stream_create_encoded(int64_t nmics, const void* enc, int enc_is_complex, int64_t nch, int64_t n_sets, const void* wL,
                                        const void* wR, int filters_are_complex, int64_t len, int layout, int basis, int64_t block,
                                        emagls_decode_stream** s);
int emagls_decode_group_create_encoded(int64_t nmics, const void* enc, int enc_is_complex, int64_t nch, int64_t n_sets, const void* wL,
                                       const void* wR, int filters_are_complex, int64_t len, int layout, int basis, int64_t block,
                                       int64_t n_listeners, emagls_decode_group** g);

int emagls_get_magls_filters_dc(const double* hL, const double* hR, int64_t nsamp, int64_t ndirs, const double* azi, const double* zen,
                                int order, double fs, int64_t len, int apply_diffuseness_const, int basis, void* wL, void* wR);
int emagls_get_emagls_filters_dc(const double* hL, const double* hR, int64_t nsamp, int64_t ndirs, const double* azi, const double* zen,
                                 double mic_radius, const double* mic_azi, const double* mic_zen, int64_t nmics, int order, double fs,
                                 int64_t len, int apply_diffuseness_const, int basis, void* wL, void* wR);
int emagls_get_emagls2_filters_dc(const double* hL, const double* hR, int64_t nsamp, int64_t ndirs, const double* azi, const double* zen,
                                  double mic_radius, const double* mic_azi, const double* mic_zen, int64_t nmics, int order, double fs,
                                  int64_t len, int apply_diffuseness_const, int basis, void* wL, void* wR);


int emagls_get_magls_filters_2d(const double* hL, const double* hR, int64_t nsamp, int64_t ndirs, const double* hrir_azi,
                                int order, double fs, int64_t len, int basis, void* wL, void* wR);

#define EMAGLS_RADIAL_TIKHONOV 0
#define EMAGLS_RADIAL_SOFTLIMIT 1
#define EMAGLS_RADIAL_FULL 2
#define EMAGLS_RADIAL_NONE 3
int emagls_get_radial_filter(int order, double fs, double sma_radius, int64_t ir_len, int oversampling, int filter_type,
                             double regul_const, double noise_gain_db, void* rad);
int64_t emagls_apply_radial_filter_rows(int64_t nsamp, int64_t ir_len, int oversampling);
int emagls_apply_radial_filter(const double* sig, int64_t nsamp, int order, double fs, double sma_radius, int64_t ir_len,
                               int oversampling, int filter_type, double regul_const, double noise_gain_db, double* out);
int emagls_sh_encode(const double* sig, int64_t nsamp, int64_t nmics, const double* mic_azi, const double* mic_zen, int order,
                     int basis, void* out);
int emagls_ch_basis(int order, int64_t ndirs, const double* azi, int basis, void* Y);
int emagls_get_smair_matrix(int order, double fs, int64_t ir_len, int oversampling, double sma_radius, const double* mic_azi,
                            const double* mic_zen, int64_t nmics, int basis, int return_raw_mic_sigs, int radial_filter_type,
                            double regul_const, double noise_gain_db, void* smair, int* sim_order);
int64_t emagls_eq_filter_nfft(int64_t len);
int emagls_get_magls_spherical_head_filter(double mic_radius, int order, double fs, int64_t len, double* w_shf, double* W_shf);
int emagls_get_magls_array_diffuse_filter(double mic_radius, const double* mic_azi, const double* mic_zen, int64_t nmics, int order,
                                          double fs, int64_t len, int basis, const void* Y_hi, double* w_adf);

#define EMAGLS_MODEL_SH 0
#define EMAGLS_MODEL_EMAGLS 1
#define EMAGLS_MODEL_EMAGLS2 2
#define EMAGLS_MODEL_ATF 3
#define EMAGLS_MODEL_EMA_CH 5
#define EMAGLS_MODEL_EMA_SH 6
int emagls_rendered_hrtfs(int model, const void* wL, const void* wR, int w_is_complex, int64_t len, int64_t nchan, int64_t nsets,
                          const double* dir_azi, const double* dir_zen, int64_t ndirs, double fs, int order, int basis,
                          double mic_radius, const double* mic_azi, const double* mic_zen, int64_t nmics, const double* atf,
                          int64_t atf_taps, int64_t nfft, const double* hL, const double* hR, int64_t nsamp, int64_t nhrir_sets,
                          const double* weights, void* Hhat, double* mag_err_db, double* ild_err_db, double* cov_hat, double* cov_ref);


typedef struct emagls_plan emagls_plan;

typedef struct emagls_design_desc {
    int kind;
    int basis;
    int order;
    double fs;
    int64_t len;
    int64_t nsamp;
    int64_t ndirs;
    double mic_radius;
    int64_t nmics;
    double f_trans;
    int64_t atf_taps;
    int64_t natf;
    int custom_basis;
    int diffuseness;
    int sim_order_pad;
} emagls_design_desc;

typedef struct emagls_plan_info {
    int nfft, num_pos_freqs, k_cut , sim_order, num_sh_sim, num_channels;
    int out_is_complex;
    int64_t out_rows, out_cols;
    double grp_delay_l, grp_delay_r;
    double mean_grid_dev_deg;
    int num_sweep_launches;
    int64_t device_bytes;
    int gram_from, hh_end, hh_orders, g_first;
    int sim_order_own;
    int sweep_form, sweep_units;
} emagls_plan_info;

int emagls_plan_create(const emagls_design_desc* desc, emagls_plan** plan);
int emagls_plan_destroy(emagls_plan* plan);
int emagls_plan_set_hrir_grid(emagls_plan* plan, const double* azi, const double* zen);
int emagls_plan_set_mic_grid(emagls_plan* plan, const double* azi, const double* zen);
int emagls_plan_set_hrirs(emagls_plan* plan, const double* hL, const double* hR);
int emagls_plan_set_basis(emagls_plan* plan, const void* Y_hrir, const void* Y_mic);
int emagls_plan_set_atfs(emagls_plan* plan, const double* atf_irs, const double* atf_azi, const double* atf_zen);
int emagls_plan_execute(emagls_plan* plan);
int emagls_plan_synchronize(emagls_plan* plan);
int emagls_plan_get_filters(emagls_plan* plan, void* wL, void* wR);
int emagls_plan_get_info(emagls_plan* plan, emagls_plan_info* info);
int emagls_plan_sweep_form_in_batch(emagls_plan* plan, int designs, int* form);
int emagls_plan_set_streams(emagls_plan* plan, int nstreams);
int emagls_plan_set_profiling(emagls_plan* plan, int level);
int emagls_plan_num_stages(emagls_plan* plan);
const char* emagls_plan_stage_name(emagls_plan* plan, int stage);
int emagls_plan_stage_times(emagls_plan* plan, double* ms, int n);
int emagls_plan_sweep_kernel_time(emagls_plan* plan, double* total_ms, int* launches);
int emagls_plan_debug_buffer(emagls_plan* plan, const char* name, void* dst, size_t* nbytes);
void* emagls_plan_stream(emagls_plan* plan);

typedef struct emagls_batch emagls_batch;
int emagls_batch_create(emagls_plan** plans, int nplans, emagls_batch** batch);
int emagls_set_batch_max(int max_designs, int* previous);
int emagls_batch_set_geometry_sharing(emagls_batch* batch, int enable);
int emagls_batch_shares_geometry(emagls_batch* batch, int* shared);
int emagls_batch_geometry_runs(emagls_batch* batch, long long* cold, long long* warm);
typedef struct emagls_job {
    emagls_design_desc desc;
    const double* hL;
    const double* hR;
    const double* hrir_azi;
    const double* hrir_zen;
    const double* mic_azi;
    const double* mic_zen;
    const double* atf;
    const double* atf_azi;
    const double* atf_zen;
    void* wL;
    void* wR;
} emagls_job;
#define EMAGLS_JOBS_SHARE_GEOMETRY 1
#define EMAGLS_JOBS_INDEPENDENT 2
int emagls_jobs_run(const emagls_job* jobs, int64_t njobs, int batch_size, int in_flight, int flags);
int emagls_jobs_shard(const emagls_job* jobs, int64_t njobs, int world, int max_batch, int* rank_of_job, int* order_in_rank, int* sim_order_pad);
int emagls_jobs_run_devices(const emagls_job* jobs, int64_t njobs, const int* devices, int ndevices, int batch_size, int in_flight, int flags);
int emagls_design_out_shape(const emagls_design_desc* desc, int64_t* rows, int64_t* cols, int* is_complex);
int emagls_jobs_set_profiling(int level);
int emagls_jobs_sweep_times(double* ms, int* designs, int capacity, int* count);
int emagls_jobs_geometry_runs(long long* independent, long long* cold, long long* warm);
int emagls_jobs_would_share_geometry(const emagls_job* jobs, int njobs, int* share);

int emagls_design_hrir_sets(int kind, const double* hL, const double* hR, int64_t nsamp, int64_t ndirs, int64_t nsets,
                            const double* hrir_azi, const double* hrir_zen, double mic_radius, const double* mic_azi, const double* mic_zen,
                            int64_t nmics, int order, double fs, int64_t len, int basis, void* wL, void* wR);
int emagls_from_atf_hrir_sets(const double* hL, const double* hR, int64_t nsamp, int64_t ndirs, int64_t nsets, const double* hrir_azi,
                              const double* hrir_zen, const double* atf_irs, int64_t atf_taps, int64_t nmics, int64_t natf, const double* atf_azi,
                              const double* atf_zen, double fs, int64_t filter_len, double f_trans, double* wL, double* wR, double* mean_dev);
int emagls_batch_shares_atf_side(emagls_batch* batch, int* shared);
int emagls_batch_execute(emagls_batch* batch);
int emagls_batch_synchronize(emagls_batch* batch);
int emagls_batch_get_filters(emagls_batch* batch, void* const* wL, void* const* wR);
int emagls_batch_set_profiling(emagls_batch* batch, int level);
int emagls_batch_lane_mode(emagls_batch* batch, int* lanes);
int emagls_batch_set_stream(emagls_batch* batch, void* hip_stream);
int emagls_batch_set_side_stream(emagls_batch* batch, void* hip_stream);
int emagls_batch_sweep_time(emagls_batch* batch, double* ms);
int emagls_batch_set_streams(emagls_batch* batch, int nstreams);
int emagls_batch_set_stage_order(emagls_batch* batch, int order);
int emagls_batch_destroy(emagls_batch* batch);

#ifdef __cplusplus
}
#endif
#endif
```

Measured before the change: 3910 filter sets/s.

## Pair two designs sharing geometry per workgroup in register-resident sweep

Adds a PAIR variant of the register-resident sweep kernel in which each workgroup advances two designs that share one geometry. The synthesized operand (synth_units) and the bsc ring are computed once per frequency bin and reused by both per-design chains, while Habs, Winit, outputs, LDS scratch and abort flags are duplicated per chain. This halves the number of workgroups and the repeated synthesis work, at the cost of more LDS, serialized per-design chains inside a block, and different wave-count and residency choices. Pairing is enabled only for batches with shared geometry that are not alone (overridable with EMAGLS_REG_PAIR), and debug entry points expose the chosen layout and a launch counter.

New measurement: 3854 filter sets/s. 0.986x the previous value.

```diff
diff --git a/emagls_amd/_lib.py b/emagls_amd/_lib.py
--- a/emagls_amd/_lib.py
+++ b/emagls_amd/_lib.py
@@ -54,6 +54,8 @@
     "emagls_self_test": (C.c_int, [C.c_int, C.POINTER(C.c_double)]),
     "emagls_debug_synth_operand": (C.c_int, [C.c_void_p, C.c_int, C.c_int, C.c_void_p, c_i64, C.c_int, C.c_void_p, C.c_void_p]),
     "emagls_debug_synth_cosines": (C.c_int, [C.c_void_p, C.c_void_p, c_i64, C.c_void_p, C.c_void_p, C.c_int, C.c_void_p]),
+    "emagls_debug_reg_pair_layout": (C.c_int, [C.c_int, C.c_int, C.c_int, C.c_int, C.POINTER(C.c_int)]),
+    "emagls_debug_reg_pair_launches": (C.c_int, [C.POINTER(C.c_longlong)]),
     "emagls_sh_basis": (C.c_int, [C.c_int, c_i64, C.c_void_p, C.c_void_p, C.c_int, C.c_void_p]),
     "emagls_sh_basis_device": (C.c_int, [C.c_int, c_i64, C.c_void_p, C.c_void_p, C.c_int, C.c_void_p, C.c_void_p]),
     "emagls_modal_bn": (C.c_int, [C.c_int, c_i64, C.c_void_p, C.c_void_p]),
diff --git a/emagls_amd/csrc/batch_run.hip b/emagls_amd/csrc/batch_run.hip
--- a/emagls_amd/csrc/batch_run.hip
+++ b/emagls_amd/csrc/batch_run.hip
@@ -17,6 +17,7 @@
         }
     const bool reg = b.plans[0]->sweep_persist && reg_sweep_wanted(b.plans.data(), nb);
     for (auto* q : b.plans) q->reg_sweep = reg;
+    const bool pair = reg && reg_sweep_pair_wanted(b.geo_share, b.alone, nb) && reg_sweep_pick_waves((int)b.plans[0]->D, nb, true) != 0;
     if (!reg && nb > SWEEP_MULTI_MAX) throw Error(EMAGLS_ERR_UNSUPPORTED, "internal: more than 16 designs in a batch need the register-resident sweep");
     HalfSweepMulti h{};
     h.n = std::min(nb, SWEEP_MULTI_MAX);
@@ -27,7 +28,7 @@
     if (q0.sweep_persist) {
         hipStream_t ss = b.stream;
         {
-            SweepGate gate(ss, reg ? reg_sweep_gate_cost((int)q0.D, nb) : 0);
+            SweepGate gate(ss, reg ? reg_sweep_gate_cost((int)q0.D, nb, pair) : 0);
             if (b.lanes) { BatchScope sc(nb, b.stride); launch_zero(q0.get("ll"), q0.bufs["ll"].bytes, ss); }
             else for (auto* q : b.plans) launch_zero(q->get("ll"), q->bufs["ll"].bytes, ss);
             if (reg) {
@@ -35,7 +36,7 @@
                 reg_args_upload(ha.data(), nb, b.sweep_args_dev, b.sweep_args_last, ss);
             }
             if (b.prof_level >= 1) HIP_CHECK(hipEventRecord(b.sweep_ev[0], ss));
-            if (reg) launch_sweep_reg(static_cast<const HalfSweepArgs*>(b.sweep_args_dev), ha[0], nb, ss);
+            if (reg) launch_sweep_reg(static_cast<const HalfSweepArgs*>(b.sweep_args_dev), ha[0], nb, ss, pair);
             else if (q0.synth) launch_sweep_synth(h, ss); else launch_sweep_persist(h, ss);
             if (b.prof_level >= 1) HIP_CHECK(hipEventRecord(b.sweep_ev[1], ss));
         }
diff --git a/emagls_amd/csrc/capi.hip b/emagls_amd/csrc/capi.hip
--- a/emagls_amd/csrc/capi.hip
+++ b/emagls_amd/csrc/capi.hip
@@ -164,6 +164,20 @@
     });
 }
 
+int emagls_debug_reg_pair_layout(int ndirs, int designs, int cus, int force_waves, int* out) {
+    return guarded([&] {
+        if (!out || ndirs < 1 || designs < 1 || cus < 8) throw Error(EMAGLS_ERR_ARG, "invalid argument");
+        reg_pair_layout_debug(ndirs, designs, cus, force_waves, out);
+    });
+}
+
+int emagls_debug_reg_pair_launches(long long* count) {
+    return guarded([&] {
+        if (!count) throw Error(EMAGLS_ERR_ARG, "invalid argument");
+        *count = reg_pair_launches();
+    });
+}
+
 int emagls_debug_synth_operand(const void* bsc, int nbins, int nord_pad, const double* x, int64_t nx, int gs, void* g_plus, void* g_minus) {
     return guarded([&] { synth_operand_debug(bsc, nbins, nord_pad, x, nx, gs, g_plus, g_minus); });
 }
diff --git a/emagls_amd/csrc/kernels.hpp b/emagls_amd/csrc/kernels.hpp
--- a/emagls_amd/csrc/kernels.hpp
+++ b/emagls_amd/csrc/kernels.hpp
@@ -104,10 +104,13 @@
 size_t reg_sweep_ll_bytes(int D, int nmics);
 int reg_sweep_capacity(int D);
 int reg_sweep_slots_per_xcd();
-int reg_sweep_pick_waves(int D, int ndesigns);
-int reg_sweep_gate_cost(int D, int ndesigns);
-bool reg_sweep_fits(int D, int nmics, int nunits, int nOrd, int ndesigns);
-void launch_sweep_reg(const HalfSweepArgs* args_dev, const HalfSweepArgs& a0, int n, hipStream_t st);
+bool reg_sweep_pair_wanted(bool one_geometry, bool alone, int ndesigns);
+int reg_sweep_pick_waves(int D, int ndesigns, bool pair = false);
+int reg_sweep_gate_cost(int D, int ndesigns, bool pair = false);
+bool reg_sweep_fits(int D, int nmics, int nunits, int nOrd, int ndesigns, bool pair = false);
+void launch_sweep_reg(const HalfSweepArgs* args_dev, const HalfSweepArgs& a0, int n, hipStream_t st, bool pair = false);
+long long reg_pair_launches();
+void reg_pair_layout_debug(int D, int ndesigns, int cus, int force_nw, int* out);
 double reg_contract_selftest();
 double gram_tile_selftest(bool four);
 void store_sweep_args(const HalfSweepArgs* host, int n, HalfSweepArgs* dev, hipStream_t st);
diff --git a/emagls_amd/csrc/sweep_reg.hip b/emagls_amd/csrc/sweep_reg.hip
--- a/emagls_amd/csrc/sweep_reg.hip
+++ b/emagls_amd/csrc/sweep_reg.hip
@@ -3,8 +3,11 @@
 #include "synth_common.hpp"
 
 #include <algorithm>
+#include <atomic>
 #include <map>
 #include <mutex>
+#include <tuple>
+#include <type_traits>
 
 namespace emagls {
 
@@ -124,9 +127,10 @@
 constexpr int RG_NEX = 4 * PS_CMAX;
 constexpr int RG_SVC = 256;
 
-template <int NUL, int NW>
+template <int NUL, int NW, bool PAIR>
 __global__ void __launch_bounds__(64 * NW) __attribute__((amdgpu_waves_per_eu(3))) sweep_reg_kernel(const HalfSweepArgs* __restrict__ args, int n, int nWG, int spread, int prio) {
     constexpr int NT = 64 * NW, DPW = 32 * NW;
+    constexpr int NCH = PAIR ? 2 : 1;
     constexpr int NU2 = 2 * NUL;
     constexpr int NVW = 8 * NU2;
     constexpr int GA = (NUL + 1) / 2, GB = NUL - GA;
@@ -134,50 +138,66 @@
     extern __shared__ __attribute__((aligned(16))) char dyn[];
     cplx* ring = reinterpret_cast<cplx*>(dyn);
     cplx* ms = ring + 2 * SY_NORD;
-    cplx* WE = ms + PS_CMAX * RG_MLD;
-    cplx* WO = WE + 2 * NU2;
-    double* vt = reinterpret_cast<double*>(WO + 2 * NU2);
-    double* wpart = vt + 2 * RG_NEX;
-    double* xs = wpart + NW * NVW;
+    constexpr int WCS = 4 * NU2, VCS = 2 * RG_NEX + NW * NVW;
+    cplx* WE0 = ms + PS_CMAX * RG_MLD;
+    double* vt0 = reinterpret_cast<double*>(WE0 + NCH * WCS);
+    double* xs = vt0 + NCH * VCS;
     __shared__ int s_abort, s_local;
 
     int design, member;
-    if (spread) {
+    if (spread && !PAIR) {
         design = (int)blockIdx.x / nWG;
         member = (int)blockIdx.x - design * nWG;
     } else {
         const int xcd = blockIdx.x & 7, rest = blockIdx.x >> 3;
         const int sub = rest / nWG;
         member = rest - sub * nWG;
-        design = xcd + 8 * sub;
+        design = NCH * (xcd + 8 * sub);
     }
     if (design >= n) return;
+    const bool hasB = PAIR && design + 1 < n;
     if (prio) __builtin_amdgcn_s_setprio(3);
     const HalfSweepArgs& a = args[design];
     const int tid = threadIdx.x;
     const int C = a.C, P = a.P, D = a.D, kfirst = a.kfirst, kabs0 = a.kabs0;
     const int64_t ldH = a.ldH;
     const int nord_pad = a.nord_pad;
-    const gcd_t Habs = RG_GLOBAL(const double, a.Habs);
     const gcc_t Mw = RG_GLOBAL(const cplx, a.Mw);
     const gcc_t bsc = RG_GLOBAL(const cplx, a.bsc);
-    const gcd_t Winit = RG_GLOBAL(const double, a.Winit);
-    cplx __attribute__((address_space(1)))* const Uout = RG_GLOBAL(cplx, a.U);
-    long long* const timing = a.timing;
-    int* const abort_flag = a.abort_flag;
     const long long wait_ticks = a.wait_ticks;
     const int* smap = a.smap;
     const int npr = smap[32], nsg = smap[33], nun = npr + nsg;
-    const gu64_t part_ll = RG_GLOBAL(u64, a.ll);
-    const gu64_t xcc_ll = part_ll + (size_t)2 * nWG * RG_NEX * 2;
+    gcd_t Habs_c[NCH], Winit_c[NCH];
+    cplx __attribute__((address_space(1)))* Uout_c[NCH];
+    long long* timing_c[NCH];
+    int* abort_c[NCH];
+    gu64_t part_c[NCH];
+#pragma unroll
+    for (int c = 0; c < NCH; ++c) {
+        const HalfSweepArgs& ac = args[design + ((c && hasB) ? 1 : 0)];
+        Habs_c[c] = RG_GLOBAL(const double, ac.Habs);
+        Winit_c[c] = RG_GLOBAL(const double, ac.Winit);
+        Uout_c[c] = RG_GLOBAL(cplx, ac.U);
+        timing_c[c] = ac.timing;
+        abort_c[c] = ac.abort_flag;
+        part_c[c] = RG_GLOBAL(u64, ac.ll);
+    }
+    long long* const timing = timing_c[0];
+    int* const abort_flag = abort_c[0];
+    const gu64_t xcc_ll = part_c[0] + (size_t)2 * nWG * RG_NEX * 2;
+    auto flag_both = [&]() __attribute__((always_inline)) {
+        if (PAIR && hasB && tid == 0)
+#pragma unroll
+            for (int c = 0; c < NCH; ++c) __hip_atomic_store(abort_c[c], 1, __ATOMIC_RELAXED, __HIP_MEMORY_SCOPE_AGENT);
+    };
     if (tid == 0) { s_abort = 0; s_local = 0; }
     const int d0 = member * DPW;
     auto dir_of = [&](int t, int s) __attribute__((always_inline)) { return d0 + 32 * (t >> 6) + 16 * s + ((t & 63) >> 2); };
 
     {
-        const size_t ncplx = (size_t)2 * SY_NORD + PS_CMAX * RG_MLD + 4 * NU2;
+        const size_t ncplx = (size_t)2 * SY_NORD + PS_CMAX * RG_MLD + NCH * WCS;
         for (size_t i = tid; i < ncplx; i += NT) ring[i] = mk(0, 0);
-        for (int i = tid; i < 2 * RG_NEX + NW * NVW; i += NT) vt[i] = 0.0;
+        for (int i = tid; i < NCH * VCS; i += NT) vt0[i] = 0.0;
         double sd[2], cd[2], daz[2];
 #pragma unroll
         for (int s = 0; s < 2; ++s) {
@@ -218,14 +238,15 @@
 #pragma unroll
         for (int i = 0; i < NLM; ++i) ms[r * RG_MLD + c0 + i] = (r < C && c0 + i < C) ? mReg[i] : mk(0, 0);
     };
-    double hCur[2], hNext[2] = {0.0, 0.0};
-    auto fetch_h = [&](int kb, double (&h)[2], int t) __attribute__((always_inline)) {
+    double hCur[2];
+    auto fetch_h = [&](gcd_t Habs, int kb, double (&h)[2], int t) __attribute__((always_inline)) {
         const int kbg = (kb < P ? kb : P - 1) - kabs0;
         const gcd_t He = Habs + ((int64_t)((t >> 1) & 1) * (P - kabs0) + kbg) * ldH;
 #pragma unroll
         for (int s = 0; s < 2; ++s) h[s] = He[dir_of(t, s) < D ? dir_of(t, s) : D - 1];
     };
-    fetch_h(kfirst, hCur, tid);
+    hCur[0] = 0.0; hCur[1] = 0.0;
+    if (!PAIR) fetch_h(Habs_c[0], kfirst, hCur, tid);
     if (tid < RG_SVC) { fetch_m(kfirst, tid); stage_m(tid); }
 
     if (tid < 64) {
@@ -251,7 +272,7 @@
     }
     __syncthreads();
     const bool local = s_local != 0;
-    if (s_abort) return;
+    if (s_abort) { flag_both(); return; }
 
     const bool slot8 = nun > 16 || GB < 2;
     cplx E[NUL], O[NUL];
@@ -259,26 +280,25 @@
     for (int u = 0; u < NUL; ++u) { E[u] = mk(0, 0); O[u] = mk(0, 0); }
 
 #define RSTAMP(i) do { if (timing && member == 1 && tid == 0 && kb < P) timing[(int64_t)kb * 16 + (i)] = (long long)wall_clock64(); } while (0)
-    for (int kb = kfirst; kb <= P; ++kb) {
+    auto run_chain = [&](auto cc, int kb) __attribute__((always_inline)) -> int {
+        constexpr int ch = decltype(cc)::value;
         const bool first = (kb == kfirst);
         const bool last = (kb == P);
         const bool nyq = (kb == P - 1);
-        RSTAMP(7);
-        if (!last) {
-            const cplx* bs = ring + (kb & 1) * SY_NORD;
-            const double* xcol = xs + launder(tid);
-            synth_units<0, GA, NUL, NT>(xcol, E, O, bs, nord_pad);
-            __builtin_amdgcn_sched_barrier(0);
-            if (slot8) synth_units<GA, GB, NUL, NT>(xcol, E, O, bs, nord_pad);
-            else synth_units<GA, GB - 1, NUL, NT>(xcol, E, O, bs, nord_pad);
-            __builtin_amdgcn_sched_barrier(0);
-        }
+        long long* const timing = timing_c[ch];
+        int* const abort_flag = abort_c[ch];
+        const gu64_t part_ll = part_c[ch];
+        cplx* const WE = WE0 + ch * WCS;
+        cplx* const WO = WE + 2 * NU2;
+        double* const vt = vt0 + ch * VCS;
+        double* const wpart = vt + 2 * RG_NEX;
+        const bool moves_m = !PAIR || ch == 1 || !hasB;
         RSTAMP(0);
         if (launder(tid) < RG_SVC) {
             const int t = launder(tid);
             const int j = t & (RG_NEX - 1), half = t >> 7;
             if (first) {
-                vt[t] = half == 0 ? Winit[j] : 0.0;
+                vt[t] = half == 0 ? Winit_c[ch][j] : 0.0;
             } else {
                 const unsigned tag = (unsigned)(kb - 1);
                 const gu64_t src = part_ll + ((size_t)((kb - 1) & 1) * nWG * RG_NEX + j) * 2;
@@ -309,7 +329,9 @@
         }
         RSTAMP(2);
         __syncthreads();
-        if (s_abort) break;
+        if (s_abort) return 1;
+        double hL[2] = {0.0, 0.0};
+        if (PAIR) fetch_h(Habs_c[ch], kb, hL, launder(tid));
         if (launder(tid) < RG_SVC) {
             const int t = launder(tid);
             const int part = t & 3, pair = t >> 2, e = pair >> 5, c = pair & 31;
@@ -331,16 +353,16 @@
                     WE[e * NU2 + npr + (c - 2 * npr)] = acc; WO[e * NU2 + npr + (c - 2 * npr)] = acc;
                 }
                 if (member == 0 && !first) {
-                    cplx __attribute__((address_space(1)))* dst = Uout + ((int64_t)e * P + (kb - 1)) * PS_CMAX + c;
+                    cplx __attribute__((address_space(1)))* dst = Uout_c[ch] + ((int64_t)e * P + (kb - 1)) * PS_CMAX + c;
                     const cplx v = vc[c] + vc[RG_NEX / 2 + c];
                     dst->x = v.x; dst->y = v.y;
                 }
             }
         }
-        if (last) break;
+        if (last) return 2;
         __syncthreads();
         RSTAMP(3);
-        const bool svc = launder(tid) < RG_SVC;
+        const bool svc = launder(tid) < RG_SVC && moves_m;
         if (svc) fetch_m(kb, launder(tid));
         cplx ts[2];
         {
@@ -375,7 +397,7 @@
             for (int s = 0; s < 2; ++s) {
                 const cplx pe0 = group_sum<4>(p[s][0]), pe1 = group_sum<4>(p[s][1]);
                 const cplx pe = (x & 2) ? pe1 : pe0;
-                ts[s] = dir_of(t, s) < D ? unit_phase(hCur[s], pe, nyq) : mk(0, 0);
+                ts[s] = dir_of(t, s) < D ? unit_phase(PAIR ? hL[s] : hCur[s], pe, nyq) : mk(0, 0);
             }
         }
         __builtin_amdgcn_sched_barrier(0);
@@ -385,8 +407,8 @@
         }
         {
             const int t = launder(tid);
-            fetch_h(kb + 1, hNext, t);
-            if (t < nord_pad) ring[(kb & 1) * SY_NORD + t] = ldg(bsc + (int64_t)(kb + 2 < P ? kb + 2 : P - 1) * nord_pad + t);
+            if (!PAIR) fetch_h(Habs_c[0], kb + 1, hCur, t);
+            if (ch == 0 && t < nord_pad) ring[(kb & 1) * SY_NORD + t] = ldg(bsc + (int64_t)(kb + 2 < P ? kb + 2 : P - 1) * nord_pad + t);
         }
         __syncthreads();
         RSTAMP(4);
@@ -409,8 +431,27 @@
             gll_put(dst + 1, tg | (bits >> 32), local);
         }
         RSTAMP(5);
-        hCur[0] = hNext[0]; hCur[1] = hNext[1];
-    }
+        return 0;
+    };
+    for (int kb = kfirst; kb <= P; ++kb) {
+        RSTAMP(7);
+        if (kb != P) {
+            const cplx* bs = ring + (kb & 1) * SY_NORD;
+            const double* xcol = xs + launder(tid);
+            synth_units<0, GA, NUL, NT>(xcol, E, O, bs, nord_pad);
+            __builtin_amdgcn_sched_barrier(0);
+            if (slot8) synth_units<GA, GB, NUL, NT>(xcol, E, O, bs, nord_pad);
+            else synth_units<GA, GB - 1, NUL, NT>(xcol, E, O, bs, nord_pad);
+            __builtin_amdgcn_sched_barrier(0);
+        }
+        int r = run_chain(std::integral_constant<int, 0>{}, kb);
+        if (PAIR && hasB && r != 1) {
+            if (r == 2) __syncthreads();
+            r = run_chain(std::integral_constant<int, NCH - 1>{}, kb);
+        }
+        if (r) break;
+    }
+    if (s_abort) flag_both();
 #undef RSTAMP
 }
 
@@ -438,42 +479,60 @@
 }
 static_assert(sizeof(HalfSweepArgs) % 8 == 0, "argument block in whole words");
 
-size_t reg_dyn_bytes(int nul, int nw) {
-    const size_t nu2 = 2 * (size_t)nul, nvw = 8 * nu2;
-    return sizeof(cplx) * ((size_t)2 * SY_NORD + PS_CMAX * RG_MLD + 4 * nu2) +
-           sizeof(double) * (2 * RG_NEX + (size_t)nw * nvw + (size_t)nul * 64 * nw);
+size_t reg_dyn_bytes(int nul, int nw, bool pair) {
+    const size_t nu2 = 2 * (size_t)nul, nvw = 8 * nu2, nch = pair ? 2 : 1;
+    return sizeof(cplx) * ((size_t)2 * SY_NORD + PS_CMAX * RG_MLD + nch * 4 * nu2) +
+           sizeof(double) * (nch * (2 * RG_NEX + (size_t)nw * nvw) + (size_t)nul * 64 * nw);
 }
 constexpr int RG_WAVES[] = {4, 6, 8, 10, 12};
-const void* reg_kernel_ptr(int nw) {
+constexpr int RG_NFORMS = (int)(sizeof(RG_WAVES) / sizeof(RG_WAVES[0]));
+template <bool PAIR> const void* reg_kernel_ptr_of(int nw) {
     switch (nw) {
-        case 4: return reinterpret_cast<const void*>(sweep_reg_kernel<RG_NUL, 4>);
-        case 6: return reinterpret_cast<const void*>(sweep_reg_kernel<RG_NUL, 6>);
-        case 8: return reinterpret_cast<const void*>(sweep_reg_kernel<RG_NUL, 8>);
-        case 10: return reinterpret_cast<const void*>(sweep_reg_kernel<RG_NUL, 10>);
-        default: return reinterpret_cast<const void*>(sweep_reg_kernel<RG_NUL, 12>);
-    }
-}
+        case 4: return reinterpret_cast<const void*>(sweep_reg_kernel<RG_NUL, 4, PAIR>);
+        case 6: return reinterpret_cast<const void*>(sweep_reg_kernel<RG_NUL, 6, PAIR>);
+        case 8: return reinterpret_cast<const void*>(sweep_reg_kernel<RG_NUL, 8, PAIR>);
+        case 10: return reinterpret_cast<const void*>(sweep_reg_kernel<RG_NUL, 10, PAIR>);
+        default: return reinterpret_cast<const void*>(sweep_reg_kernel<RG_NUL, 12, PAIR>);
+    }
+}
+const void* reg_kernel_ptr(int nw, bool pair) { return pair ? reg_kernel_ptr_of<true>(nw) : reg_kernel_ptr_of<false>(nw); }
 void reg_set_attributes() {
     static PerDeviceOnce attr_once;
     if (attr_once.first())
-        for (int nw : RG_WAVES) HIP_CHECK(hipFuncSetAttribute(reg_kernel_ptr(nw), hipFuncAttributeMaxDynamicSharedMemorySize, 150 * 1024));
+        for (int nw : RG_WAVES)
+            for (int pair = 0; pair < 2; ++pair) HIP_CHECK(hipFuncSetAttribute(reg_kernel_ptr(nw, pair != 0), hipFuncAttributeMaxDynamicSharedMemorySize, 150 * 1024));
 }
 int reg_nwg(int D, int nw) { return (int)ceil_div(D, 32 * nw); }
-int reg_occupancy(int nw) {
+int reg_occupancy(int nw, bool pair) {
     static std::mutex mu;
-    static std::map<std::pair<int, int>, int> cache;
+    static std::map<std::tuple<int, int, bool>, int> cache;
     int dev = 0;
     HIP_CHECK(hipGetDevice(&dev));
     std::lock_guard<std::mutex> lk(mu);
-    auto it = cache.find({dev, nw});
+    auto it = cache.find({dev, nw, pair});
     if (it != cache.end()) return it->second;
     reg_set_attributes();
     int nb = 0;
-    if (hipOccupancyMaxActiveBlocksPerMultiprocessor(&nb, reg_kernel_ptr(nw), 64 * nw, reg_dyn_bytes(RG_NUL, nw)) != hipSuccess) { (void)hipGetLastError(); nb = 0; }
-    cache[{dev, nw}] = nb;
+    if (hipOccupancyMaxActiveBlocksPerMultiprocessor(&nb, reg_kernel_ptr(nw, pair), 64 * nw, reg_dyn_bytes(RG_NUL, nw, pair)) != hipSuccess) { (void)hipGetLastError(); nb = 0; }
+    cache[{dev, nw, pair}] = nb;
     return nb;
 }
 int reg_wg_cost(int nw) { return nw == 4 ? 1 : 3; }
+bool reg_valid_waves(int nw) { for (int w : RG_WAVES) if (w == nw) return true; return false; }
+
+int reg_pair_pick(int D, int npairs, int cus, const int* occ, int force_nw) {
+    if (npairs < 1 || 2 * npairs > REG_SWEEP_MAX + 1) return 0;
+    const int nsub = (int)ceil_div(npairs, 8);
+    auto fits = [&](int i) { return nsub * reg_nwg(D, RG_WAVES[i]) <= cus && occ[i] >= 1; };
+    for (int i = 0; i < RG_NFORMS; ++i)
+        if (RG_WAVES[i] == force_nw && fits(i)) return force_nw;
+    for (int i = RG_NFORMS; i-- > 0;)
+        if (fits(i)) return RG_WAVES[i];
+    return 0;
+}
+int reg_pair_cost(int D, int npairs, int nw) { return nw ? (int)ceil_div(npairs, 8) * reg_nwg(D, nw) * 3 : 0; }
+std::atomic<long long> g_pair_launches{0};
+int reg_forced_waves() { const char* e = getenv("EMAGLS_REG_WAVES"); return e ? atoi(e) : 0; }
 
 }
 
@@ -487,56 +546,89 @@
     return sizeof(u64) * ((size_t)2 * nwg * RG_NEX * 2 + nwg + 64);
 }
 int reg_sweep_slots_per_xcd() { return 3 * (sweep_cu_budget() / 8); }
-int reg_sweep_pick_waves(int D, int ndesigns) {
+bool reg_sweep_pair_wanted(bool one_geometry, bool alone, int ndesigns) {
+    const char* e = getenv("EMAGLS_REG_PAIR");
+    const int mode = e ? atoi(e) : 1;
+    return mode != 0 && one_geometry && ndesigns >= 2 && (mode == 2 || !alone);
+}
+static int reg_pair_pick_waves(int D, int ndesigns);
+int reg_sweep_pick_waves(int D, int ndesigns, bool pair) {
+    if (pair) return reg_pair_pick_waves(D, ndesigns);
     if (ndesigns < 1 || ndesigns > REG_SWEEP_MAX) return 0;
     const int nsub = (int)ceil_div(ndesigns, 8), cus = sweep_cu_budget() / 8;
     if (const char* e = getenv("EMAGLS_REG_WAVES")) {
         const int nw = atoi(e);
-        if ((nw == 4 || nw == 6 || nw == 8 || nw == 10 || nw == 12) && nsub * reg_nwg(D, nw) * reg_wg_cost(nw) <= 3 * cus && reg_occupancy(nw) >= (nw == 4 ? 3 : 1)) return nw;
-    }
-    for (int nw : RG_WAVES) if (nsub * reg_nwg(D, nw) <= cus && reg_occupancy(nw) >= 1) return nw;
-    return (nsub * reg_nwg(D, 4) <= 3 * cus && reg_occupancy(4) >= 3) ? 4 : 0;
+        if (reg_valid_waves(nw) && nsub * reg_nwg(D, nw) * reg_wg_cost(nw) <= 3 * cus && reg_occupancy(nw, false) >= (nw == 4 ? 3 : 1)) return nw;
+    }
+    for (int nw : RG_WAVES) if (nsub * reg_nwg(D, nw) <= cus && reg_occupancy(nw, false) >= 1) return nw;
+    return (nsub * reg_nwg(D, 4) <= 3 * cus && reg_occupancy(4, false) >= 3) ? 4 : 0;
 }
 int reg_sweep_spread_waves(int D, int ndesigns) {
     const char* es = getenv("EMAGLS_REG_SPREAD");
     const int mode = es ? atoi(es) : 2;
     if (mode == 0 || ndesigns < 1 || ndesigns > REG_SWEEP_MAX || getenv("EMAGLS_REG_WAVES")) return 0;
-    const int cus = sweep_cu_budget(), local = reg_sweep_pick_waves(D, ndesigns);
+    const int cus = sweep_cu_budget(), local = reg_sweep_pick_waves(D, ndesigns, false);
     for (int nw : RG_WAVES)
-        if (ndesigns * reg_nwg(D, nw) <= cus && reg_occupancy(nw) >= 1) return (mode == 1 || local == 0 || nw < local) ? nw : 0;
+        if (ndesigns * reg_nwg(D, nw) <= cus && reg_occupancy(nw, false) >= 1) return (mode == 1 || local == 0 || nw < local) ? nw : 0;
     return 0;
 }
-int reg_sweep_gate_cost(int D, int ndesigns) {
+static int reg_pair_pick_waves(int D, int ndesigns) {
+    if (ndesigns < 2 || ndesigns > REG_SWEEP_MAX) return 0;
+    int occ[RG_NFORMS];
+    for (int i = 0; i < RG_NFORMS; ++i) occ[i] = reg_occupancy(RG_WAVES[i], true);
+    int prefer = reg_forced_waves();
+    if (!reg_valid_waves(prefer)) prefer = reg_sweep_spread_waves(D, ndesigns);
+    if (!prefer) prefer = reg_sweep_pick_waves(D, ndesigns, false);
+    return reg_pair_pick(D, (int)ceil_div(ndesigns, 2), sweep_cu_budget() / 8, occ, prefer);
+}
+int reg_sweep_gate_cost(int D, int ndesigns, bool pair) {
+    if (pair) return reg_pair_cost(D, (int)ceil_div(ndesigns, 2), reg_pair_pick_waves(D, ndesigns));
     if (const int ns = reg_sweep_spread_waves(D, ndesigns)) return (int)ceil_div((int64_t)ndesigns * reg_nwg(D, ns), 8) * reg_wg_cost(ns);
-    const int nw = reg_sweep_pick_waves(D, ndesigns);
+    const int nw = reg_sweep_pick_waves(D, ndesigns, false);
     return nw ? (int)ceil_div(ndesigns, 8) * reg_nwg(D, nw) * reg_wg_cost(nw) : 0;
 }
 int reg_sweep_capacity(int D) {
     int n = 0;
-    for (int k = 8; k <= REG_SWEEP_MAX; k += 8) if (reg_sweep_pick_waves(D, k)) n = k;
+    for (int k = 8; k <= REG_SWEEP_MAX; k += 8) if (reg_sweep_pick_waves(D, k, false)) n = k;
     return n;
 }
-bool reg_sweep_fits(int D, int nmics, int nunits, int nOrd, int ndesigns) {
-    return reg_sweep_supported(D, nmics, nunits, nOrd) && reg_sweep_pick_waves(D, ndesigns) != 0;
-}
-
-void launch_sweep_reg(const HalfSweepArgs* args_dev, const HalfSweepArgs& a0, int n, hipStream_t st) {
-    const int ns = reg_sweep_spread_waves(a0.D, n);
-    const int nw = ns ? ns : reg_sweep_pick_waves(a0.D, n);
+bool reg_sweep_fits(int D, int nmics, int nunits, int nOrd, int ndesigns, bool pair) {
+    return reg_sweep_supported(D, nmics, nunits, nOrd) && reg_sweep_pick_waves(D, ndesigns, pair) != 0;
+}
+long long reg_pair_launches() { return g_pair_launches.load(std::memory_order_relaxed); }
+void reg_pair_layout_debug(int D, int ndesigns, int cus, int force_nw, int* out) {
+    const int occ[RG_NFORMS] = {1, 1, 1, 1, 1};
+    const int npairs = (int)ceil_div(ndesigns, 2);
+    const int nw = (ndesigns >= 2 && ndesigns <= REG_SWEEP_MAX && D >= 1) ? reg_pair_pick(D, npairs, cus / 8, occ, force_nw) : 0;
+    out[0] = nw;
+    out[1] = nw ? reg_nwg(D, nw) : 0;
+    out[2] = npairs * out[1];
+    out[3] = reg_pair_cost(D, npairs, nw);
+    out[4] = 3 * (cus / 8);
+}
+
+void launch_sweep_reg(const HalfSweepArgs* args_dev, const HalfSweepArgs& a0, int n, hipStream_t st, bool pair) {
+    const int ns = pair ? 0 : reg_sweep_spread_waves(a0.D, n);
+    const int nw = ns ? ns : reg_sweep_pick_waves(a0.D, n, pair);
     if (!nw) throw Error(2, "register-resident sweep: the launch cannot be resident");
     const int nWG = reg_nwg(a0.D, nw), spread = ns ? 1 : 0;
-    const unsigned nblocks = spread ? (unsigned)(n * nWG) : 8u * (unsigned)nWG * (unsigned)ceil_div(n, 8);
-    const size_t dyn = reg_dyn_bytes(RG_NUL, nw);
+    const unsigned nblocks = spread ? (unsigned)(n * nWG) : 8u * (unsigned)nWG * (unsigned)ceil_div(pair ? (int)ceil_div(n, 2) : n, 8);
+    const size_t dyn = reg_dyn_bytes(RG_NUL, nw, pair);
     reg_set_attributes();
     static const int prio = [] { const char* e = getenv("EMAGLS_REG_PRIO"); return e ? atoi(e) : 1; }();
+#define EMAGLS_REG_LAUNCH(NW_) do { \
+        if (pair) sweep_reg_kernel<RG_NUL, NW_, true><<<dim3(nblocks), 64 * NW_, dyn, st>>>(args_dev, n, nWG, spread, prio); \
+        else sweep_reg_kernel<RG_NUL, NW_, false><<<dim3(nblocks), 64 * NW_, dyn, st>>>(args_dev, n, nWG, spread, prio); } while (0)
     switch (nw) {
-        case 4: sweep_reg_kernel<RG_NUL, 4><<<dim3(nblocks), 256, dyn, st>>>(args_dev, n, nWG, spread, prio); break;
-        case 6: sweep_reg_kernel<RG_NUL, 6><<<dim3(nblocks), 384, dyn, st>>>(args_dev, n, nWG, spread, prio); break;
-        case 8: sweep_reg_kernel<RG_NUL, 8><<<dim3(nblocks), 512, dyn, st>>>(args_dev, n, nWG, spread, prio); break;
-        case 10: sweep_reg_kernel<RG_NUL, 10><<<dim3(nblocks), 640, dyn, st>>>(args_dev, n, nWG, spread, prio); break;
-        default: sweep_reg_kernel<RG_NUL, 12><<<dim3(nblocks), 768, dyn, st>>>(args_dev, n, nWG, spread, prio); break;
-    }
+        case 4: EMAGLS_REG_LAUNCH(4); break;
+        case 6: EMAGLS_REG_LAUNCH(6); break;
+        case 8: EMAGLS_REG_LAUNCH(8); break;
+        case 10: EMAGLS_REG_LAUNCH(10); break;
+        default: EMAGLS_REG_LAUNCH(12); break;
+    }
+#undef EMAGLS_REG_LAUNCH
     KERNEL_CHECK();
+    if (pair) g_pair_launches.fetch_add(1, std::memory_order_relaxed);
 }
 
 double reg_contract_selftest() {
diff --git a/include/emagls.h b/include/emagls.h
--- a/include/emagls.h
+++ b/include/emagls.h
@@ -39,6 +39,9 @@
 int emagls_self_test(int which, double* max_err);
 int emagls_debug_synth_operand(const void* bsc, int nbins, int nord_pad, const double* x, int64_t nx, int gs, void* g_plus, void* g_minus);
 int emagls_debug_synth_cosines(const double* dir_azi, const double* dir_zen, int64_t ndirs, const double* mic_azi, const double* mic_zen, int nmics, double* x2);
+
+int emagls_debug_reg_pair_layout(int ndirs, int designs, int cus, int force_waves, int* out);
+int emagls_debug_reg_pair_launches(long long* count);
 
 
 int emagls_sh_basis(int order, int64_t ndirs, const double* azi, const double* zen, int basis, void* Y);
```
